# befelix/safe_learning

Hardware: NVIDIA H100
Metric: grid-point Lyapunov checks/sec (2D pendulum, M=500 GP) (higher is better)
Workload: dtype f64

## Files before the change

### include/slb200.h

```cpp
#ifndef SLB200_H
#define SLB200_H

#include <stdint.h>

#ifdef __cplusplus
extern "C" {
#endif

#define SLB_ABI_VERSION 6
#define SLB_MAX_DIM 6
#define SLB_MAX_IN  8
#define SLB_MAX_OUT 6
#define SLB_MAX_ACT 2
#define SLB_TILE_POINTS 64
#define SLB_HEAD_RANK 64
#define SLB_MAX_RANKS 16

typedef struct slb_grid {
    int32_t ndim;
    int32_t _pad;
    int64_t nindex;
    int64_t num_points[SLB_MAX_DIM];
    double  offset[SLB_MAX_DIM];
    double  unit_maxes[SLB_MAX_DIM];
    double  upper[SLB_MAX_DIM];
    const double* discrete_points;
} slb_grid;

enum slb_fn_kind {
    SLB_FN_NONE = 0,
    SLB_FN_CONSTANT = 1,
    SLB_FN_LINEAR = 2,
    SLB_FN_QUADRATIC = 3,
    SLB_FN_TRIANGULATION = 4,
    SLB_FN_PENDULUM = 5,
    SLB_FN_CARTPOLE = 6,
    SLB_FN_LYAPUNOV_NN = 7,
    SLB_FN_MLP = 8,
    SLB_FN_VANDERPOL = 9,
    SLB_FN_PIECEWISE_CONSTANT = 10
};
#define SLB_FLAG_SATURATE 1u
#define SLB_FLAG_ABS      2u
#define SLB_FLAG_NORM1    4u
#define SLB_FLAG_PROJECT  8u
#define SLB_FLAG_SCALE   16u
#define SLB_FLAG_GRADIENT 32u
#define SLB_FLAG_MAXABS  64u

typedef struct slb_function {
    int32_t kind;
    int32_t in_dim;
    int32_t out_dim;
    uint32_t flags;
    double  out_scale;
    double  lower, upper;
    double  cparams[24];
    const double*  matrix;
    const double*  hyperplanes;
    const int64_t* unit_simplices;
    const int32_t* corner_simplex;
    int32_t nsimplex;
    int32_t _pad;
    slb_grid grid;
} slb_function;

enum slb_kernel_kind {
    SLB_K_RBF = 0,
    SLB_K_MATERN12 = 1,
    SLB_K_MATERN32 = 2,
    SLB_K_MATERN52 = 3,
    SLB_K_LINEAR = 4,
    SLB_K_CONSTANT = 5,
    SLB_K_WHITE = 6
};
#define SLB_MAX_KPRIM 6

typedef struct slb_kernel_prim {
    int32_t kind;
    int32_t term;
    double  variance;
    double  w[SLB_MAX_IN];
} slb_kernel_prim;

typedef struct slb_kernel {
    int32_t num_prims;
    int32_t _pad;
    slb_kernel_prim prims[SLB_MAX_KPRIM];
} slb_kernel;

typedef struct slb_gp_factor {
    int32_t M;
    int32_t nrb;
    const double* Xs;
    const double* Wpack;
    double lengthscales[SLB_MAX_IN];
    double variance;
    double scale;
    double kss;
    slb_kernel kernel;
    const double* Whead;
    const double* Wheadp;
    const double* Xhead;
    int32_t head_rows;
    int32_t _pad2;
    const double* Xf;
    double hmax;
} slb_gp_factor;

typedef struct slb_gp_output {
    int32_t factor;
    int32_t _pad;
    double  beta;
    const double* alpha;
    const double* gamma;
    const double* prior_mean;
    const double* gamma_f;
    double gamma_l1;
} slb_gp_output;

typedef struct slb_gp_stack {
    int32_t num_outputs;
    int32_t num_factors;
    int32_t input_dim;
    int32_t _pad;
    slb_gp_factor factors[SLB_MAX_OUT];
    slb_gp_output outputs[SLB_MAX_OUT];
} slb_gp_stack;

typedef struct slb_sweep {
    slb_grid     grid;
    slb_function policy;
    slb_function dynamics;
    slb_gp_stack gp;
    slb_function lyapunov;
    slb_function lipschitz_v;
    double lv_const;
    double lf_const;
    double tau;
    slb_function lipschitz_f;
    const double* lf_values;
    int64_t lf_index_base;
} slb_sweep;

typedef struct slb_bellman {
    slb_grid     grid;
    slb_function policy;
    slb_function dynamics;
    slb_gp_stack gp;
    slb_function reward;
    slb_function value;
    double gamma;
    int32_t fixed_action;
    int32_t _pad;
    double action[SLB_MAX_ACT];
} slb_bellman;


typedef struct slb_fail_key {
    uint64_t key_value;
    int64_t  key_index;
    int64_t  n_ok;
    int64_t  _pad;
} slb_fail_key;

typedef struct slb_prefix_stats {
    int64_t  n_safe;
    int64_t  n_below;
    uint64_t max_below;
    uint64_t max_all;
} slb_prefix_stats;

typedef struct slb_exchange {
    int32_t world;
    int32_t rank;
    slb_fail_key* slots[SLB_MAX_RANKS];
    int64_t* seq_dev;
} slb_exchange;

int         slb_abi_version(void);
const char* slb_last_error(void);
int         slb_device_count(void);
int         slb_struct_sizes(int64_t* out, int32_t n);
int64_t     slb_launch_count(void);
void        slb_note_graph_replay(int64_t kernels);

int         slb_debug_phase_timing(void* buffer_dev);
int         slb_debug_head_timing(void* buffer_dev);
int         slb_debug_stage1_timing(void* buffer_dev);
int         slb_record_factor_dependency(void* stream);
int         slb_restore_tables(void* dst_dev, const void* src_host, int64_t split_bytes, int64_t total_bytes,
                               void* stream, void* side_stream);
int         slb_debug_filter_stages(int32_t mask);
int         slb_debug_screening_probe(double* mu_dev, double* dm_dev);
int         slb_debug_det_fast(int32_t enable);
int         slb_debug_refine_split(int64_t upto32);

int64_t slb_packed_len(int32_t M);
int slb_pack_factor(void* stream, const double* Linv_dev, int32_t M, double* Wpack_dev);

int slb_pivoted_subset(void* stream, const double* kernel_dev, int32_t M, int32_t r,
                       int64_t* picks_dev, double* scratch_dev);

int slb_gp_predict(void* stream, const slb_gp_stack* gp, const double* points_dev, int64_t n,
                   double* mean_dev, double* err_dev, int32_t want_var);
int slb_gp_mean(void* stream, const slb_gp_stack* gp, const double* points_dev, int64_t n, double* mean_dev);
int64_t slb_gp_vjp_workspace(const slb_gp_stack* gp, int64_t n);
int slb_gp_vjp(void* stream, const slb_gp_stack* gp, const double* points_dev, int64_t n,
               const double* grad_mean_dev, const double* grad_err_dev, double* grad_points_dev,
               void* workspace_dev);

#define SLB_GP_HYPER_TILE 64
#define SLB_GP_HYPER_SLOTS (SLB_MAX_KPRIM * (1 + SLB_MAX_IN) + 1)
int64_t slb_gp_lml_grad_workspace(int32_t M);
int slb_gp_lml_grad(void* stream, const double* X_dev, int32_t M, int32_t d_in, const slb_kernel* kern,
                    const double* Kinv_dev, const double* alpha_dev, double* grad_dev, void* workspace_dev);
int slb_gp_lml_grad_cols(void* stream, const double* X_dev, int32_t M, int32_t d_in, const slb_kernel* kern,
                         const double* Kinv_dev, const double* alpha_dev, int32_t k, double* grad_dev,
                         void* workspace_dev);

int slb_lyapunov_sweep(void* stream, const slb_sweep* cfg, int64_t idx_begin, int64_t idx_end,
                       uint8_t* negative_dev, double* values_dev, double* decrease_dev,
                       double* threshold_dev, double* mean_dev, double* err_dev);
int64_t slb_filter_workspace(int64_t n);
int slb_debug_filter_lists(int64_t n, int64_t* offsets);
int slb_filter_stage1(const slb_sweep* cfg);
#define SLB_MEAN_NONE 0
#define SLB_MEAN_FP64 1
#define SLB_MEAN_FP32_SCREENED 2
#define SLB_MEAN_GRID_FACTORED 3
int slb_filter_mean_scheme(const slb_sweep* cfg);
int slb_lyapunov_sweep_filtered(void* stream, const slb_sweep* cfg, int64_t idx_begin,
                                int64_t idx_end, uint8_t* negative_dev, double* values_dev,
                                void* workspace_dev, int64_t* stats_dev);
int slb_safe_set_step(void* stream, const slb_sweep* cfg, int64_t idx_begin, int64_t idx_end,
                      uint8_t* negative_dev, const double* values_dev, const uint8_t* initial_dev,
                      void* workspace_dev, int64_t* stats_dev, slb_fail_key* key_dev, uint8_t* safe_dev,
                      slb_prefix_stats* prefix_stats_dev);
int slb_debug_refine(void* stream, const slb_sweep* cfg, int64_t idx_begin, int64_t n_max,
                     const int64_t* list_dev, const unsigned long long* count_dev,
                     uint8_t* negative_dev, double* values_dev, double* mean_dev, double* err_dev,
                     void* workspace_dev);
int slb_lyapunov_points(void* stream, const slb_sweep* cfg, const double* states_dev, int64_t n,
                        uint8_t* negative_dev, double* values_dev, double* decrease_dev,
                        double* threshold_dev, double* mean_dev, double* err_dev);

int64_t slb_first_fail_workspace(int64_t n);
int slb_first_fail(void* stream, const double* values_dev, const uint8_t* negative_dev,
                   const uint8_t* initial_dev , int64_t n, int64_t idx_begin,
                   void* workspace_dev, slb_fail_key* result_dev);
int slb_first_fail_x(void* stream, const double* values_dev, const uint8_t* negative_dev,
                     const uint8_t* initial_dev, int64_t n, int64_t idx_begin, void* workspace_dev,
                     slb_fail_key* result_dev, const slb_exchange* xchg);
int slb_apply_prefix_x(void* stream, const double* values_dev, const uint8_t* initial_dev,
                       int64_t n, int64_t idx_begin, slb_fail_key* key_out_dev, uint8_t* safe_dev,
                       void* workspace_dev, slb_prefix_stats* stats_dev, const slb_exchange* xchg);
int slb_combine_fail_keys(void* stream, const slb_fail_key* gathered_dev, int32_t world,
                          slb_fail_key* out_dev);
int slb_apply_prefix(void* stream, const double* values_dev, const uint8_t* initial_dev,
                     int64_t n, int64_t idx_begin, const slb_fail_key* key_dev,
                     uint8_t* safe_dev, void* workspace_dev, slb_prefix_stats* stats_dev);

int64_t slb_no_shrink_workspace(int64_t n, int64_t batch);
int slb_no_shrink_scan(void* stream, const int64_t* order_dev, const uint8_t* negative_dev,
                       const uint8_t* prev_safe_dev, const uint8_t* initial_dev, const double* n_req_dev,
                       int64_t n, int64_t batch, int64_t max_refinement, void* workspace_dev,
                       uint8_t* candidates_dev);
int slb_no_shrink_resolve(void* stream, const int64_t* order_dev, const double* values_dev,
                          const uint8_t* negative_dev, const uint8_t* prev_safe_dev,
                          const int64_t* prev_refinement_dev, const uint8_t* initial_dev,
                          const double* n_req_dev, const uint8_t* refined_dev, int64_t n, int64_t batch,
                          int64_t max_refinement, void* workspace_dev, uint8_t* safe_dev,
                          int64_t* refinement_dev, int64_t* cmax_position_dev, double* cmax_dev);

int slb_eval_function(void* stream, const slb_function* fn, const double* points_dev, int64_t n,
                      double* out_dev);
int slb_function_columns(const slb_function* fn);
int slb_index_to_state(void* stream, const slb_grid* grid, int64_t idx_begin, int64_t idx_end,
                       double* states_dev);

int slb_bellman_sweep(void* stream, const slb_bellman* cfg, int64_t idx_begin, int64_t idx_end,
                      double* out_dev);
int64_t slb_bellman_argmax_workspace(const slb_bellman* cfg, int32_t n_actions);
int slb_bellman_argmax(void* stream, const slb_bellman* cfg, int64_t idx_begin, int64_t idx_end,
                       const double* actions_dev, int32_t n_actions, const double* constraint_dev,
                       int32_t* best_dev, double* best_value_dev, void* workspace_dev);
int slb_max_abs_diff(void* stream, const double* a_dev, const double* b_dev, int64_t n,
                     double* result_dev);

int64_t slb_rollout_workspace(const slb_bellman* cfg, int64_t n, int32_t reward);
int slb_rollout(void* stream, const slb_bellman* cfg, const double* states_dev, int64_t idx_begin,
                int64_t n, int32_t horizon, const double* equilibrium_host, double tol,
                uint8_t* roa_dev, double* end_states_dev, double* traj_dev, void* workspace_dev);
int slb_reward_rollout(void* stream, const slb_bellman* cfg, const double* states_dev, int64_t idx_begin,
                       int64_t n, int32_t horizon, const double* discount_dev, double tol,
                       double* sums_dev, int64_t* stop_dev, void* workspace_dev);
int slb_rollout_gp_mean(void* stream, const slb_bellman* cfg, const double* states_dev, int64_t idx_begin,
                        int64_t n, int32_t horizon, const double* equilibrium_host, double tol,
                        uint8_t* roa_dev, double* end_states_dev, double* traj_dev, void* workspace_dev);
int slb_reward_rollout_gp_mean(void* stream, const slb_bellman* cfg, const double* states_dev,
                               int64_t idx_begin, int64_t n, int32_t horizon, const double* discount_dev,
                               double tol, double* sums_dev, int64_t* stop_dev, void* workspace_dev);

#define SLB_VALUE_STATS 16
#define SLB_VALUE_CONVERGED 0
#define SLB_VALUE_MAX_ITERS 1
#define SLB_VALUE_NEGATIVE_WEIGHT 2
#define SLB_VALUE_NOT_CONTRACTIVE 3
#define SLB_VALUE_NAN 4
int slb_value_operator(void* stream, const slb_bellman* cfg, int64_t idx_begin, int64_t idx_end,
                       void* cols_dev, double* weights_dev, double* rewards_dev, uint64_t* stats_dev);
int slb_value_operator_points(void* stream, const slb_function* value, const double* next_states_dev,
                              int64_t n, void* cols_dev, double* weights_dev, uint64_t* stats_dev);
int64_t slb_value_solve_workspace(int64_t n, int32_t ncols);
int slb_value_solve(void* stream, int64_t n, int32_t ncols, const void* cols_dev, const double* weights_dev,
                    const double* rewards_dev, double gamma, double tol, int64_t max_iters,
                    double* v_inout_dev, void* workspace_dev, uint64_t* stats_dev);

int64_t slb_function_vjp_workspace(const slb_function* fn, int64_t n);
int slb_function_vjp(void* stream, const slb_function* fn, const double* points_dev, int64_t n,
                     const double* grad_out_dev, double* grad_in_dev, double* grad_params_dev,
                     double* out_dev, void* workspace_dev);
int slb_grid_nearest_index(void* stream, const slb_grid* grid, const double* points_dev, int64_t n,
                           int64_t* idx_dev);
int slb_triangulation_rows(void* stream, const slb_function* fn, const double* points_dev, int64_t n,
                           int64_t* cols_dev, double* weights_dev);

#ifdef __cplusplus
}
#endif
#endif
```

### safe_learning_b200/_native.py

```python

from __future__ import annotations

import ctypes as C
import os

SLB_MAX_DIM = 6
SLB_MAX_IN = 8
SLB_MAX_OUT = 6
SLB_MAX_ACT = 2
SLB_TILE_POINTS = 64
SLB_HEAD_RANK = 64
SLB_MAX_RANKS = 16

FN_NONE, FN_CONSTANT, FN_LINEAR, FN_QUADRATIC, FN_TRIANGULATION, FN_PENDULUM, FN_CARTPOLE, \
    FN_LYAPUNOV_NN, FN_MLP, FN_VANDERPOL, FN_PIECEWISE_CONSTANT = range(11)
FLAG_SATURATE, FLAG_ABS, FLAG_NORM1, FLAG_PROJECT, FLAG_SCALE, FLAG_GRADIENT, FLAG_MAXABS = \
    1, 2, 4, 8, 16, 32, 64
K_RBF, K_MATERN12, K_MATERN32, K_MATERN52, K_LINEAR, K_CONSTANT, K_WHITE = range(7)
SLB_MAX_KPRIM = 6
SLB_GP_HYPER_TILE = 64
SLB_GP_HYPER_SLOTS = SLB_MAX_KPRIM * (1 + SLB_MAX_IN) + 1
ABI_VERSION = 6
VALUE_STATS = 16
VALUE_CONVERGED, VALUE_MAX_ITERS, VALUE_NEGATIVE_WEIGHT, VALUE_NOT_CONTRACTIVE, VALUE_NAN = range(5)
MEAN_NONE, MEAN_FP64, MEAN_FP32_SCREENED, MEAN_GRID_FACTORED = range(4)

UINT64_MAX = (1 << 64) - 1
INT64_MAX = (1 << 63) - 1


class NativeLibraryError(RuntimeError):
    """libslb200 is missing, mismatched, or reported an error."""


class SlbGrid(C.Structure):
    _fields_ = [("ndim", C.c_int32), ("_pad", C.c_int32), ("nindex", C.c_int64),
                ("num_points", C.c_int64 * SLB_MAX_DIM), ("offset", C.c_double * SLB_MAX_DIM),
                ("unit_maxes", C.c_double * SLB_MAX_DIM), ("upper", C.c_double * SLB_MAX_DIM),
                ("discrete_points", C.c_void_p)]


class SlbFunction(C.Structure):
    _fields_ = [("kind", C.c_int32), ("in_dim", C.c_int32), ("out_dim", C.c_int32),
                ("flags", C.c_uint32), ("out_scale", C.c_double), ("lower", C.c_double),
                ("upper", C.c_double), ("cparams", C.c_double * 24), ("matrix", C.c_void_p),
                ("hyperplanes", C.c_void_p), ("unit_simplices", C.c_void_p),
                ("corner_simplex", C.c_void_p), ("nsimplex", C.c_int32), ("_pad", C.c_int32), ("grid", SlbGrid)]


class SlbKernelPrim(C.Structure):
    _fields_ = [("kind", C.c_int32), ("term", C.c_int32), ("variance", C.c_double),
                ("w", C.c_double * SLB_MAX_IN)]


class SlbKernel(C.Structure):
    _fields_ = [("num_prims", C.c_int32), ("_pad", C.c_int32),
                ("prims", SlbKernelPrim * SLB_MAX_KPRIM)]


class SlbGpFactor(C.Structure):
    _fields_ = [("M", C.c_int32), ("nrb", C.c_int32), ("Xs", C.c_void_p), ("Wpack", C.c_void_p),
                ("lengthscales", C.c_double * SLB_MAX_IN), ("variance", C.c_double),
                ("scale", C.c_double), ("kss", C.c_double), ("kernel", SlbKernel),
                ("Whead", C.c_void_p), ("Wheadp", C.c_void_p), ("Xhead", C.c_void_p),
                ("head_rows", C.c_int32),
                ("_pad2", C.c_int32), ("Xf", C.c_void_p), ("hmax", C.c_double)]


class SlbGpOutput(C.Structure):
    _fields_ = [("factor", C.c_int32), ("_pad", C.c_int32), ("beta", C.c_double),
                ("alpha", C.c_void_p), ("gamma", C.c_void_p), ("prior_mean", C.c_void_p),
                ("gamma_f", C.c_void_p), ("gamma_l1", C.c_double)]


class SlbGpStack(C.Structure):
    _fields_ = [("num_outputs", C.c_int32), ("num_factors", C.c_int32),
                ("input_dim", C.c_int32), ("_pad", C.c_int32),
                ("factors", SlbGpFactor * SLB_MAX_OUT), ("outputs", SlbGpOutput * SLB_MAX_OUT)]


class SlbSweep(C.Structure):
    _fields_ = [("grid", SlbGrid), ("policy", SlbFunction), ("dynamics", SlbFunction),
                ("gp", SlbGpStack), ("lyapunov", SlbFunction), ("lipschitz_v", SlbFunction),
                ("lv_const", C.c_double), ("lf_const", C.c_double), ("tau", C.c_double),
                ("lipschitz_f", SlbFunction), ("lf_values", C.c_void_p),
                ("lf_index_base", C.c_int64)]


class SlbBellman(C.Structure):
    _fields_ = [("grid", SlbGrid), ("policy", SlbFunction), ("dynamics", SlbFunction),
                ("gp", SlbGpStack), ("reward", SlbFunction), ("value", SlbFunction),
                ("gamma", C.c_double), ("fixed_action", C.c_int32), ("_pad", C.c_int32),
                ("action", C.c_double * SLB_MAX_ACT)]


class SlbFailKey(C.Structure):
    _fields_ = [("key_value", C.c_uint64), ("key_index", C.c_int64), ("n_ok", C.c_int64),
                ("_pad", C.c_int64)]


class SlbPrefixStats(C.Structure):
    _fields_ = [("n_safe", C.c_int64), ("n_below", C.c_int64), ("max_below", C.c_uint64),
                ("max_all", C.c_uint64)]


class SlbExchange(C.Structure):
    _fields_ = [("world", C.c_int32), ("rank", C.c_int32),
                ("slots", C.c_void_p * SLB_MAX_RANKS), ("seq_dev", C.c_void_p)]


_STRUCTS = (SlbGrid, SlbFunction, SlbGpFactor, SlbGpOutput, SlbGpStack, SlbSweep, SlbBellman,
            SlbFailKey, SlbPrefixStats, SlbExchange)

LIB_PATH = os.path.join(os.path.dirname(os.path.abspath(__file__)), "libslb200.so")

_vp, _i64, _i32, _dp = C.c_void_p, C.c_int64, C.c_int32, C.c_void_p

SIGNATURES = {
    "slb_abi_version": (C.c_int, []),
    "slb_last_error": (C.c_char_p, []),
    "slb_device_count": (C.c_int, []),
    "slb_struct_sizes": (C.c_int, [C.POINTER(C.c_int64), _i32]),
    "slb_launch_count": (C.c_int64, []),
    "slb_note_graph_replay": (None, [_i64]),
    "slb_debug_phase_timing": (C.c_int, [_vp]),
    "slb_debug_head_timing": (C.c_int, [_vp]),
    "slb_debug_stage1_timing": (C.c_int, [_vp]),
    "slb_record_factor_dependency": (C.c_int, [_vp]),
    "slb_restore_tables": (C.c_int, [_vp, _vp, _i64, _i64, _vp, _vp]),
    "slb_debug_refine_split": (C.c_int, [_i64]),
    "slb_debug_det_fast": (C.c_int, [_i32]),
    "slb_debug_filter_stages": (C.c_int, [_i32]),
    "slb_debug_screening_probe": (C.c_int, [_dp, _dp]),
    "slb_filter_stage1": (C.c_int, [C.POINTER(SlbSweep)]),
    "slb_filter_mean_scheme": (C.c_int, [C.POINTER(SlbSweep)]),
    "slb_packed_len": (C.c_int64, [_i32]),
    "slb_pack_factor": (C.c_int, [_vp, _dp, _i32, _dp]),
    "slb_pivoted_subset": (C.c_int, [_vp, _dp, _i32, _i32, _vp, _dp]),
    "slb_gp_predict": (C.c_int, [_vp, C.POINTER(SlbGpStack), _dp, _i64, _dp, _dp, _i32]),
    "slb_lyapunov_sweep": (C.c_int, [_vp, C.POINTER(SlbSweep), _i64, _i64, _dp, _dp, _dp, _dp,
                                     _dp, _dp]),
    "slb_lyapunov_points": (C.c_int, [_vp, C.POINTER(SlbSweep), _dp, _i64, _dp, _dp, _dp, _dp,
                                      _dp, _dp]),
    "slb_filter_workspace": (C.c_int64, [_i64]),
    "slb_debug_filter_lists": (C.c_int, [_i64, C.POINTER(C.c_int64)]),
    "slb_lyapunov_sweep_filtered": (C.c_int, [_vp, C.POINTER(SlbSweep), _i64, _i64, _dp, _dp, _vp,
                                              _vp]),
    "slb_safe_set_step": (C.c_int, [_vp, C.POINTER(SlbSweep), _i64, _i64, _dp, _dp, _dp, _vp, _vp, _vp,
                                    _dp, _vp]),
    "slb_debug_refine": (C.c_int, [_vp, C.POINTER(SlbSweep), _i64, _i64, _vp, _vp, _vp, _dp, _dp, _dp,
                                   _vp]),
    "slb_first_fail_workspace": (C.c_int64, [_i64]),
    "slb_first_fail_x": (C.c_int, [_vp, _dp, _dp, _dp, _i64, _i64, _vp, _vp,
                                   C.POINTER(SlbExchange)]),
    "slb_apply_prefix_x": (C.c_int, [_vp, _dp, _dp, _i64, _i64, _vp, _dp, _vp, _vp,
                                     C.POINTER(SlbExchange)]),
    "slb_first_fail": (C.c_int, [_vp, _dp, _dp, _dp, _i64, _i64, _vp, _vp]),
    "slb_combine_fail_keys": (C.c_int, [_vp, _vp, _i32, _vp]),
    "slb_apply_prefix": (C.c_int, [_vp, _dp, _dp, _i64, _i64, _vp, _dp, _vp, _vp]),
    "slb_no_shrink_workspace": (C.c_int64, [_i64, _i64]),
    "slb_no_shrink_scan": (C.c_int, [_vp, _dp, _dp, _dp, _dp, _dp, _i64, _i64, _i64, _vp, _dp]),
    "slb_no_shrink_resolve": (C.c_int, [_vp, _dp, _dp, _dp, _dp, _dp, _dp, _dp, _dp, _i64, _i64, _i64,
                                        _vp, _dp, _dp, _dp, _dp]),
    "slb_eval_function": (C.c_int, [_vp, C.POINTER(SlbFunction), _dp, _i64, _dp]),
    "slb_function_columns": (C.c_int, [C.POINTER(SlbFunction)]),
    "slb_index_to_state": (C.c_int, [_vp, C.POINTER(SlbGrid), _i64, _i64, _dp]),
    "slb_bellman_sweep": (C.c_int, [_vp, C.POINTER(SlbBellman), _i64, _i64, _dp]),
    "slb_bellman_argmax_workspace": (C.c_int64, [C.POINTER(SlbBellman), _i32]),
    "slb_bellman_argmax": (C.c_int, [_vp, C.POINTER(SlbBellman), _i64, _i64, _dp, _i32, _dp, _dp,
                                     _dp, _vp]),
    "slb_max_abs_diff": (C.c_int, [_vp, _dp, _dp, _i64, _dp]),
    "slb_rollout_workspace": (C.c_int64, [C.POINTER(SlbBellman), _i64, _i32]),
    "slb_rollout": (C.c_int, [_vp, C.POINTER(SlbBellman), _dp, _i64, _i64, _i32, _dp, C.c_double,
                              _vp, _dp, _dp, _vp]),
    "slb_reward_rollout": (C.c_int, [_vp, C.POINTER(SlbBellman), _dp, _i64, _i64, _i32, _dp,
                                     C.c_double, _dp, _vp, _vp]),
    "slb_rollout_gp_mean": (C.c_int, [_vp, C.POINTER(SlbBellman), _dp, _i64, _i64, _i32, _dp, C.c_double,
                                      _vp, _dp, _dp, _vp]),
    "slb_reward_rollout_gp_mean": (C.c_int, [_vp, C.POINTER(SlbBellman), _dp, _i64, _i64, _i32, _dp,
                                             C.c_double, _dp, _vp, _vp]),
    "slb_value_operator": (C.c_int, [_vp, C.POINTER(SlbBellman), _i64, _i64, _vp, _dp, _dp, _vp]),
    "slb_value_operator_points": (C.c_int, [_vp, C.POINTER(SlbFunction), _dp, _i64, _vp, _dp, _vp]),
    "slb_value_solve_workspace": (C.c_int64, [_i64, _i32]),
    "slb_value_solve": (C.c_int, [_vp, _i64, _i32, _vp, _dp, _dp, C.c_double, C.c_double, _i64, _dp,
                                  _vp, _vp]),
    "slb_function_vjp_workspace": (C.c_int64, [C.POINTER(SlbFunction), _i64]),
    "slb_function_vjp": (C.c_int, [_vp, C.POINTER(SlbFunction), _dp, _i64, _dp, _dp, _dp, _dp, _vp]),
    "slb_triangulation_rows": (C.c_int, [_vp, C.POINTER(SlbFunction), _dp, _i64, _vp, _dp]),
    "slb_grid_nearest_index": (C.c_int, [_vp, C.POINTER(SlbGrid), _dp, _i64, _vp]),
    "slb_gp_mean": (C.c_int, [_vp, C.POINTER(SlbGpStack), _dp, _i64, _dp]),
    "slb_gp_vjp_workspace": (C.c_int64, [C.POINTER(SlbGpStack), _i64]),
    "slb_gp_vjp": (C.c_int, [_vp, C.POINTER(SlbGpStack), _dp, _i64, _dp, _dp, _dp, _vp]),
    "slb_gp_lml_grad_workspace": (C.c_int64, [_i32]),
    "slb_gp_lml_grad": (C.c_int, [_vp, _dp, _i32, _i32, C.POINTER(SlbKernel), _dp, _dp, _dp, _vp]),
    "slb_gp_lml_grad_cols": (C.c_int, [_vp, _dp, _i32, _i32, C.POINTER(SlbKernel), _dp, _dp, _i32, _dp, _vp]),
}

_lib = None


def load():
    global _lib
    if _lib is not None:
        return _lib
    if not os.path.exists(LIB_PATH):
        raise NativeLibraryError(
            "%s not found: build it with `python -c 'import __graft_entry__ as g; g.build()'` "
            "(nvcc, sm_90a). safe_learning_b200 has no CPU fallback." % LIB_PATH)
    lib = C.CDLL(LIB_PATH)
    for name, (res, args) in SIGNATURES.items():
        fn = getattr(lib, name)
        fn.restype = res
        fn.argtypes = args
    if lib.slb_abi_version() != ABI_VERSION:
        raise NativeLibraryError("libslb200 ABI version %d != %d (rebuild: python -c 'import "
                                 "__graft_entry__ as g; g.build()')"
                                 % (lib.slb_abi_version(), ABI_VERSION))
    _check_layout(lib)
    _lib = lib
    return lib


def _check_layout(lib):
    sizes = (C.c_int64 * len(_STRUCTS))()
    n = lib.slb_struct_sizes(sizes, len(_STRUCTS))
    if n != len(_STRUCTS):
        raise NativeLibraryError("libslb200 reports %d ABI structs, binding has %d"
                                 % (n, len(_STRUCTS)))
    for st, size in zip(_STRUCTS, sizes):
        if C.sizeof(st) != size:
            raise NativeLibraryError("layout mismatch for %s: ctypes %d bytes, C %d bytes"
                                     % (st.__name__, C.sizeof(st), size))


def last_error():
    return load().slb_last_error().decode("utf-8", "replace")


def check(rc, what):
    if rc != 0:
        raise NativeLibraryError("%s failed (rc=%d): %s" % (what, rc, last_error()))


def require_device():
    lib = load()
    n = lib.slb_device_count()
    if n <= 0:
        raise NativeLibraryError("no CUDA device available: %s" % (last_error() or "count=0"))
    return n


def launch_count():
    return int(load().slb_launch_count())
```

### safe_learning_b200/csrc/common.cuh

```cuda
#pragma once
#include <cuda_runtime.h>
#include <stdint.h>
#include <math.h>

#include <type_traits>

#include "../../include/slb200.h"
#include "exp2_tab64.h"

constexpr int SLB_NUM_SMS = 132;

void slb_set_error(const char* fmt, ...);
void slb_count_launch();

#define SLB_CHECK(cond, ...)                                                     \
    do {                                                                         \
        if (!(cond)) { slb_set_error(__VA_ARGS__); return 1; }                   \
    } while (0)

#define SLB_CUDA(call)                                                           \
    do {                                                                         \
        cudaError_t e__ = (call);                                                \
        if (e__ != cudaSuccess) {                                                \
            slb_set_error("%s failed: %s (%s:%d)", #call, cudaGetErrorString(e__), \
                          __FILE__, __LINE__);                                   \
            return 2;                                                            \
        }                                                                        \
    } while (0)

#define SLB_LAUNCH_CHECK()                                                       \
    do {                                                                         \
        slb_count_launch();                                                      \
        SLB_CUDA(cudaGetLastError());                                            \
    } while (0)

int slb_validate_function(const slb_function* f, const char* what, int expect_in );
int slb_fn_columns(const slb_function& f);
int slb_validate_dynamics(const slb_function* f, const char* who, int d, int m);
int slb_validate_kernel(const slb_kernel& K, int d_in, const char* who);
int slb_validate_gp(const slb_gp_stack* gp);
int slb_validate_staged_tables(const slb_gp_stack* gp, const char* who);
int slb_validate_grid(const slb_grid* g, bool need_points);
int slb_validate_range(const char* who, int64_t idx_begin, int64_t idx_end, int64_t nindex);
int slb_validate_sweep(const slb_sweep* cfg, bool explicit_states, int* m_out);

template <int LO, int HI, class F>
int slb_dispatch_dim(int d, const char* what, F&& launch) {
    SLB_CHECK(d >= LO && d <= HI, "%s %d not compiled (%d..%d)", what, d, LO, HI);
    if constexpr (LO < HI) {
        if (d > LO) return slb_dispatch_dim<LO + 1, HI>(d, what, launch);
    }
    return launch(std::integral_constant<int, LO>{});
}

#define SLB_DEV __device__ __forceinline__

SLB_DEV double f64mul(double a, double b) { return __dmul_rn(a, b); }
SLB_DEV double f64add(double a, double b) { return __dadd_rn(a, b); }
SLB_DEV double f64sub(double a, double b) { return __dsub_rn(a, b); }

SLB_DEV uint64_t value_key(double v) {
    if (v == 0.0) v = 0.0;
    uint64_t b = (uint64_t)__double_as_longlong(v);
    return (b & 0x8000000000000000ull) ? ~b : (b | 0x8000000000000000ull);
}
SLB_DEV double key_value(uint64_t k) {
    uint64_t b = (k & 0x8000000000000000ull) ? (k & 0x7fffffffffffffffull) : ~k;
    return __longlong_as_double((long long)b);
}

struct __align__(16) slb_fold {
    unsigned long long lo, hi;
    unsigned long long n_ok;
    unsigned int ticket;
    unsigned int _pad;
    unsigned long long acc[4];
};
struct slb_fold_target {
    const double* values;
    const uint8_t* initial;
    slb_fold* rec;
};

SLB_DEV unsigned long long atom_cas128(slb_fold* p, unsigned long long lo, unsigned long long hi,
                                       unsigned long long new_lo, unsigned long long new_hi,
                                       unsigned long long* got_hi) {
    unsigned long long got_lo;
    asm volatile("{\n\t.reg .b128 d, c, s;\n\t"
                 "mov.b128 c, {%2, %3};\n\t"
                 "mov.b128 s, {%4, %5};\n\t"
                 "atom.global.cas.b128 d, [%6], c, s;\n\t"
                 "mov.b128 {%0, %1}, d;\n\t}"
                 : "=l"(got_lo), "=l"(*got_hi)
                 : "l"(lo), "l"(hi), "l"(new_lo), "l"(new_hi), "l"(p)
                 : "memory");
    return got_lo;
}

SLB_DEV void fold_key(slb_fold* rec, uint64_t kv, int64_t ki) {
    const unsigned long long hi = ~kv, lo = (unsigned long long)(INT64_MAX - ki);
    unsigned long long cur_hi;
    asm volatile("ld.relaxed.gpu.global.u64 %0, [%1];" : "=l"(cur_hi) : "l"(&rec->hi) : "memory");
    if (hi < cur_hi) return;
    unsigned long long cur_lo = 0;
    while (hi > cur_hi || (hi == cur_hi && lo > cur_lo)) {
        unsigned long long got_hi;
        const unsigned long long got_lo = atom_cas128(rec, cur_lo, cur_hi, lo, hi, &got_hi);
        if (got_lo == cur_lo && got_hi == cur_hi) return;
        cur_lo = got_lo;
        cur_hi = got_hi;
    }
}

SLB_DEV void fold_decided(const slb_fold_target& t, bool mine, bool negative, int64_t rel, int64_t idx_begin) {
    const bool ok = mine && (negative || (t.initial != nullptr && t.initial[rel] != 0));
    const bool fail = mine && !ok;
    const unsigned okb = __ballot_sync(0xffffffffu, ok);
    const unsigned failb = __ballot_sync(0xffffffffu, fail);
    uint64_t kv = fail ? value_key(t.values[rel]) : ~0ull;
    int64_t ki = fail ? idx_begin + rel : INT64_MAX;
    if (failb != 0) {
#pragma unroll
        for (int off = 16; off > 0; off >>= 1) {
            const uint64_t ov = __shfl_xor_sync(0xffffffffu, kv, off);
            const int64_t oi = __shfl_xor_sync(0xffffffffu, ki, off);
            if (ov < kv || (ov == kv && oi < ki)) { kv = ov; ki = oi; }
        }
    }
    if ((threadIdx.x & 31) != 0) return;
    if (okb != 0) atomicAdd(&t.rec->n_ok, (unsigned long long)__popc(okb));
    if (failb != 0) fold_key(t.rec, kv, ki);
}

__constant__ double c_exp2_tab[64] = {SLB_EXP2_TAB64};

SLB_DEV void load_exp_table(double* tab_smem) {
    for (int i = threadIdx.x; i < 64; i += blockDim.x) tab_smem[i] = c_exp2_tab[i];
}

SLB_DEV double exp_neg_tab(double x, const double* __restrict__ tab) {
    const double MAGIC = 6755399441055744.0;
    const double t = fma(x, 92.33248261689366, MAGIC);
    const int n = __double2loint(t);
    const double nd = t - MAGIC;
    double r = fma(nd, -0.01083042469326756, x);
    r = fma(nd, -2.9815858269852933e-12, r);
    double p = 1.0 / 120.0;
    p = fma(p, r, 1.0 / 24.0);
    p = fma(p, r, 1.0 / 6.0);
    p = fma(p, r, 0.5);
    p = fma(p, r, 1.0);
    p = p * r;
    const double T = tab[n & 63];
    const double v = fma(T, p, T);
    const double s = __hiloint2double(__double2hiint(v) + ((n >> 6) << 20), __double2loint(v));
    return x < -700.0 ? 0.0 : s;
}

template <int DIN>
SLB_DEV double kernel_expr_cross(const slb_kernel& K, const double* z, const double* x,
                                 const double* exptab) {
    double total = 0.0, term = 1.0;
    int cur = 0;
    for (int i = 0; i < K.num_prims; ++i) {
        const slb_kernel_prim& P = K.prims[i];
        if (P.term != cur) { total += term; term = 1.0; cur = P.term; }
        double v;
        if (P.kind == SLB_K_LINEAR) {
            v = 0.0;
#pragma unroll
            for (int c = 0; c < DIN; ++c) v = fma(P.w[c] * z[c], x[c], v);
        } else if (P.kind == SLB_K_CONSTANT) {
            v = P.variance;
        } else if (P.kind == SLB_K_WHITE) {
            v = 0.0;
        } else {
            double r2 = 0.0;
#pragma unroll
            for (int c = 0; c < DIN; ++c) {
                const double df = (z[c] - x[c]) * P.w[c];
                r2 = fma(df, df, r2);
            }
            if (P.kind == SLB_K_RBF) {
                v = P.variance * exp_neg_tab(-0.5 * r2, exptab);
            } else {
                const double r = sqrt(r2 + 1e-12);
                if (P.kind == SLB_K_MATERN12) {
                    v = P.variance * exp_neg_tab(-r, exptab);
                } else if (P.kind == SLB_K_MATERN32) {
                    const double sr = 1.7320508075688772 * r;
                    v = P.variance * (1.0 + sr) * exp_neg_tab(-sr, exptab);
                } else {
                    const double sr = 2.23606797749979 * r;
                    v = P.variance * (1.0 + sr + (5.0 / 3.0) * (r * r)) * exp_neg_tab(-sr, exptab);
                }
            }
        }
        term *= v;
    }
    return K.num_prims > 0 ? total + term : 0.0;
}

template <int DIN, int U>
SLB_DEV void kernel_expr_cross_n(const slb_kernel& K, const double* z, const double* const (&x)[U],
                                 const double* exptab, double (&out)[U]) {
    double total[U], term[U];
#pragma unroll
    for (int u = 0; u < U; ++u) { total[u] = 0.0; term[u] = 1.0; }
    int cur = 0;
    for (int i = 0; i < K.num_prims; ++i) {
        const slb_kernel_prim& P = K.prims[i];
        const int kind = P.kind;
        const double var = P.variance;
        if (P.term != cur) {
#pragma unroll
            for (int u = 0; u < U; ++u) { total[u] += term[u]; term[u] = 1.0; }
            cur = P.term;
        }
        double w[DIN];
#pragma unroll
        for (int c = 0; c < DIN; ++c) w[c] = P.w[c];
        double v[U];
        if (kind == SLB_K_LINEAR) {
#pragma unroll
            for (int c = 0; c < DIN; ++c) w[c] *= z[c];
#pragma unroll
            for (int u = 0; u < U; ++u) {
                double a = 0.0;
#pragma unroll
                for (int c = 0; c < DIN; ++c) a = fma(w[c], x[u][c], a);
                v[u] = a;
            }
        } else if (kind == SLB_K_CONSTANT || kind == SLB_K_WHITE) {
#pragma unroll
            for (int u = 0; u < U; ++u) v[u] = kind == SLB_K_CONSTANT ? var : 0.0;
        } else {
            double r2[U];
#pragma unroll
            for (int u = 0; u < U; ++u) {
                double a = 0.0;
#pragma unroll
                for (int c = 0; c < DIN; ++c) {
                    const double df = (z[c] - x[u][c]) * w[c];
                    a = fma(df, df, a);
                }
                r2[u] = a;
            }
            if (kind == SLB_K_RBF) {
#pragma unroll
                for (int u = 0; u < U; ++u) v[u] = var * exp_neg_tab(-0.5 * r2[u], exptab);
            } else {
                const double cs = kind == SLB_K_MATERN12 ? 1.0
                                : kind == SLB_K_MATERN32 ? 1.7320508075688772 : 2.23606797749979;
                const double c1 = kind == SLB_K_MATERN12 ? 0.0 : 1.0;
                const double c2 = kind == SLB_K_MATERN52 ? 1.0 / 3.0 : 0.0;
#pragma unroll
                for (int u = 0; u < U; ++u) {
                    const double sr = cs * sqrt(r2[u] + 1e-12);
                    v[u] = var * fma(fma(c2, sr, c1), sr, 1.0) * exp_neg_tab(-sr, exptab);
                }
            }
        }
#pragma unroll
        for (int u = 0; u < U; ++u) term[u] *= v[u];
    }
#pragma unroll
    for (int u = 0; u < U; ++u) out[u] = K.num_prims > 0 ? total[u] + term[u] : 0.0;
}

template <int DIN>
SLB_DEV double kernel_expr_diag(const slb_kernel& K, const double* z) {
    double total = 0.0, term = 1.0;
    int cur = 0;
    for (int i = 0; i < K.num_prims; ++i) {
        const slb_kernel_prim& P = K.prims[i];
        if (P.term != cur) { total += term; term = 1.0; cur = P.term; }
        double v = P.variance;
        if (P.kind == SLB_K_LINEAR) {
            v = 0.0;
#pragma unroll
            for (int c = 0; c < DIN; ++c) v = fma(P.w[c] * z[c], z[c], v);
        }
        term *= v;
    }
    return K.num_prims > 0 ? total + term : 0.0;
}

SLB_DEV void grid_index_to_state(const slb_grid& g, int64_t idx, double* x) {
    if (g.nindex <= 0x7fffffffll) {
        unsigned rest = (unsigned)idx;
#pragma unroll
        for (int c = SLB_MAX_DIM - 1; c >= 0; --c) {
            if (c < g.ndim) {
                const unsigned n = (unsigned)g.num_points[c];
                const unsigned q = rest / n;
                const unsigned i = rest - q * n;
                rest = q;
                x[c] = f64add(f64mul((double)i, g.unit_maxes[c]), g.offset[c]);
            }
        }
        return;
    }
#pragma unroll
    for (int c = SLB_MAX_DIM - 1; c >= 0; --c) {
        if (c < g.ndim) {
            const int64_t n = g.num_points[c];
            const int64_t i = idx % n;
            idx /= n;
            x[c] = f64add(f64mul((double)i, g.unit_maxes[c]), g.offset[c]);
        }
    }
}

SLB_DEV int64_t grid_nearest_index(const slb_grid& g, const double* inv, const double* x) {
    int64_t idx = 0;
    for (int c = 0; c < g.ndim; ++c) {
        const double xc = x[c];
        if (xc != xc) return -1;
        const double cl = xc < g.offset[c] ? g.offset[c] : (xc > g.upper[c] ? g.upper[c] : xc);
        const double k = rint(f64mul(f64sub(cl, g.offset[c]), inv[c]));
        const int64_t n = g.num_points[c];
        const int64_t i = k > 0.0 ? (k < (double)(n - 1) ? (int64_t)k : n - 1) : 0;
        idx = idx * n + i;
    }
    return idx;
}

SLB_DEV double fmod_exact_pos(double a, double b) {
    double q = floor(a / b);
    double r = fma(-q, b, a);
    if (r < 0.0) r = fma(-(q - 1.0), b, a);
    else if (r >= b) r = fma(-(q + 1.0), b, a);
    return r;
}

enum { TRI_EVAL, TRI_WEIGHTS, TRI_CELL };

template <int FORM>
SLB_DEV void tri_lookup(const slb_function& f, const double* xin, double* out, int64_t* corner_out = nullptr,
                        int* simplex_out = nullptr) {
    const slb_grid& g = f.grid;
    const int d = g.ndim;
    const double eps = 2.220446049250313e-16;
    double unit[SLB_MAX_DIM];
    int64_t corner = 0;
    int poff = 0;
    int pattern = 0;
    bool all_clipped = true;
    for (int c = 0; c < d; ++c) {
        const double* pts = g.discrete_points + poff;
        const int n = (int)g.num_points[c];
        poff += n;
        const double xc = xin[c];
        int k = (int)floor((xc - g.offset[c]) / g.unit_maxes[c]);
        k = k < 0 ? 0 : (k > n - 1 ? n - 1 : k);
        while (k + 1 <= n - 1 && pts[k + 1] <= xc) ++k;
        while (k >= 0 && pts[k] > xc) --k;
        k = k < 0 ? 0 : (k > n - 2 ? n - 2 : k);
        corner = corner * g.num_points[c] + k;
        double cen = f64sub(xc, g.offset[c]);
        const double lo = 2.0 * eps;
        const double hi = f64sub(f64sub(g.upper[c], g.offset[c]), 2.0 * eps);
        if (cen < lo) cen = lo;
        else if (cen > hi) { cen = hi; pattern |= 1 << c; }
        else all_clipped = false;
        unit[c] = fmod_exact_pos(cen, g.unit_maxes[c]);
    }
    if constexpr (FORM == TRI_CELL) {
        double base[SLB_MAX_DIM];
        grid_index_to_state(g, corner, base);
        for (int c = 0; c < d; ++c) unit[c] = f64sub(fmin(fmax(xin[c], g.offset[c]), g.upper[c]), base[c]);
        all_clipped = false;
    }
    int best = 0;
    double best_min = -1e300;
    const bool tabled = all_clipped && f.corner_simplex != nullptr;
    if (tabled) best = f.corner_simplex[pattern];
    for (int s = 0; s < f.nsimplex && !tabled; ++s) {
        const int64_t v0 = f.unit_simplices[s * (d + 1)];
        double o[SLB_MAX_DIM];
        if (g.nindex <= 0x7fffffffll) {
            unsigned t = (unsigned)v0;
            for (int c = d - 1; c >= 0; --c) {
                const unsigned n = (unsigned)g.num_points[c];
                const unsigned qq = t / n;
                o[c] = (double)(t - qq * n) * g.unit_maxes[c];
                t = qq;
            }
        } else {
            int64_t t = v0;
            for (int c = d - 1; c >= 0; --c) {
                o[c] = (double)(t % g.num_points[c]) * g.unit_maxes[c];
                t /= g.num_points[c];
            }
        }
        const double* H = f.hyperplanes + (size_t)s * d * d;
        double wsum = 0.0, wmin = 1e300;
        for (int c = 0; c < d; ++c) {
            double w = 0.0;
            for (int k = 0; k < d; ++k) w += (unit[k] - o[k]) * H[k * d + c];
            wsum += w;
            wmin = fmin(wmin, w);
        }
        wmin = fmin(wmin, 1.0 - wsum);
        if (wmin > best_min) { best_min = wmin; best = s; }
        if (wmin >= -1e-12) break;
    }
    const int64_t* simp = f.unit_simplices + (size_t)best * (d + 1);
    const double* H = f.hyperplanes + (size_t)best * d * d;
    double origin[SLB_MAX_DIM], off[SLB_MAX_DIM];
    grid_index_to_state(g, simp[0] + corner, origin);
    for (int c = 0; c < d; ++c) {
        double xc = xin[c];
        if (f.flags & SLB_FLAG_PROJECT) xc = xc < g.offset[c] ? g.offset[c] : (xc > g.upper[c] ? g.upper[c] : xc);
        off[c] = f64sub(xc, origin[c]);
    }
    double w[SLB_MAX_DIM + 1];
    for (int c = 0; c < d; ++c) {
        double acc = f64mul(off[0], H[c]);
        for (int k = 1; k < d; ++k) acc = f64add(acc, f64mul(off[k], H[k * d + c]));
        w[c + 1] = acc;
    }
    double acc = w[1];
    for (int c = 2; c <= d; ++c) acc = f64add(acc, w[c]);
    w[0] = f64sub(1.0, acc);
    if constexpr (FORM != TRI_EVAL) {
        for (int c = 0; c <= d; ++c) out[c] = w[c];
        *corner_out = corner;
        *simplex_out = best;
        return;
    }
    if (f.flags & SLB_FLAG_GRADIENT) {
        bool nan = false;
        for (int c = 0; c < d; ++c) nan = nan || xin[c] != xin[c];
        if (nan) {
            for (int k = 0; k < d; ++k) out[k] = __longlong_as_double(0x7ff8000000000000ll);
            return;
        }
        for (int k = 0; k < d; ++k) {
            double hs = H[k * d];
            for (int c = 1; c < d; ++c) hs = f64add(hs, H[k * d + c]);
            double v = f64mul(-hs, f.matrix[simp[0] + corner]);
            for (int c = 0; c < d; ++c)
                v = f64add(v, f64mul(H[k * d + c], f.matrix[simp[c + 1] + corner]));
            out[k] = v;
        }
        return;
    }
    const int od = f.out_dim;
    for (int o = 0; o < od; ++o) {
        double v = f64mul(w[0], f.matrix[(simp[0] + corner) * od + o]);
        for (int k = 1; k <= d; ++k)
            v = f64add(v, f64mul(w[k], f.matrix[(simp[k] + corner) * od + o]));
        out[o] = v;
    }
}

SLB_DEV void eval_pendulum(const slb_function& f, const double* in, double* out) {
    const double* p = f.cparams;
    const double g_l = p[0], inertia = p[1], fric_i = p[2], dt = p[3];
    const bool has_norm = p[9] != 0.0, has_fric = p[10] != 0.0;
    double th = in[0], om = in[1], u = in[2];
    if (has_norm) { th = f64mul(th, p[4]); om = f64mul(om, p[5]); u = f64mul(u, p[6]); }
    const double ui = u / inertia;
    for (int i = 0; i < 10; ++i) {
        double acc = f64add(f64mul(g_l, sin(th)), ui);
        if (has_fric) acc = f64sub(acc, f64mul(fric_i, om));
        const double th_n = f64add(th, f64mul(dt, om));
        const double om_n = f64add(om, f64mul(dt, acc));
        th = th_n; om = om_n;
    }
    if (has_norm) { th = f64mul(th, p[7]); om = f64mul(om, p[8]); }
    out[0] = th; out[1] = om;
}

SLB_DEV void eval_cartpole(const slb_function& f, const double* in, double* out) {
    const double* p = f.cparams;
    const double m = p[0], M = p[1], L = p[2], b = p[3], g = p[4], dt = p[5];
    const bool has_norm = p[15] != 0.0;
    double s[4] = {in[0], in[1], in[2], in[3]};
    double u = in[4];
    if (has_norm) { for (int c = 0; c < 4; ++c) s[c] = f64mul(s[c], p[6 + c]); u = f64mul(u, p[10]); }
    for (int i = 0; i < 10; ++i) {
        const double th = s[1], v = s[2], om = s[3];
        const double st = sin(th), ct = cos(th), s2t = sin(2.0 * th);
        const double det = L * (M + m * (st * st));
        const double v_dot = (u - m * L * (om * om) * st - b * om * ct + 0.5 * m * g * L * s2t) * L / det;
        const double om_dot = (u * ct - 0.5 * m * L * (om * om) * s2t - b * (m + M) * om / (m * L)
                               + (m + M) * g * st) / det;
        s[0] = f64add(s[0], f64mul(dt, v));
        s[1] = f64add(s[1], f64mul(dt, om));
        s[2] = f64add(s[2], f64mul(dt, v_dot));
        s[3] = f64add(s[3], f64mul(dt, om_dot));
    }
    if (has_norm) for (int c = 0; c < 4; ++c) s[c] = f64mul(s[c], p[11 + c]);
    for (int c = 0; c < 4; ++c) out[c] = s[c];
}

SLB_DEV void vanderpol_scale(double& x, double& y, double tx, double ty) {
    const double xs = f64add(f64mul(x, tx), f64mul(y, 0.0));
    y = f64add(f64mul(x, 0.0), f64mul(y, ty));
    x = xs;
}

SLB_DEV void eval_vanderpol(const slb_function& f, const double* in, double* out) {
    const double* p = f.cparams;
    const double damping = p[0], dt = p[1];
    const bool has_norm = p[2] != 0.0;
    double x = in[0], y = in[1];
    if (has_norm) vanderpol_scale(x, y, p[3], p[4]);
    for (int i = 0; i < 10; ++i) {
        const double y_dot = f64add(x, f64mul(f64mul(damping, f64sub(f64mul(x, x), 1.0)), y));
        x = f64add(x, f64mul(dt, -y));
        y = f64add(y, f64mul(dt, y_dot));
    }
    if (has_norm) vanderpol_scale(x, y, p[5], p[6]);
    out[0] = x; out[1] = y;
}

#define SLB_NN_MAX_LAYERS 8
#define SLB_NN_MAX_WIDTH 64
#define SLB_NN_HD __host__ __device__ __forceinline__

SLB_NN_HD int nn_layers(const slb_function& f) { return (int)f.cparams[0]; }
SLB_NN_HD int nn_out(const slb_function& f, int l) { return (int)f.cparams[1 + l]; }
SLB_NN_HD int nn_width(const slb_function& f, int l) { return l == 0 ? f.in_dim : nn_out(f, l - 1); }
SLB_NN_HD int nn_act(const slb_function& f, int l) { return (int)f.cparams[9 + l]; }
SLB_NN_HD bool nn_use_bias(const slb_function& f) { return f.kind == SLB_FN_MLP && f.cparams[18] != 0.0; }
SLB_NN_HD bool nn_bias(const slb_function& f, int l) { return nn_use_bias(f) && l + 1 < nn_layers(f); }
SLB_NN_HD double nn_scale(const slb_function& f) { return f.cparams[17]; }
SLB_NN_HD int64_t nn_layer_size(int wi, int wo, bool bias) { return (int64_t)wo * wi + (bias ? wo : 0); }

SLB_DEV double activate(double acc, int act) {
    return act == 0 ? tanh(acc) : (act == 1 ? fmax(acc, 0.0) : acc);
}

SLB_DEV double activate_grad(double h, int act) {
    return act == 0 ? 1.0 - h * h : (act == 1 ? (h > 0.0 ? 1.0 : 0.0) : 1.0);
}

template <class X, class W, class B>
SLB_DEV double nn_unit(int n, X x, W w, bool has_bias, B bias, int act) {
    double acc = f64mul(x(0), w(0));
    for (int k = 1; k < n; ++k) acc = f64add(acc, f64mul(x(k), w(k)));
    if (has_bias) acc = f64add(acc, bias());
    return activate(acc, act);
}

SLB_DEV void nn_layer(const double* P, int wi, int wo, bool bias, int act, const double* h, double* g) {
    const double* b = P + (size_t)wo * wi;
    for (int o = 0; o < wo; ++o) {
        const double* row = P + (size_t)o * wi;
        g[o] = nn_unit(wi, [&](int k) { return h[k]; }, [&](int k) { return row[k]; }, bias,
                       [&] { return b[o]; }, act);
    }
}

template <int KIND>
SLB_DEV void eval_network(const slb_function& f, const double* in, double* out) {
    double h[SLB_NN_MAX_WIDTH], g[SLB_NN_MAX_WIDTH];
    int width = f.in_dim;
    for (int k = 0; k < width; ++k) h[k] = in[k];
    const double* P = f.matrix;
    const int layers = nn_layers(f);
    const bool use_bias = KIND == SLB_FN_MLP && nn_use_bias(f);
    for (int l = 0; l < layers; ++l) {
        const int od = nn_out(f, l);
        const bool bias = use_bias && l + 1 < layers;
        nn_layer(P, width, od, bias, nn_act(f, l), h, g);
        P += nn_layer_size(width, od, bias);
        width = od;
        for (int k = 0; k < width; ++k) h[k] = g[k];
    }
    if constexpr (KIND == SLB_FN_MLP) {
        for (int k = 0; k < width; ++k) out[k] = f64mul(h[k], nn_scale(f));
    } else {
        double v = f64mul(h[0], h[0]);
        for (int k = 1; k < width; ++k) v = f64add(v, f64mul(h[k], h[k]));
        out[0] = v;
    }
}

static __device__ __noinline__ int network_input_gradient(const slb_function& f, const double* in, double* out) {
    double h[SLB_NN_MAX_WIDTH], g[SLB_NN_MAX_WIDTH];
    double d[SLB_NN_MAX_WIDTH], e[SLB_NN_MAX_WIDTH];
    const int layers = nn_layers(f);
    const bool mlp = f.kind == SLB_FN_MLP, use_bias = nn_use_bias(f);
    for (int l = layers - 1; l >= 0; --l) {
        int width = f.in_dim;
        for (int k = 0; k < width; ++k) h[k] = in[k];
        const double* P = f.matrix;
        const double* W = P;
        int wi = width;
        for (int j = 0; j <= l; ++j) {
            const int od = nn_out(f, j);
            const bool bias = use_bias && j + 1 < layers;
            nn_layer(P, width, od, bias, nn_act(f, j), h, g);
            W = P;
            wi = width;
            P += nn_layer_size(width, od, bias);
            width = od;
            for (int k = 0; k < width; ++k) h[k] = g[k];
        }
        const int act = nn_act(f, l);
        if (l == layers - 1) {
            for (int o = 0; o < width; ++o) d[o] = (mlp ? nn_scale(f) : 2.0 * h[o]) * activate_grad(h[o], act);
        } else {
            for (int o = 0; o < width; ++o) d[o] = e[o] * activate_grad(h[o], act);
        }
        for (int k = 0; k < wi; ++k) {
            double s = 0.0;
            for (int o = 0; o < width; ++o) s = fma(d[o], W[(size_t)o * wi + k], s);
            e[k] = s;
        }
    }
    for (int k = 0; k < f.in_dim; ++k) out[k] = e[k];
    return f.in_dim;
}

#ifdef SLB_EVAL_NOINLINE
#define SLB_EVAL_ATTR static __device__ __noinline__
#else
#define SLB_EVAL_ATTR static __device__ __forceinline__
#endif
SLB_EVAL_ATTR int eval_fn(const slb_function& f, const double* in, double* out) {
    int od = f.out_dim;
    switch (f.kind) {
    case SLB_FN_CONSTANT:
        for (int o = 0; o < od; ++o) out[o] = f.cparams[o];
        break;
    case SLB_FN_LINEAR:
        for (int o = 0; o < od; ++o) {
            const double* row = f.matrix + o * f.in_dim;
            double acc = f64mul(in[0], row[0]);
            for (int k = 1; k < f.in_dim; ++k) acc = f64add(acc, f64mul(in[k], row[k]));
            out[o] = acc;
        }
        break;
    case SLB_FN_QUADRATIC: {
        const int n = f.in_dim;
        double total = 0.0;
        for (int c = 0; c < n; ++c) {
            double lin = f64mul(in[0], f.matrix[c]);
            for (int r = 1; r < n; ++r) lin = f64add(lin, f64mul(in[r], f.matrix[r * n + c]));
            const double prod = f64mul(lin, in[c]);
            total = (c == 0) ? prod : f64add(total, prod);
        }
        out[0] = total;
        od = 1;
        break;
    }
    case SLB_FN_TRIANGULATION:
        tri_lookup<TRI_EVAL>(f, in, out);
        break;
    case SLB_FN_PENDULUM:
        eval_pendulum(f, in, out); od = 2;
        break;
    case SLB_FN_CARTPOLE:
        eval_cartpole(f, in, out); od = 4;
        break;
    case SLB_FN_VANDERPOL:
        eval_vanderpol(f, in, out); od = 2;
        break;
    case SLB_FN_LYAPUNOV_NN:
#ifndef SLB_NO_NETWORK_GRADIENT
        if (f.flags & SLB_FLAG_GRADIENT) { od = network_input_gradient(f, in, out); break; }
#endif
        eval_network<SLB_FN_LYAPUNOV_NN>(f, in, out); od = 1;
        break;
    case SLB_FN_MLP:
#ifndef SLB_NO_NETWORK_GRADIENT
        if (f.flags & SLB_FLAG_GRADIENT) { od = network_input_gradient(f, in, out); break; }
#endif
        eval_network<SLB_FN_MLP>(f, in, out);
        break;
    default: {
        const int64_t v = f.kind == SLB_FN_PIECEWISE_CONSTANT ? grid_nearest_index(f.grid, f.cparams, in) : -1;
        for (int o = 0; o < od; ++o)
            out[o] = v < 0 ? __longlong_as_double(0x7ff8000000000000ll) : f.matrix[v * od + o];
        break;
    }
    }
    if (f.flags & SLB_FLAG_SATURATE)
        for (int o = 0; o < od; ++o) out[o] = fmin(fmax(out[o], f.lower), f.upper);
    if (f.flags & (SLB_FLAG_ABS | SLB_FLAG_NORM1))
        for (int o = 0; o < od; ++o) out[o] = fabs(out[o]);
    if (f.flags & SLB_FLAG_NORM1) {
        double acc = out[0];
        for (int o = 1; o < od; ++o) acc = f64add(acc, out[o]);
        out[0] = acc;
        od = 1;
    }
    if (f.flags & SLB_FLAG_MAXABS) {
        double acc = fabs(out[0]);
        for (int o = 1; o < od; ++o) acc = fmax(acc, fabs(out[o]));
        out[0] = acc;
        od = 1;
    }
    if (f.flags & SLB_FLAG_SCALE)
        for (int o = 0; o < od; ++o) out[o] = f64mul(out[o], f.out_scale);
    return od;
}

SLB_DEV int eval_fn_small(const slb_function& f, const double* in, double* out) {
    const int n = f.in_dim;
    if (f.kind == SLB_FN_LINEAR && n <= 4 && f.out_dim <= 2 &&
        !(f.flags & (SLB_FLAG_MAXABS | SLB_FLAG_GRADIENT))) {
        int od = f.out_dim;
        double x[4];
#pragma unroll
        for (int k = 0; k < 4; ++k) x[k] = k < n ? in[k] : 0.0;
        double y[2];
#pragma unroll
        for (int o = 0; o < 2; ++o) {
            if (o < od) {
                const double* row = f.matrix + o * n;
                double acc = f64mul(x[0], __ldg(row));
#pragma unroll
                for (int k = 1; k < 4; ++k)
                    if (k < n) acc = f64add(acc, f64mul(x[k], __ldg(row + k)));
                y[o] = acc;
            } else {
                y[o] = 0.0;
            }
        }
        if (f.flags & SLB_FLAG_SATURATE) {
            y[0] = fmin(fmax(y[0], f.lower), f.upper);
            y[1] = fmin(fmax(y[1], f.lower), f.upper);
        }
        if (f.flags & (SLB_FLAG_ABS | SLB_FLAG_NORM1)) { y[0] = fabs(y[0]); y[1] = fabs(y[1]); }
        if (f.flags & SLB_FLAG_NORM1) {
            if (od == 2) y[0] = f64add(y[0], y[1]);
            od = 1;
        }
        if (f.flags & SLB_FLAG_SCALE) { y[0] = f64mul(y[0], f.out_scale); y[1] = f64mul(y[1], f.out_scale); }
        out[0] = y[0];
        if (od == 2) out[1] = y[1];
        return od;
    }
    if (f.kind == SLB_FN_QUADRATIC && n <= 4 && !(f.flags & ~SLB_FLAG_SCALE)) {
        double x[4];
#pragma unroll
        for (int k = 0; k < 4; ++k) x[k] = k < n ? in[k] : 0.0;
        double total = 0.0;
#pragma unroll
        for (int c = 0; c < 4; ++c) {
            if (c < n) {
                double lin = f64mul(x[0], __ldg(f.matrix + c));
#pragma unroll
                for (int r = 1; r < 4; ++r)
                    if (r < n) lin = f64add(lin, f64mul(x[r], __ldg(f.matrix + r * n + c)));
                const double prod = f64mul(lin, x[c]);
                total = (c == 0) ? prod : f64add(total, prod);
            }
        }
        if (f.flags & SLB_FLAG_SCALE) total = f64mul(total, f.out_scale);
        out[0] = total;
        return 1;
    }
    return eval_fn(f, in, out);
}

template <int N> struct slb_vec { double v[N]; };
constexpr int SLB_MAX_LIN_OUT = 4;

template <int N, int MO>
SLB_DEV slb_vec<MO> eval_linear_reg(const slb_function& f, const double (&x)[N], int& cols) {
    const int od = f.out_dim;
    slb_vec<MO> y;
#pragma unroll
    for (int o = 0; o < MO; ++o) {
        y.v[o] = 0.0;
        if (o < od) {
            const double* row = f.matrix + o * N;
            double acc = f64mul(x[0], __ldg(row));
#pragma unroll
            for (int k = 1; k < N; ++k) acc = f64add(acc, f64mul(x[k], __ldg(row + k)));
            y.v[o] = acc;
        }
    }
    if (f.flags & SLB_FLAG_SATURATE) {
#pragma unroll
        for (int o = 0; o < MO; ++o) y.v[o] = fmin(fmax(y.v[o], f.lower), f.upper);
    }
    if (f.flags & (SLB_FLAG_ABS | SLB_FLAG_NORM1)) {
#pragma unroll
        for (int o = 0; o < MO; ++o) y.v[o] = fabs(y.v[o]);
    }
    cols = od;
    if (f.flags & SLB_FLAG_NORM1) {
#pragma unroll
        for (int o = 1; o < MO; ++o)
            if (o < od) y.v[0] = f64add(y.v[0], y.v[o]);
        cols = 1;
    }
    if (f.flags & SLB_FLAG_SCALE) {
#pragma unroll
        for (int o = 0; o < MO; ++o) y.v[o] = f64mul(y.v[o], f.out_scale);
    }
    return y;
}

template <int N>
SLB_DEV double eval_quadratic_reg(const slb_function& f, const double (&x)[N]) {
    double total = 0.0;
#pragma unroll
    for (int c = 0; c < N; ++c) {
        double lin = f64mul(x[0], __ldg(f.matrix + c));
#pragma unroll
        for (int r = 1; r < N; ++r) lin = f64add(lin, f64mul(x[r], __ldg(f.matrix + r * N + c)));
        const double prod = f64mul(lin, x[c]);
        total = (c == 0) ? prod : f64add(total, prod);
    }
    if (f.flags & SLB_FLAG_SCALE) total = f64mul(total, f.out_scale);
    return total;
}

SLB_DEV void prefetch_descriptor_operands(const slb_sweep& cfg) {
    const int i = threadIdx.x;
    const void* p = nullptr;
    if (i == 0) p = cfg.policy.matrix;
    else if (i == 1) p = cfg.lyapunov.matrix;
    else if (i == 2) p = cfg.lipschitz_v.matrix;
    else if (i == 3) p = cfg.lipschitz_f.matrix;
    else if (i < 4 + cfg.gp.num_outputs && i < 4 + SLB_MAX_OUT) p = cfg.gp.outputs[i - 4].prior_mean;
    if (p != nullptr) asm volatile("prefetch.global.L1 [%0];" ::"l"(p));
}

struct slb_decision { double vx, decrease, threshold; bool negative; };

SLB_DEV void lyapunov_state_terms(const slb_sweep& cfg, const double* x, int64_t flat_index,
                                  double* vx_out, double* threshold_out) {
    double tmp[SLB_MAX_OUT], vx[1];
    eval_fn_small(cfg.lyapunov, x, vx);
    *vx_out = vx[0];
    double lvx;
    if (cfg.lipschitz_v.kind != SLB_FN_NONE) {
        const int nl = eval_fn_small(cfg.lipschitz_v, x, tmp);
        lvx = tmp[0];
        if (nl > 1) {
            lvx = fabs(tmp[0]);
            for (int j = 1; j < nl; ++j) lvx = f64add(lvx, fabs(tmp[j]));
        }
    } else {
        lvx = cfg.lv_const;
    }
    double lf = cfg.lf_const;
    if (cfg.lf_values != nullptr && flat_index >= 0) {
        lf = cfg.lf_values[flat_index - cfg.lf_index_base];
    } else if (cfg.lipschitz_f.kind != SLB_FN_NONE) {
        eval_fn_small(cfg.lipschitz_f, x, tmp);
        lf = tmp[0];
    }
    *threshold_out = f64mul(f64mul(-lvx, f64add(1.0, lf)), cfg.tau);
}

template <int D>
SLB_DEV void lyapunov_state_terms_closed(const slb_sweep& cfg, const double (&x)[D], int64_t flat_index,
                                         double* vx_out, double* threshold_out) {
    *vx_out = eval_quadratic_reg<D>(cfg.lyapunov, x);
    double lvx = cfg.lv_const;
    if (cfg.lipschitz_v.kind != SLB_FN_NONE) {
        int nl;
        const slb_vec<SLB_MAX_LIN_OUT> lv = eval_linear_reg<D, SLB_MAX_LIN_OUT>(cfg.lipschitz_v, x, nl);
        lvx = lv.v[0];
        if (nl > 1) {
            lvx = fabs(lv.v[0]);
#pragma unroll
            for (int j = 1; j < SLB_MAX_LIN_OUT; ++j)
                if (j < nl) lvx = f64add(lvx, fabs(lv.v[j]));
        }
    }
    double lf = cfg.lf_const;
    if (cfg.lf_values != nullptr && flat_index >= 0) {
        lf = cfg.lf_values[flat_index - cfg.lf_index_base];
    } else if (cfg.lipschitz_f.kind != SLB_FN_NONE) {
        int nf;
        lf = eval_linear_reg<D, SLB_MAX_LIN_OUT>(cfg.lipschitz_f, x, nf).v[0];
    }
    *threshold_out = f64mul(f64mul(-lvx, f64add(1.0, lf)), cfg.tau);
}

SLB_DEV double lyapunov_error_bound(const slb_sweep& cfg, const double* mu, const double* err) {
    const int d = cfg.grid.ndim;
    double tmp[SLB_MAX_OUT];
    double bound;
    if (cfg.lipschitz_v.kind != SLB_FN_NONE) {
        const int nl = eval_fn_small(cfg.lipschitz_v, mu, tmp);
        if (nl == 1) {
            bound = f64mul(tmp[0], err[0]);
            for (int j = 1; j < d; ++j) bound = f64add(bound, f64mul(tmp[0], err[j]));
        } else {
            bound = f64mul(tmp[0], err[0]);
            for (int j = 1; j < d; ++j) bound = f64add(bound, f64mul(tmp[j], err[j]));
        }
    } else {
        bound = f64mul(cfg.lv_const, err[0]);
        for (int j = 1; j < d; ++j) bound = f64add(bound, f64mul(cfg.lv_const, err[j]));
    }
    return bound;
}

SLB_DEV slb_decision lyapunov_combine(double vx, double threshold, double vm, double bound) {
    slb_decision r;
    r.vx = vx;
    r.threshold = threshold;
    r.decrease = f64add(f64sub(vm, vx), bound);
    r.negative = r.decrease < r.threshold;
    return r;
}

SLB_DEV slb_decision lyapunov_decide(const slb_sweep& cfg, const double* x, int64_t flat_index,
                                     const double* mu, const double* err) {
    double vx, threshold, vm[1];
    lyapunov_state_terms(cfg, x, flat_index, &vx, &threshold);
    eval_fn_small(cfg.lyapunov, mu, vm);
    const double bound = err != nullptr ? lyapunov_error_bound(cfg, mu, err) : 0.0;
    return lyapunov_combine(vx, threshold, vm[0], bound);
}
```

### safe_learning_b200/csrc/filter.cu

```cuda
#define SLB_EVAL_NOINLINE 1
#include "common.cuh"

#include <atomic>
#include <string.h>
#include <type_traits>

#include "gp_mean_staged.cuh"
#include "gp_mean_grid.cuh"
#include "gp_args.h"

namespace {

constexpr int FT = 64;
constexpr int HR = SLB_HEAD_RANK;
constexpr int HT = 512;
constexpr int HW = HT / 32;
constexpr int HP = 8;
constexpr int HEAD_CTAS = SLB_NUM_SMS;
constexpr int64_t CHUNK = 1 << 22;
constexpr int64_t WS_FOLD = 64 + SLB_SPLIT_TICKET_BYTES;
constexpr int64_t WS_PARTIAL = WS_FOLD + 128;
constexpr int64_t WS_HEAD = WS_PARTIAL + (int64_t)SLB_SPLIT_PARTIAL_BYTES;
static_assert(sizeof(slb_fold) <= WS_PARTIAL - WS_FOLD && WS_FOLD % 16 == 0, "fold record slot");


struct filter_side { double dec0, thr, guard, coef[SLB_MAX_OUT], z[SLB_MAX_IN], dm[SLB_MAX_OUT]; };

struct filter_plan {
    int mean_scheme;
    int factors_staged;
    int mean_off[SLB_MAX_OUT];
    int mean_doubles;
    int tabs;
    int kbuf;
    int sd;
    int wbuf, xbuf;
    int mbuf, mu, merr;
    int need;
    int doubles;
};

struct filter_args {
    int64_t n;
    int64_t idx_begin;
    uint8_t* negative;
    double* values;
    int64_t* list_a;
    filter_side* side_a;
    int64_t* list_b;
    unsigned long long* counts;
    unsigned long long* stats;
    int chunk_rows;
    int max_outputs_per_factor;
    filter_plan plan;
    int prefetch_factors;
    double* probe_mu;
    double* probe_dm;
    unsigned long long* timing;
    unsigned long long* timing1;
    int head_schedule;
    slb_fold_target fold;
};

enum { HM_ENTRY, HM_TABLES, HM_BOUND0, HM_BOUND, HM_SCREENED, HM_MEANS, HM_DECIDED, HM_EXIT };
SLB_DEV void timing_mark(const filter_args& a, int slot) {
    if (a.timing == nullptr || (threadIdx.x & 31) != 0) return;
    unsigned long long t;
    asm volatile("mov.u64 %0, %%globaltimer;" : "=l"(t));
    atomicMax(a.timing + slot, t);
}
SLB_DEV void head_mark(const filter_args& a, int mark) { timing_mark(a, blockIdx.x * 8 + mark); }
enum { S1_ENTRY, S1_PROLOGUE, S1_ITEM, S1_MEANS = S1_ITEM + 4, S1_EXIT };
SLB_DEV void stage1_mark(const filter_args& a, int mark) {
    if (a.timing1 == nullptr || (threadIdx.x & 31) != 0) return;
    unsigned long long t;
    asm volatile("mov.u64 %0, %%globaltimer;" : "=l"(t));
    atomicMax(a.timing1 + blockIdx.x * 8 + mark, t);
}

SLB_DEV int decide(const filter_side& t, const double* shi, int d) {
    double ub = 0.0, lb = 0.0;
    for (int j = 0; j < d; ++j) {
        const double e = t.coef[j] * shi[j];
        ub += fmax(e, 0.0);
        lb += fmin(e, 0.0);
        if (!(e == e)) { ub = e; lb = e; break; }
    }
    const double slack = t.guard + 1e-6 * (fabs(ub) + fabs(lb));
    if (t.dec0 + ub + slack < t.thr) return 1;
    if (t.dec0 + lb - slack >= t.thr) return 0;
    return -1;
}

SLB_DEV long long list_append(bool take, unsigned long long* counter) {
    const unsigned ballot = __ballot_sync(0xffffffffu, take);
    if (ballot == 0) return -1;
    const int lane = threadIdx.x & 31;
    unsigned long long base = 0;
    if (lane == __ffs(ballot) - 1) base = atomicAdd(counter, (unsigned long long)__popc(ballot));
    base = __shfl_sync(0xffffffffu, base, __ffs(ballot) - 1);
    return take ? (long long)(base + __popc(ballot & ((1u << lane) - 1))) : -1;
}

SLB_DEV void count_stat(bool hit, unsigned long long* slot) {
    const unsigned ballot = __ballot_sync(0xffffffffu, hit);
    if (ballot != 0 && (threadIdx.x & 31) == 0) atomicAdd(slot, (unsigned long long)__popc(ballot));
}

SLB_DEV void mean_decision_terms(const slb_sweep& cfg, filter_side& t, double vx, const double* mu,
                                 const double* mean_err) {
    const int D = cfg.gp.num_outputs;
    double vm[1];
    eval_fn_small(cfg.lyapunov, mu, vm);
    t.dec0 = f64sub(vm[0], vx);
    double lvmu = 0.0;
    double lverr = 0.0;
    {
        double lv[SLB_MAX_OUT];
        int nl = 1;
        if (cfg.lipschitz_v.kind != SLB_FN_NONE) nl = eval_fn_small(cfg.lipschitz_v, mu, lv);
        else lv[0] = cfg.lv_const;
        for (int j = 0; j < SLB_MAX_OUT; ++j) {
            const double l = j < D ? (nl == 1 ? lv[0] : lv[j]) : 0.0;
            t.coef[j] = j < D ? l * cfg.gp.outputs[j].beta : 0.0;
            if (j < D) { lvmu += fabs(l * mu[j]); lverr += fabs(l) * mean_err[j]; }
        }
    }
    t.guard = 1e-6 * (fabs(vm[0]) + fabs(vx) + fabs(t.thr) + lvmu) + 4.0 * lverr + 1e-300;
}

template <int D>
struct cf_terms { double dec0, thr, guard, coef[D]; };

template <int D>
SLB_DEV void cf_mean_terms(const slb_sweep& cfg, cf_terms<D>& t, double vx, const double (&mu)[D],
                           const double (&mean_err)[D]) {
    const double vm = eval_quadratic_reg<D>(cfg.lyapunov, mu);
    t.dec0 = f64sub(vm, vx);
    int nl = 1;
    slb_vec<SLB_MAX_LIN_OUT> lv;
    lv.v[0] = cfg.lv_const;
    if (cfg.lipschitz_v.kind != SLB_FN_NONE) lv = eval_linear_reg<D, SLB_MAX_LIN_OUT>(cfg.lipschitz_v, mu, nl);
    double lvmu = 0.0, lverr = 0.0;
#pragma unroll
    for (int j = 0; j < D; ++j) {
        const double l = nl == 1 ? lv.v[0] : lv.v[j];
        t.coef[j] = l * cfg.gp.outputs[j].beta;
        lvmu += fabs(l * mu[j]);
        lverr += fabs(l) * mean_err[j];
    }
    t.guard = 1e-6 * (fabs(vm) + fabs(vx) + fabs(t.thr) + lvmu) + 4.0 * lverr + 1e-300;
}

template <int D>
SLB_DEV double screening_slack(const slb_sweep& cfg, const double (&mu)[D], const double (&dm)[D],
                               const double (&shi)[D]) {
    const slb_function& V = cfg.lyapunov;
    double poison = 0.0;
    if constexpr (D < 4) {
#pragma unroll
        for (int i = 0; i < D; ++i) poison += 0.0 * mu[i] + 0.0 * dm[i];
    }
    double bs[D];
#pragma unroll
    for (int j = 0; j < D; ++j) bs[j] = f64mul(fabs(cfg.gp.outputs[j].beta), shi[j]);
    double dv = 0.0;
#pragma unroll
    for (int i = 0; i < D; ++i) {
        double gi = 0.0;
#pragma unroll
        for (int r = 0; r < D; ++r) gi += mu[r] * (__ldg(V.matrix + r * D + i) + __ldg(V.matrix + i * D + r));
        dv += fabs(gi) * dm[i];
#pragma unroll
        for (int j = 0; j < D; ++j) dv += fabs(__ldg(V.matrix + i * D + j)) * dm[i] * dm[j];
    }
    dv += poison;
    if (V.flags & SLB_FLAG_SCALE) dv *= fabs(V.out_scale);
    double dl = 0.0;
    const slb_function& L = cfg.lipschitz_v;
    if (L.kind == SLB_FN_LINEAR) {
        const double sc = (L.flags & SLB_FLAG_SCALE) ? fabs(L.out_scale) : 1.0;
        const int mo = L.out_dim;
        double row[SLB_MAX_LIN_OUT];
#pragma unroll
        for (int o = 0; o < SLB_MAX_LIN_OUT; ++o) {
            row[o] = 0.0;
#pragma unroll
            for (int i = 0; i < D; ++i)
                if (o < mo) row[o] += fabs(__ldg(L.matrix + o * D + i)) * dm[i];
        }
        if ((L.flags & SLB_FLAG_NORM1) || mo == 1) {
            double sb = bs[0];
#pragma unroll
            for (int j = 1; j < D; ++j) sb = f64add(sb, bs[j]);
            dl = sc * (row[0] + row[1] + row[2] + row[3]) * sb;
        } else {
#pragma unroll
            for (int j = 0; j < D; ++j) dl += sc * row[j] * bs[j];
            if constexpr (D < 4) dl += 0.0 * sc;
        }
    }
    return 1.000001 * (dv + dl);
}

template <int D>
SLB_DEV int cf_decide(const cf_terms<D>& t, const double (&shi)[D]) {
    double ub = 0.0, lb = 0.0;
#pragma unroll
    for (int j = 0; j < D; ++j) {
        const double e = t.coef[j] * shi[j];
        ub += fmax(e, 0.0);
        lb += fmin(e, 0.0);
        if (!(e == e)) { ub = e; lb = e; }
    }
    const double slack = t.guard + 1e-6 * (fabs(ub) + fabs(lb));
    if (t.dec0 + ub + slack < t.thr) return 1;
    if (t.dec0 + lb - slack >= t.thr) return 0;
    return -1;
}

template <int D>
SLB_DEV int screened_outcome(const slb_sweep& cfg, double vx, double thr, const double (&mu)[D],
                             const double (&dm)[D], const double (&shi)[D]) {
    cf_terms<D> t;
    t.thr = thr;
    double zero[D];
#pragma unroll
    for (int j = 0; j < D; ++j) zero[j] = 0.0;
    cf_mean_terms<D>(cfg, t, vx, mu, zero);
    t.guard += screening_slack<D>(cfg, mu, dm, shi);
    return cf_decide<D>(t, shi);
}

template <int D>
SLB_DEV void cf_prior_sigma(const slb_gp_stack& gp, double (&shi)[D]) {
#pragma unroll
    for (int j = 0; j < D; ++j) shi[j] = sqrt(gp.factors[gp.outputs[j].factor].variance);
}

template <int D, class Fn>
SLB_DEV void cf_for_outputs_on_factor(const slb_gp_stack& gp, int f, Fn&& fn) {
    unsigned mask = 0;
#pragma unroll
    for (int o = 0; o < D; ++o)
        if (gp.outputs[o].factor == f) mask |= 1u << o;
    const auto call = [&](auto no) {
        constexpr int NO = decltype(no)::value;
        int outs[NO];
        unsigned m = mask;
#pragma unroll
        for (int q = 0; q < NO; ++q) { outs[q] = __ffs(m) - 1; m &= m - 1; }
        fn(no, outs);
    };
    switch (__popc(mask)) {
    case 1: call(std::integral_constant<int, 1>{}); break;
    case 2: if constexpr (D >= 2) call(std::integral_constant<int, 2>{}); break;
    case 3: if constexpr (D >= 3) call(std::integral_constant<int, 3>{}); break;
    case 4: if constexpr (D >= 4) call(std::integral_constant<int, 4>{}); break;
    default: break;
    }
}

template <int DIN>
SLB_DEV bool stage1_point(const slb_sweep& cfg, int64_t index, double* z, double* vx, double* thr) {
    grid_index_to_state(cfg.grid, index, z);
    lyapunov_state_terms(cfg, z, index, vx, thr);
    double u[SLB_MAX_OUT];
    const int m = eval_fn_small(cfg.policy, z, u);
    for (int c = 0; c < m; ++c) z[cfg.grid.ndim + c] = u[c];
    bool sane = true;
#pragma unroll
    for (int c = 0; c < DIN; ++c) sane &= fabs(z[c]) < 1e100;
    return sane;
}

template <int DIN>
SLB_DEV void prior_sigma_bound(const slb_gp_stack& gp, const double* z, double* shi) {
    for (int j = 0; j < gp.num_outputs; ++j) {
        const slb_gp_factor& F = gp.factors[gp.outputs[j].factor];
        shi[j] = sqrt(F.kernel.num_prims > 0 ? kernel_expr_diag<DIN>(F.kernel, z) : F.variance);
    }
}

SLB_DEV long long stage1_finish(const filter_args& a, bool valid, int64_t rel, int outcome, double vx) {
    const bool undecided = valid && outcome < 0;
    if (valid) {
        a.negative[rel] = outcome > 0 ? 1 : 0;
        if (a.values != nullptr) a.values[rel] = vx;
    }
    const long long slot = list_append(undecided, a.counts + 0);
    if (undecided) a.list_a[slot] = rel;
    if (a.fold.rec != nullptr) fold_decided(a.fold, valid && outcome >= 0, outcome > 0, rel, a.idx_begin);
    if (a.stats != nullptr) {
        count_stat(valid && !undecided, a.stats + 0);
        count_stat(valid, a.stats + 3);
    }
    return slot;
}

template <int DIN, int D>
SLB_DEV void stage1_screened_finish(const slb_sweep& cfg, const filter_args& a, bool valid, bool sane, int64_t rel,
                                    const double* z, double thr, double vx, const double* mu_in,
                                    const double* dm_in) {
    double mu[D], dm[D], shi[D];
#pragma unroll
    for (int j = 0; j < D; ++j) { mu[j] = mu_in[j]; dm[j] = dm_in[j]; }
    if (a.probe_mu != nullptr && valid) {
#pragma unroll
        for (int o = 0; o < D; ++o) {
            a.probe_mu[rel * D + o] = mu[o];
            a.probe_dm[rel * D + o] = sane ? dm[o] : f64_inf();
        }
    }
    cf_prior_sigma<D>(cfg.gp, shi);
    const int screened = screened_outcome<D>(cfg, vx, thr, mu, dm, shi);
    const long long slot = stage1_finish(a, valid, rel, sane ? screened : -1, vx);
    if (slot >= 0) {
        filter_side* dst = a.side_a + slot;
        dst->dec0 = vx;
        dst->thr = thr;
#pragma unroll
        for (int c = 0; c < DIN; ++c) dst->z[c] = z[c];
#pragma unroll
        for (int j = 0; j < D; ++j) {
            dst->coef[j] = mu[j];
            dst->dm[j] = sane ? dm[j] : f64_inf();
        }
    }
}

template <int DIN>
__global__ void __launch_bounds__(FT, 7)
filter_mean_kernel(const __grid_constant__ slb_sweep cfg, const filter_args a) {
    extern __shared__ __align__(16) unsigned char smem_raw[];
    prefetch_descriptor_operands(cfg);
    mean_pipe P;
    double *tab512, *tab64;
    mean_pipe_setup(P, smem_raw, DIN, a.chunk_rows, a.max_outputs_per_factor, cfg.gp, &tab512, &tab64);
    uint64_t* bar = P.bar;
    if (threadIdx.x == 0) mean_pipe_init(P, tab512);
    mean_pipe_start<DIN>(cfg.gp, P);
    __syncthreads();

    const int64_t rel0 = (int64_t)blockIdx.x * FT + threadIdx.x;
    const bool valid = rel0 < a.n;
    const int64_t rel = valid ? rel0 : a.n - 1;
    filter_side t;
    double vx;
    const bool sane = stage1_point<DIN>(cfg, a.idx_begin + rel, t.z, &vx, &t.thr);

    slb_bulk::mbar_wait(bar + 2, 0);
    double mu[SLB_MAX_OUT];
    double mean_err[SLB_MAX_OUT];
    gp_mean_staged<DIN, true>(cfg.gp, t.z, mu, mean_err, tab512, tab64, P);

    mean_decision_terms(cfg, t, vx, mu, mean_err);

    double shi[SLB_MAX_OUT];
    prior_sigma_bound<DIN>(cfg.gp, t.z, shi);
    const long long slot = stage1_finish(a, valid, rel, sane ? decide(t, shi, cfg.gp.num_outputs) : -1, vx);
    if (slot >= 0) a.side_a[slot] = t;
    timing_mark(a, HEAD_CTAS * 8);
}

template <int DIN, int D>
__global__ void __launch_bounds__(FT, 7)
filter_mean32_kernel(const __grid_constant__ slb_sweep cfg, const filter_args a) {
    extern __shared__ __align__(16) unsigned char smem_raw[];
    __shared__ double s_cen[SLB_MAX_IN];
    prefetch_descriptor_operands(cfg);
    mean_pipe P;
    mean32_bufs B;
    mean32_bufs_setup<DIN>(B, mean_pipe_setup(P, smem_raw, DIN, a.chunk_rows, a.max_outputs_per_factor, cfg.gp,
                                              nullptr, nullptr), a.chunk_rows, FT / 32);
    if (threadIdx.x == 0) mean_pipe_init(P, nullptr);
    mean_pipe_start<DIN>(cfg.gp, P);

    const int64_t rel0 = (int64_t)blockIdx.x * FT + threadIdx.x;
    const bool valid = rel0 < a.n;
    const int64_t rel = valid ? rel0 : a.n - 1;
    double z[SLB_MAX_IN], vx, thr;
    bool sane = stage1_point<DIN>(cfg, a.idx_begin + rel, z, &vx, &thr);
    if (threadIdx.x == FT / 2) {
#pragma unroll
        for (int c = 0; c < DIN; ++c) s_cen[c] = z[c];
    }
    __syncthreads();
    double zcen[DIN];
#pragma unroll
    for (int c = 0; c < DIN; ++c) zcen[c] = s_cen[c];

    double mu[SLB_MAX_OUT], dm[SLB_MAX_OUT];
    gp_mean32_staged<DIN>(cfg.gp, z, zcen, mu, dm, sane, P, B);
    stage1_screened_finish<DIN, D>(cfg, a, valid, sane, rel, z, thr, vx, mu, dm);
    timing_mark(a, HEAD_CTAS * 8);
}

constexpr int GRID_OUTPUTS = 2;

template <int D>
__global__ void __launch_bounds__(GT, 2)
filter_grid_mean_kernel(const __grid_constant__ slb_sweep cfg, const filter_args a) {
    static_assert(D == GRID_OUTPUTS, "the factored grid mean is written for z = [x0, x1, u]");
    stage1_mark(a, S1_ENTRY);
    extern __shared__ __align__(16) unsigned char smem_raw[];
    double* smem = reinterpret_cast<double*>(smem_raw);
    double* tab = smem + GSMEM_TAB;
    double* zs = smem + GSMEM_Z;
    double* mus = smem + GSMEM_MU;
    double* dms = smem + GSMEM_DM;
    int* present = reinterpret_cast<int*>(smem + GSMEM_REG);
    int8_t* regs = reinterpret_cast<int8_t*>(present + GT / 32);
    for (int i = threadIdx.x; i < 512; i += GT) tab[i] = g_exp_tables[i];
    prefetch_descriptor_operands(cfg);
    for (int f = 0; f < cfg.gp.num_factors; ++f) {
        const size_t bytes = (size_t)padded_rows(cfg.gp.factors[f].M) * 4 * sizeof(double);
        for (size_t off = (size_t)threadIdx.x * 128; off < bytes; off += (size_t)GT * 128)
            asm volatile("prefetch.global.L2 [%0];" ::"l"(reinterpret_cast<const char*>(cfg.gp.factors[f].Xf) + off));
    }
#pragma unroll
    for (int o = 0; o < D; ++o) {
        const size_t bytes = (size_t)padded_rows(cfg.gp.factors[cfg.gp.outputs[o].factor].M) * sizeof(double);
        for (size_t off = (size_t)threadIdx.x * 128; off < bytes; off += (size_t)GT * 128)
            asm volatile("prefetch.global.L2 [%0];" ::"l"(reinterpret_cast<const char*>(cfg.gp.outputs[o].gamma_f) + off));
    }
    const slb_grid& g = cfg.grid;
    const int64_t n0 = g.num_points[0], n1 = g.num_points[1];
    const int64_t ntc = (n1 + GC - 1) / GC;
    const int64_t row0 = a.idx_begin / n1 + (int64_t)(blockIdx.x / ntc) * GR;
    const int64_t col0 = (int64_t)(blockIdx.x % ntc) * GC;
    const slb_function& pol = cfg.policy;

    const int pt = threadIdx.x;
    const int64_t gi = row0 + pt / GC, gk = col0 + pt % GC;
    const int64_t flat = gi * n1 + gk;
    const bool valid = gi < n0 && gk < n1 && flat >= a.idx_begin && flat < a.idx_begin + a.n;
    const int64_t rel = valid ? flat - a.idx_begin : 0;
    const double x[D] = {f64add(f64mul((double)gi, g.unit_maxes[0]), g.offset[0]),
                         f64add(f64mul((double)gk, g.unit_maxes[1]), g.offset[1])};
    double vx, thr;
    lyapunov_state_terms_closed<D>(cfg, x, a.idx_begin + rel, &vx, &thr);
    int cols;
    const double u = eval_linear_reg<D, 1>(pol, x, cols).v[0];
    const bool sane = fabs(x[0]) < 1e100 && fabs(x[1]) < 1e100 && fabs(u) < 1e100;
    zs[pt * 3 + 0] = x[0];
    zs[pt * 3 + 1] = x[1];
    zs[pt * 3 + 2] = u;
    {
        const double ulo = (pol.flags & SLB_FLAG_SCALE) ? f64mul(pol.lower, pol.out_scale) : pol.lower;
        const double uhi = (pol.flags & SLB_FLAG_SCALE) ? f64mul(pol.upper, pol.out_scale) : pol.upper;
        const int reg = !(valid && sane) ? -1
                        : (pol.flags & SLB_FLAG_SATURATE) && u == ulo ? 0
                        : (pol.flags & SLB_FLAG_SATURATE) && u == uhi ? 1 : 2;
        regs[pt] = (int8_t)reg;
        const unsigned rbits = __reduce_or_sync(0xffffffffu, reg >= 0 ? 1u << reg : 0u);
        if ((threadIdx.x & 31) == 0) present[threadIdx.x >> 5] = (int)rbits;
    }
#pragma unroll
    for (int o = 0; o < GNO; ++o) { mus[pt * GNO + o] = 0.0; dms[pt * GNO + o] = f64_inf(); }
    __syncthreads();
    stage1_mark(a, S1_PROLOGUE);

    int regimes = 0;
#pragma unroll
    for (int w = 0; w < GT / 32; ++w) regimes |= present[w];
    const int grp = threadIdx.x / GGT;
    int item = 0;
    for (int f = 0; f < cfg.gp.num_factors; ++f) {
        cf_for_outputs_on_factor<D>(cfg.gp, f, [&](auto no, const int* outs) {
            constexpr int NO = decltype(no)::value;
            for (int r = 0; r < 3; ++r) {
                if (!((regimes >> r) & 1)) continue;
                if (item % GG == grp) {
                    constexpr int NP = NO == 4 ? 2 : NO;
#pragma unroll
                    for (int q0 = 0; q0 < NO; q0 += NP)
                        grid_mean_item<NP>(cfg, f, r, outs + q0, smem + grp * GGRP, tab, row0, col0, zs, regs, mus,
                                           dms);
                    stage1_mark(a, S1_ITEM + min(item, 3));
                }
                ++item;
            }
        });
    }
    __syncthreads();
    stage1_mark(a, S1_MEANS);

    double mu[D], dm[D], shi[D];
#pragma unroll
    for (int j = 0; j < D; ++j) {
        mu[j] = mus[pt * GNO + j];
        dm[j] = sane ? dms[pt * GNO + j] : f64_inf();
    }
    if (a.probe_mu != nullptr && valid) {
#pragma unroll
        for (int o = 0; o < D; ++o) {
            a.probe_mu[rel * D + o] = mu[o];
            a.probe_dm[rel * D + o] = dm[o];
        }
    }
    cf_prior_sigma<D>(cfg.gp, shi);
    const int outcome = sane ? screened_outcome<D>(cfg, vx, thr, mu, dm, shi) : -1;
    const bool undecided = valid && outcome < 0;
    if (valid) {
        a.negative[rel] = outcome > 0 ? 1 : 0;
        if (a.values != nullptr) a.values[rel] = vx;
    }
    if (a.fold.rec != nullptr) fold_decided(a.fold, valid && outcome >= 0, outcome > 0, rel, a.idx_begin);
    bool fp64 = sane;
#pragma unroll
    for (int j = 0; j < D; ++j) fp64 &= dm[j] < f64_inf();
    constexpr int NW = GT / 32;
    unsigned* s_cnt = reinterpret_cast<unsigned*>(zs);
    unsigned long long* s_base = reinterpret_cast<unsigned long long*>(s_cnt + 4 * NW);
    const int lane = threadIdx.x & 31, warp = threadIdx.x >> 5;
    const unsigned und = __ballot_sync(0xffffffffu, undecided);
    {
        const unsigned dec = __ballot_sync(0xffffffffu, valid && !undecided);
        const unsigned val = __ballot_sync(0xffffffffu, valid);
        const unsigned open = __ballot_sync(0xffffffffu, undecided && !fp64);
        if (lane == 0) {
            s_cnt[0 * NW + warp] = __popc(und);
            s_cnt[1 * NW + warp] = __popc(dec);
            s_cnt[2 * NW + warp] = __popc(val);
            s_cnt[3 * NW + warp] = __popc(open);
        }
    }
    __syncthreads();
    if (threadIdx.x < 4) {
        unsigned total = 0;
#pragma unroll
        for (int w = 0; w < NW; ++w) total += s_cnt[threadIdx.x * NW + w];
        if (threadIdx.x == 0) *s_base = total != 0 ? atomicAdd(a.counts + 0, (unsigned long long)total) : 0;
        else if (total != 0 && threadIdx.x == 3) atomicAdd(a.counts + 2, (unsigned long long)total);
        else if (total != 0 && a.stats != nullptr) atomicAdd(a.stats + (threadIdx.x == 1 ? 0 : 3), (unsigned long long)total);
    }
    __syncthreads();
    if (undecided) {
        unsigned long long slot = *s_base + __popc(und & ((1u << lane) - 1));
        for (int w = 0; w < warp; ++w) slot += s_cnt[w];
        a.list_a[slot] = rel;
        filter_side* dst = a.side_a + slot;
        dst->dec0 = vx;
        dst->thr = thr;
        dst->z[0] = x[0];
        dst->z[1] = x[1];
        dst->z[2] = u;
#pragma unroll
        for (int j = 0; j < D; ++j) {
            dst->coef[j] = mu[j];
            dst->dm[j] = dm[j];
        }
    }
    timing_mark(a, HEAD_CTAS * 8);
    stage1_mark(a, S1_EXIT);
}


template <int DIN, int NO>
SLB_DEV void head_mean_factor(const double* __restrict__ xf, int Mp, const double* zs, double zz, int r,
                              int L, const double* __restrict__ tab512, double* dot) {
    constexpr int W = DIN + 1;
    const double* __restrict__ gm = xf + (size_t)Mp * W;
    double d0[NO], d1[NO];
#pragma unroll
    for (int q = 0; q < NO; ++q) { d0[q] = 0.0; d1[q] = 0.0; }
    for (int j = r; j < Mp; j += 4 * L) {
        double arg[4];
#pragma unroll
        for (int u = 0; u < 4; ++u) {
            const int jc = min(j + L * u, Mp - 1);
            double row[W];
            load_row<W>(xf + jc * W, row);
            double acc = row[DIN] + zz;
#pragma unroll
            for (int c = 0; c < DIN; ++c) acc = fma(zs[c], row[c], acc);
            arg[u] = acc;
        }
#pragma unroll
        for (int u = 0; u < 4; ++u) {
            bool far;
            double k = exp_neg_fast(arg[u], tab512, far);
            k = (far || j + L * u >= Mp) ? 0.0 : k;
            const int jc = min(j + L * u, Mp - 1);
#pragma unroll
            for (int q = 0; q < NO; ++q) {
                if (u & 1) d1[q] = fma(k, gm[q * Mp + jc], d1[q]);
                else d0[q] = fma(k, gm[q * Mp + jc], d0[q]);
            }
        }
    }
#pragma unroll
    for (int q = 0; q < NO; ++q) {
        double v = d0[q] + d1[q];
        for (int off = L >> 1; off > 0; off >>= 1) v += __shfl_xor_sync(0xffffffffu, v, off);
        dot[q] = v;
    }
}

template <int DIN, int D>
SLB_DEV void head_round_means(const slb_sweep& cfg, const filter_args& a, const int* slots, int nneed,
                              int64_t grp0, int64_t count, const double* mbuf, const double* tab512,
                              double* mu_s, double* merr_s, int tid0, int nthreads) {
    const int nf = cfg.gp.num_factors;
    int L = 32;
    while (L > 4 && nneed * L > nthreads) L >>= 1;
    const int r = threadIdx.x & (L - 1);
    const int per_warp = 32 / L;
    const int nloop = (nneed + per_warp - 1) / per_warp * per_warp;
    for (int i = ((int)threadIdx.x - tid0) / L; i < nloop; i += nthreads / L) {
        const bool live = i < nneed;
        const int slot = live ? (slots != nullptr ? slots[i] : i) : 0;
        const int64_t k = (grp0 + (int64_t)(slot / HP) * gridDim.x) * HP + (slot % HP);
        double z[DIN];
#pragma unroll
        for (int c = 0; c < DIN; ++c) z[c] = (live && k < count) ? a.side_a[k].z[c] : 0.0;
        for (int f = 0; f < nf; ++f) {
            const slb_gp_factor& F = cfg.gp.factors[f];
            double zs[DIN];
            double zz = 0.0;
#pragma unroll
            for (int c = 0; c < DIN; ++c) {
                zs[c] = z[c] / F.lengthscales[c];
                zz = fma(zs[c], zs[c], zz);
            }
            zz *= -0.5;
            const int Mp = padded_rows(F.M);
            const double* xf = mbuf + a.plan.mean_off[f];
            const auto factor_means = [&](auto no, const int* outs) {
                constexpr int NO = decltype(no)::value;
                double dot[NO];
                head_mean_factor<DIN, NO>(xf, Mp, zs, zz, r, L, tab512, dot);
                if (r == 0 && live) {
#pragma unroll
                    for (int q = 0; q < NO; ++q)
                        mean_output_finish<DIN>(F, cfg.gp.outputs[outs[q]], z, dot[q], zz, 1.0, false,
                                                &mu_s[slot * SLB_MAX_OUT + outs[q]],
                                                &merr_s[slot * SLB_MAX_OUT + outs[q]]);
                }
            };
            cf_for_outputs_on_factor<D>(cfg.gp, f, factor_means);
        }
    }
}

template <int DIN>
SLB_DEV void head_group_entries(const slb_sweep& cfg, const filter_args& a, int64_t grp, int64_t count,
                                filter_side& t, int64_t& rel, bool& mine, double* shi) {
    const int lane = threadIdx.x & 31;
    const int64_t k = grp * HP + min(lane, HP - 1);
    mine = lane < HP && k < count;
    t = filter_side{};
    rel = 0;
    if (mine) { t = a.side_a[k]; rel = a.list_a[k]; }
    prior_sigma_bound<DIN>(cfg.gp, t.z, shi);
    if (!mine)
        for (int j = 0; j < cfg.gp.num_outputs; ++j) shi[j] = 0.0;
}

template <int DIN, bool ALL_STAGED, bool PLAIN>
SLB_DEV double head_factor_sdev(const slb_sweep& cfg, const filter_args& a, int f, const double* z,
                                bool mine, const double* exptab, double* kw, const double* wbuf,
                                const double* xbuf, uint64_t* bar) {
    const int lane = threadIdx.x & 31;
    const slb_gp_factor& F = cfg.gp.factors[f];
    const int rows = F.head_rows;
    const bool general = !PLAIN && F.kernel.num_prims > 0;
    const double s2 = f64mul(F.scale, F.scale);
    const bool staged = ALL_STAGED || f < a.plan.factors_staged;
    const double* xh = xbuf + (size_t)f * HR * DIN;
    if (!ALL_STAGED && !staged) xh = F.Xhead;
    double zown[DIN];
#pragma unroll
    for (int c = 0; c < DIN; ++c) zown[c] = general ? z[c] : z[c] / F.lengthscales[c];
#pragma unroll
    for (int p = 0; p < HP; ++p) {
        double zs[DIN];
#pragma unroll
        for (int c = 0; c < DIN; ++c) zs[c] = __shfl_sync(0xffffffffu, zown[c], p);
#pragma unroll
        for (int h = 0; h < 2; ++h) {
            const int j = lane + 32 * h;
            double kv = 0.0;
            if (j < rows) {
                const double* xr = xh + j * DIN;
                if (general) {
                    kv = kernel_expr_cross<DIN>(F.kernel, zs, xr, exptab);
                } else {
                    double a2 = 0.0;
#pragma unroll
                    for (int c = 0; c < DIN; ++c) { const double df = zs[c] - xr[c]; a2 = fma(df, df, a2); }
                    kv = F.variance * exp_neg_tab(-0.5 * a2, exptab);
                }
                kv = s2 * kv;
            }
            kw[j * HP + p] = kv;
        }
    }
    __syncwarp();
    double ssp = 0.0;
    const double* __restrict__ Wp = wbuf + (size_t)f * HR * HR;
    if (!ALL_STAGED && !staged) Wp = F.Wheadp;
    else slb_bulk::mbar_wait(bar + 1, 0);
    double acc[8][2];
#pragma unroll
    for (int b = 0; b < 8; ++b) { acc[b][0] = 0.0; acc[b][1] = 0.0; }
#pragma unroll
    for (int sk = 0; sk < 16; ++sk) {
        const double bf = kw[(4 * sk + (lane & 3)) * HP + (lane >> 2)];
#pragma unroll
        for (int b = sk / 2; b < 8; ++b) {
            const double af = Wp[(b * 16 + sk) * 32 + lane];
            asm volatile("mma.sync.aligned.m8n8k4.row.col.f64.f64.f64.f64 {%0,%1}, {%2}, {%3}, {%0,%1};"
                         : "+d"(acc[b][0]), "+d"(acc[b][1]) : "d"(af), "d"(bf));
        }
    }
    __syncwarp();
    double v0 = 0.0, v1 = 0.0;
#pragma unroll
    for (int b = 0; b < 8; ++b) { v0 = fma(acc[b][0], acc[b][0], v0); v1 = fma(acc[b][1], acc[b][1], v1); }
#pragma unroll
    for (int off = 4; off < 32; off <<= 1) {
        v0 += __shfl_xor_sync(0xffffffffu, v0, off);
        v1 += __shfl_xor_sync(0xffffffffu, v1, off);
    }
    const double s0 = __shfl_sync(0xffffffffu, v0, (lane >> 1) & 3);
    const double s1 = __shfl_sync(0xffffffffu, v1, (lane >> 1) & 3);
    ssp = (lane & 1) ? s1 : s0;
    double kss = F.kss;
    if (general && mine) kss = s2 * kernel_expr_diag<DIN>(F.kernel, z);
    const double sdev = sqrt(f64sub(kss, ssp) / s2);
    return sdev;
}

template <int DIN, bool ALL_STAGED, int CD, int D>
SLB_DEV void head_group_bound(const slb_sweep& cfg, const filter_args& a, const double* z, bool mine,
                              const double* exptab, double* kw, const double* wbuf, const double* xbuf,
                              uint64_t* bar, double (&shi)[D]) {
    slb_bulk::mbar_wait(bar + 0, 0);
    head_mark(a, HM_TABLES);
    for (int f = 0; f < cfg.gp.num_factors; ++f) {
        if (cfg.gp.factors[f].head_rows <= 0) continue;
        const double sdev = head_factor_sdev<DIN, ALL_STAGED, (CD > 0)>(cfg, a, f, z, mine, exptab, kw, wbuf, xbuf,
                                                                        bar);
#pragma unroll
        for (int j = 0; j < D; ++j)
            if (j < cfg.gp.num_outputs && cfg.gp.outputs[j].factor == f) shi[j] = sdev;
        if (f == 0) head_mark(a, HM_BOUND0);
    }
    head_mark(a, HM_BOUND);
}

SLB_DEV int head_entry_decision(const slb_sweep& cfg, const filter_args&, filter_side& t, const double* shi,
                                bool mine, double&, bool& need) {
    need = false;
    return mine ? decide(t, shi, cfg.gp.num_outputs) : 0;
}

template <int DIN, int D>
struct cf_entry { int k; int64_t rel; double vx, thr, z[DIN], mu[D], dm[D]; };

template <int DIN, int D>
SLB_DEV void head_group_entries(const slb_sweep& cfg, const filter_args& a, int64_t grp, int64_t count,
                                cf_entry<DIN, D>& t, int64_t& rel, bool& mine, double (&shi)[D]) {
    const int lane = threadIdx.x & 31;
    const int64_t k = grp * HP + min(lane, HP - 1);
    mine = lane < HP && k < count;
    t.k = mine ? (int)k : -1;
#pragma unroll
    for (int c = 0; c < DIN; ++c) t.z[c] = mine ? a.side_a[k].z[c] : 0.0;
    rel = 0;
    cf_prior_sigma<D>(cfg.gp, shi);
    if (!mine) {
#pragma unroll
        for (int j = 0; j < D; ++j) shi[j] = 0.0;
    }
}

template <int DIN, int D>
SLB_DEV int head_entry_decision(const slb_sweep& cfg, const filter_args& a, cf_entry<DIN, D>& t,
                                const double (&shi)[D], bool mine, double& vx, bool& need) {
    t.rel = 0;
    t.vx = 0.0;
    t.thr = 0.0;
#pragma unroll
    for (int j = 0; j < D; ++j) { t.mu[j] = 0.0; t.dm[j] = 0.0; }
    if (t.k >= 0) {
        t.rel = a.list_a[t.k];
        const filter_side* e = a.side_a + t.k;
        t.vx = e->dec0;
        t.thr = e->thr;
#pragma unroll
        for (int j = 0; j < D; ++j) { t.mu[j] = e->coef[j]; t.dm[j] = e->dm[j]; }
    }
    vx = t.vx;
    const int screened = screened_outcome<D>(cfg, vx, t.thr, t.mu, t.dm, shi);
    const int outcome = mine ? screened : 0;
    bool finite = a.plan.mean_scheme == SLB_MEAN_GRID_FACTORED;
#pragma unroll
    for (int j = 0; j < D; ++j) finite &= t.dm[j] < f64_inf();
    need = mine && outcome < 0 && !finite;
    head_mark(a, HM_SCREENED);
    return outcome;
}

template <int DIN, int D>
SLB_DEV int head_mean_decision(const slb_sweep& cfg, cf_entry<DIN, D>& t, double vx, const double (&shi)[D],
                               const double* mu_s, const double* merr_s, int slot) {
    double mu[D], merr[D];
#pragma unroll
    for (int j = 0; j < D; ++j) {
        mu[j] = mu_s[slot * SLB_MAX_OUT + j];
        merr[j] = merr_s[slot * SLB_MAX_OUT + j];
    }
    cf_terms<D> terms;
    terms.thr = t.thr;
    cf_mean_terms<D>(cfg, terms, vx, mu, merr);
    return cf_decide<D>(terms, shi);
}

SLB_DEV int64_t entry_rel(const filter_side&, int64_t rel) { return rel; }
template <int DIN, int D>
SLB_DEV int64_t entry_rel(const cf_entry<DIN, D>& t, int64_t) { return t.rel; }

SLB_DEV void head_wait_landings(uint64_t* bar) {
    for (int b = 0; b < 3; ++b) slb_bulk::mbar_wait(bar + b, 0);
}

SLB_DEV void head_group_finish(const filter_args& a, bool mine, int outcome, int64_t rel, unsigned* s_stat) {
    const int lane = threadIdx.x & 31;
    const bool undecided = mine && outcome < 0;
    if (mine && outcome >= 0) a.negative[rel] = outcome > 0 ? 1 : 0;
    if (a.fold.rec != nullptr) fold_decided(a.fold, mine && outcome >= 0, outcome > 0, rel, a.idx_begin);
    const long long slot = list_append(undecided, a.counts + 1);
    if (undecided) a.list_b[slot] = rel;
    const unsigned dec = __ballot_sync(0xffffffffu, mine && !undecided);
    const unsigned und = __ballot_sync(0xffffffffu, undecided);
    if (lane == 0) {
        if (dec) atomicAdd(s_stat + 0, (unsigned)__popc(dec));
        if (und) atomicAdd(s_stat + 1, (unsigned)__popc(und));
    }
}

template <int DIN, int CD>
__global__ void __launch_bounds__(HT, 1)
filter_head_kernel(const __grid_constant__ slb_sweep cfg, const filter_args a) {
    constexpr int ND = CD > 0 ? CD : SLB_MAX_OUT;
    using entry_t = std::conditional_t<(CD > 0), cf_entry<DIN, ND>, filter_side>;
    extern __shared__ __align__(16) unsigned char smem_raw[];
    if (threadIdx.x == 0) head_mark(a, HM_ENTRY);
    prefetch_descriptor_operands(cfg);
    const filter_plan& lay = a.plan;
    double* smem = reinterpret_cast<double*>(smem_raw);
    uint64_t* bar = reinterpret_cast<uint64_t*>(smem);
    unsigned* s_stat = reinterpret_cast<unsigned*>(smem + 3);
    double* tab512 = smem + lay.tabs;
    double* exptab = tab512 + 512;
    double* kbuf = smem + lay.kbuf;
    double* wbuf = smem + lay.wbuf;
    double* xbuf = smem + lay.xbuf;
    double* mbuf = smem + lay.mbuf;
    const int nf = cfg.gp.num_factors;
    const bool means = CD > 0 && (lay.mean_scheme != SLB_MEAN_GRID_FACTORED || a.counts[2] != 0);
    if (threadIdx.x == 0) {
        for (int b = 0; b < 3; ++b) slb_bulk::mbar_init(bar + b, 1);
        slb_bulk::fence_barrier_init();
        slb_bulk::fence_proxy_async();
        unsigned xbytes = 576 * sizeof(double), wbytes = 0;
        for (int f = 0; f < lay.factors_staged; ++f)
            if (cfg.gp.factors[f].head_rows > 0) {
                xbytes += (unsigned)(HR * DIN) * sizeof(double);
                wbytes += (unsigned)(HR * HR) * sizeof(double);
            }
        slb_bulk::mbar_arrive_expect_tx(bar + 0, xbytes);
        slb_bulk::copy_g2s(tab512, g_exp_tables, 576 * sizeof(double), bar + 0);
        for (int f = 0; f < lay.factors_staged; ++f)
            if (cfg.gp.factors[f].head_rows > 0)
                slb_bulk::copy_g2s(xbuf + (size_t)f * HR * DIN, cfg.gp.factors[f].Xhead,
                                   HR * DIN * sizeof(double), bar + 0);
        slb_bulk::mbar_arrive_expect_tx(bar + 1, wbytes);
        for (int f = 0; f < lay.factors_staged; ++f)
            if (cfg.gp.factors[f].head_rows > 0)
                slb_bulk::copy_g2s(wbuf + (size_t)f * HR * HR, cfg.gp.factors[f].Wheadp,
                                   HR * HR * sizeof(double), bar + 1);
        slb_bulk::mbar_arrive_expect_tx(bar + 2, means ? (unsigned)lay.mean_doubles * sizeof(double) : 0u);
        if (means) {
            for (int f = 0; f < nf; ++f) {
                const slb_gp_factor& F = cfg.gp.factors[f];
                const int Mp = padded_rows(F.M);
                if (Mp == 0) continue;
                double* dst = mbuf + lay.mean_off[f];
                slb_bulk::copy_g2s(dst, F.Xf, (unsigned)(Mp * (DIN + 1)) * sizeof(double), bar + 2);
                dst += (size_t)Mp * (DIN + 1);
                for (int o = 0; o < cfg.gp.num_outputs; ++o) {
                    if (cfg.gp.outputs[o].factor != f) continue;
                    slb_bulk::copy_g2s(dst, cfg.gp.outputs[o].gamma_f, (unsigned)Mp * sizeof(double), bar + 2);
                    dst += Mp;
                }
            }
        }
    }
    if (a.prefetch_factors) {
        for (int f = 0; f < nf; ++f) {
            const slb_gp_factor& F = cfg.gp.factors[f];
            const char* base = reinterpret_cast<const char*>(F.Wpack);
            const size_t nbytes = (size_t)F.nrb * (F.nrb + 1) * 32 * sizeof(double);
            for (size_t off = ((size_t)blockIdx.x * HT + threadIdx.x) * 128; off < nbytes;
                 off += (size_t)gridDim.x * HT * 128)
                asm volatile("prefetch.global.L2 [%0];" ::"l"(base + off));
            const char* xs = reinterpret_cast<const char*>(F.Xs);
            const size_t xbytes = (size_t)F.M * DIN * sizeof(double);
            if (blockIdx.x == (unsigned)f)
                for (size_t off = (size_t)threadIdx.x * 128; off < xbytes; off += (size_t)HT * 128)
                    asm volatile("prefetch.global.L2 [%0];" ::"l"(xs + off));
        }
        if (blockIdx.x == gridDim.x - 1 && threadIdx.x < cfg.gp.num_outputs) {
            const slb_gp_output& G = cfg.gp.outputs[threadIdx.x];
            const size_t abytes = (size_t)cfg.gp.factors[G.factor].M * sizeof(double);
            for (size_t off = 0; off < abytes; off += 128)
                asm volatile("prefetch.global.L2 [%0];" ::"l"(reinterpret_cast<const char*>(G.alpha) + off));
        }
    }
    if (threadIdx.x < 2) s_stat[threadIdx.x] = 0;
    if constexpr (CD > 0)
        if (threadIdx.x < 2) reinterpret_cast<int*>(smem + lay.need)[threadIdx.x] = 0;
    __syncthreads();
    const int64_t count = (int64_t)a.counts[0];
    const int64_t nwarps = (int64_t)gridDim.x * HW;
    const int64_t ngroups = (count + HP - 1) / HP;
    if ((int64_t)blockIdx.x >= ngroups) {
        head_wait_landings(bar);
        if (threadIdx.x == 0) head_mark(a, HM_EXIT);
        return;
    }
    const int warp = threadIdx.x >> 5;
    double* kw = kbuf + warp * HR * HP;
    double* sd_s = smem + lay.sd;
    double* mu_s = smem + lay.mu;
    double* merr_s = smem + lay.merr;
    int* need_s = reinterpret_cast<int*>(smem + lay.need);
    const int ng_first = (int)min((int64_t)HW, (ngroups - blockIdx.x + gridDim.x - 1) / gridDim.x);
    const bool split = a.head_schedule == 1 ||
                       (a.head_schedule == 0 && ngroups <= nwarps && ng_first * nf < HW);
    if (split) {
        const int lane = threadIdx.x & 31;
        for (int64_t grp0 = blockIdx.x; grp0 < ngroups; grp0 += nwarps) {
            const int ngr = (int)min((int64_t)HW, (ngroups - grp0 + gridDim.x - 1) / gridDim.x);
            const int npairs = ngr * nf;
            const int nbw = min(npairs, HW);
            const bool early_means = means && nbw < HW;
            if (warp < nbw) {
                slb_bulk::mbar_wait(bar + 0, 0);
                head_mark(a, HM_TABLES);
                for (int p = warp; p < npairs; p += nbw) {
                    const int i = p / nf, f = p % nf;
                    if (cfg.gp.factors[f].head_rows <= 0) continue;
                    const int64_t k = (grp0 + (int64_t)i * gridDim.x) * HP + min(lane, HP - 1);
                    const bool mine = lane < HP && k < count;
                    double tz[DIN];
#pragma unroll
                    for (int c = 0; c < DIN; ++c) tz[c] = mine ? a.side_a[k].z[c] : 0.0;
                    const double sd =
                        lay.factors_staged == nf
                            ? head_factor_sdev<DIN, true, (CD > 0)>(cfg, a, f, tz, mine, exptab, kw, wbuf, xbuf, bar)
                            : head_factor_sdev<DIN, false, (CD > 0)>(cfg, a, f, tz, mine, exptab, kw, wbuf, xbuf, bar);
                    if (lane < HP) sd_s[(i * HP + lane) * SLB_MAX_OUT + f] = sd;
                    if (f == 0) head_mark(a, HM_BOUND0);
                }
                head_mark(a, HM_BOUND);
            } else if constexpr (CD > 0) {
                if (early_means) {
                    slb_bulk::mbar_wait(bar + 0, 0);
                    slb_bulk::mbar_wait(bar + 2, 0);
                    head_round_means<DIN, CD>(cfg, a, nullptr, ngr * HP, grp0, count, mbuf, tab512, mu_s, merr_s,
                                              nbw * 32, HT - nbw * 32);
                    head_mark(a, HM_MEANS);
                }
            }
            __syncthreads();
            if constexpr (CD > 0) {
                if (means && !early_means) {
                    slb_bulk::mbar_wait(bar + 0, 0);
                    slb_bulk::mbar_wait(bar + 2, 0);
                    head_round_means<DIN, CD>(cfg, a, nullptr, ngr * HP, grp0, count, mbuf, tab512, mu_s, merr_s, 0,
                                              HT);
                    head_mark(a, HM_MEANS);
                    __syncthreads();
                }
            }
            if (warp < ngr) {
                entry_t t;
                int64_t rel;
                bool mine;
                double shi[ND];
                head_group_entries<DIN>(cfg, a, grp0 + (int64_t)warp * gridDim.x, count, t, rel, mine, shi);
                const int slot = warp * HP + min(lane, HP - 1);
#pragma unroll
                for (int j = 0; j < ND; ++j) {
                    if (j >= cfg.gp.num_outputs) break;
                    const int f = cfg.gp.outputs[j].factor;
                    if (cfg.gp.factors[f].head_rows > 0) shi[j] = sd_s[slot * SLB_MAX_OUT + f];
                }
                double vx = 0.0;
                bool need;
                int outcome = head_entry_decision(cfg, a, t, shi, mine, vx, need);
                if constexpr (CD > 0)
                    if (need) outcome = head_mean_decision(cfg, t, vx, shi, mu_s, merr_s, slot);
                head_mark(a, HM_DECIDED);
                head_group_finish(a, mine, outcome, entry_rel(t, rel), s_stat);
            }
            __syncthreads();
        }
    } else {
        int round = 0;
        for (int64_t grp0 = blockIdx.x; grp0 < ngroups; grp0 += nwarps, ++round) {
            const int64_t grp = grp0 + (int64_t)warp * gridDim.x;
            const bool active = grp < ngroups;
            const int lane = threadIdx.x & 31;
            entry_t t;
            int64_t rel = 0;
            bool mine = false, need = false;
            double shi[ND];
            double vx = 0.0;
            int outcome = 0;
            if (active) {
                head_group_entries<DIN>(cfg, a, grp, count, t, rel, mine, shi);
                if (lay.factors_staged == nf)
                    head_group_bound<DIN, true, CD>(cfg, a, t.z, mine, exptab, kw, wbuf, xbuf, bar, shi);
                else
                    head_group_bound<DIN, false, CD>(cfg, a, t.z, mine, exptab, kw, wbuf, xbuf, bar, shi);
                outcome = head_entry_decision(cfg, a, t, shi, mine, vx, need);
                if (need) need_s[2 + atomicAdd(need_s + (round & 1), 1)] = warp * HP + lane;
            }
            if constexpr (CD > 0) {
                if (threadIdx.x == 0) need_s[(round + 1) & 1] = 0;
                __syncthreads();
                const int nneed = need_s[round & 1];
                if (nneed > 0) {
                    slb_bulk::mbar_wait(bar + 2, 0);
                    head_round_means<DIN, CD>(cfg, a, need_s + 2, nneed, grp0, count, mbuf, tab512, mu_s, merr_s, 0, HT);
                    head_mark(a, HM_MEANS);
                    __syncthreads();
                    if (need) outcome = head_mean_decision(cfg, t, vx, shi, mu_s, merr_s, warp * HP + lane);
                }
            }
            if (active) {
                head_mark(a, HM_DECIDED);
                head_group_finish(a, mine, outcome, entry_rel(t, rel), s_stat);
            }
        }
    }
    head_wait_landings(bar);
    __syncthreads();
    if (a.stats != nullptr && threadIdx.x < 2 && s_stat[threadIdx.x] != 0)
        atomicAdd(a.stats + 1 + threadIdx.x, (unsigned long long)s_stat[threadIdx.x]);
    if (threadIdx.x == 0) head_mark(a, HM_EXIT);
}

double* g_probe_mu = nullptr;
double* g_probe_dm = nullptr;
unsigned long long* g_head_timing = nullptr;
unsigned long long* g_stage1_timing = nullptr;
int g_filter_stages = 3;

bool screening_applicable(const slb_sweep& cfg) {
    if (g_filter_stages & 4) return false;
    const int D = cfg.gp.num_outputs;
    for (int f = 0; f < cfg.gp.num_factors; ++f)
        if (cfg.gp.factors[f].kernel.num_prims > 0) return false;
    const slb_function& V = cfg.lyapunov;
    if (D > 4) return false;
    if (V.kind != SLB_FN_QUADRATIC || V.in_dim != D || (V.flags & ~(uint32_t)SLB_FLAG_SCALE)) return false;
    const slb_function& L = cfg.lipschitz_v;
    if (L.kind == SLB_FN_NONE) return true;
    if (L.kind != SLB_FN_LINEAR || L.in_dim != D) return false;
    if (L.flags & ~(uint32_t)(SLB_FLAG_ABS | SLB_FLAG_NORM1 | SLB_FLAG_SCALE)) return false;
    if (L.out_dim > 4) return false;
    return (L.flags & SLB_FLAG_NORM1) || L.out_dim == 1 || L.out_dim == D;
}

bool grid_mean_applicable(const slb_sweep& cfg) {
    if (g_filter_stages & 32) return false;
    const slb_function& P = cfg.policy;
    const slb_function& Lf = cfg.lipschitz_f;
    const bool lf_closed = Lf.kind == SLB_FN_NONE || cfg.lf_values != nullptr ||
                           (Lf.kind == SLB_FN_LINEAR && Lf.in_dim == 2 && Lf.out_dim <= SLB_MAX_LIN_OUT &&
                            Lf.matrix != nullptr &&
                            !(Lf.flags & ~(uint32_t)(SLB_FLAG_SATURATE | SLB_FLAG_ABS | SLB_FLAG_NORM1 |
                                                     SLB_FLAG_SCALE)));
    return screening_applicable(cfg) && cfg.grid.ndim == 2 && cfg.gp.input_dim == 3 &&
           P.kind == SLB_FN_LINEAR && P.in_dim == 2 && P.out_dim == 1 && P.matrix != nullptr &&
           !(P.flags & ~(uint32_t)(SLB_FLAG_SATURATE | SLB_FLAG_SCALE)) && lf_closed;
}

filter_plan stage1_plan(const slb_sweep& cfg) {
    const int din = cfg.gp.input_dim, nf = cfg.gp.num_factors;
    const int budget = 226 * 1024 / (int)sizeof(double);
    const int slots = HW * HP * SLB_MAX_OUT;
    filter_plan p = {};
    p.mean_scheme = SLB_MEAN_FP64;
    p.factors_staged = nf;
    while (p.factors_staged > 0 && 4 + 576 + HW * HR * HP + slots + p.factors_staged * (HR * HR + HR * din) > budget)
        --p.factors_staged;
    int off = 4;
    p.tabs = off;   off += 576;
    p.kbuf = off;   off += HW * HR * HP;
    p.sd = off;     off += slots;
    p.wbuf = off;   off += p.factors_staged * HR * HR;
    p.xbuf = off;   off += p.factors_staged * HR * din;
    p.doubles = off;
    if (!screening_applicable(cfg) || p.factors_staged != nf) return p;
    int tables = 0;
    for (int f = 0; f < nf; ++f) {
        int no = 0;
        for (int o = 0; o < cfg.gp.num_outputs; ++o) no += cfg.gp.outputs[o].factor == f;
        p.mean_off[f] = tables;
        tables += ((cfg.gp.factors[f].M + 7) & ~7) * (din + 1 + no);
    }
    const int need = (HW * HP + 4) * (int)sizeof(int) / (int)sizeof(double);
    if (off + tables + 2 * slots + need > budget) return p;
    p.mean_scheme = grid_mean_applicable(cfg) ? SLB_MEAN_GRID_FACTORED : SLB_MEAN_FP32_SCREENED;
    p.mean_doubles = tables;
    p.mbuf = off;   off += tables;
    p.mu = off;     off += slots;
    p.merr = off;   off += slots;
    p.need = off;   off += need;
    p.doubles = off;
    return p;
}

template <int DIN, int D>
int launch_filter(cudaStream_t st, const slb_sweep& cfg, const filter_args& a) {
    static std::atomic<bool> configured[64];
    int device = 0;
    SLB_CUDA(cudaGetDevice(&device));
    if (device < 0 || device >= 64 || !configured[device].load(std::memory_order_acquire)) {
        if constexpr (D == 0)
            SLB_CUDA(cudaFuncSetAttribute(filter_mean_kernel<DIN>,
                                          cudaFuncAttributeMaxDynamicSharedMemorySize, 96 * 1024));
        else
            SLB_CUDA(cudaFuncSetAttribute(filter_mean32_kernel<DIN, D>,
                                          cudaFuncAttributeMaxDynamicSharedMemorySize, 96 * 1024));
        SLB_CUDA(cudaFuncSetAttribute(filter_head_kernel<DIN, D>,
                                      cudaFuncAttributeMaxDynamicSharedMemorySize, 227 * 1024));
        if constexpr (DIN == 3 && D == GRID_OUTPUTS) {
            SLB_CUDA(cudaFuncSetAttribute(filter_grid_mean_kernel<GRID_OUTPUTS>,
                                          cudaFuncAttributeMaxDynamicSharedMemorySize,
                                          (int)grid_mean_smem_bytes()));
            SLB_CUDA(cudaFuncSetAttribute(filter_grid_mean_kernel<GRID_OUTPUTS>,
                                          cudaFuncAttributePreferredSharedMemoryCarveout,
                                          (int)cudaSharedmemCarveoutMaxShared));
        }
        if (device >= 0 && device < 64) configured[device].store(true, std::memory_order_release);
    }
    const int64_t blocks = (a.n + FT - 1) / FT;
    switch (a.plan.mean_scheme) {
    case SLB_MEAN_GRID_FACTORED:
        SLB_CHECK(DIN == 3 && D == GRID_OUTPUTS, "filtered sweep: the factored grid mean needs d_in = 3 and %d outputs",
                  GRID_OUTPUTS);
        if constexpr (DIN == 3 && D == GRID_OUTPUTS) {
            const int64_t n1 = cfg.grid.num_points[1];
            const int64_t r0 = a.idx_begin / n1, r1 = (a.idx_begin + a.n - 1) / n1;
            const int64_t tiles = ((r1 - r0) / GR + 1) * ((n1 + GC - 1) / GC);
            filter_grid_mean_kernel<GRID_OUTPUTS><<<(unsigned)tiles, GT, grid_mean_smem_bytes(), st>>>(cfg, a);
        }
        break;
    case SLB_MEAN_FP32_SCREENED:
        if constexpr (D > 0)
            filter_mean32_kernel<DIN, D><<<(unsigned)blocks, FT,
                                           mean32_smem_bytes(DIN, a.max_outputs_per_factor, a.chunk_rows, FT / 32),
                                           st>>>(cfg, a);
        break;
    default:
        if constexpr (D == 0)
            filter_mean_kernel<DIN><<<(unsigned)blocks, FT,
                                      mean_smem_bytes(DIN, a.max_outputs_per_factor, a.chunk_rows), st>>>(cfg, a);
    }
    SLB_LAUNCH_CHECK();
    if (!(g_filter_stages & 1)) return 0;
    filter_head_kernel<DIN, D><<<HEAD_CTAS, HT, (size_t)a.plan.doubles * sizeof(double), st>>>(cfg, a);
    SLB_LAUNCH_CHECK();
    return 0;
}

static_assert(SLB_MAX_ACT == 2, "the screened instantiations cover m = 1, 2");
int dispatch_filter(cudaStream_t st, const slb_sweep& cfg, const filter_args& a) {
    return slb_dispatch_dim<2, 6>(cfg.gp.input_dim, "GP input_dim", [&](auto din) {
        constexpr int DIN = decltype(din)::value;
        if (a.plan.mean_scheme == SLB_MEAN_FP64) return launch_filter<DIN, 0>(st, cfg, a);
        constexpr int DLO = DIN - 2 > 1 ? DIN - 2 : 1, DHI = DIN - 1 < 4 ? DIN - 1 : 4;
        return slb_dispatch_dim<DLO, DHI>(cfg.gp.num_outputs, "screened filter: outputs", [&](auto d) {
            return launch_filter<DIN, decltype(d)::value>(st, cfg, a);
        });
    });
}

}

int slb_launch_apply_prefix_folded(cudaStream_t st, const double* values, const uint8_t* initial, int64_t n,
                                   int64_t idx_begin, slb_fold* rec, slb_fail_key* key, uint8_t* safe,
                                   slb_prefix_stats* stats);

int slb_launch_refine(cudaStream_t st, const slb_sweep& cfg, int64_t n_max, int64_t idx_begin,
                      const int64_t* list, const unsigned long long* count, uint8_t* negative,
                      double* values, double* mean, double* err, double* split_partial, int* split_ticket,
                      const slb_fold_target& fold);

extern "C" {

int slb_debug_filter_stages(int32_t mask) {
    g_filter_stages = mask;
    return 0;
}

int slb_filter_stage1(const slb_sweep* cfg) {
    const int scheme = slb_filter_mean_scheme(cfg);
    return scheme == SLB_MEAN_NONE ? 0 : scheme == SLB_MEAN_FP64 ? 64 : 32;
}

int slb_filter_mean_scheme(const slb_sweep* cfg) {
    if (cfg == nullptr || cfg->gp.num_outputs <= 0) return SLB_MEAN_NONE;
    return stage1_plan(*cfg).mean_scheme;
}

int slb_debug_screening_probe(double* mu_dev, double* dm_dev) {
    g_probe_mu = (mu_dev != nullptr && dm_dev != nullptr) ? mu_dev : nullptr;
    g_probe_dm = g_probe_mu != nullptr ? dm_dev : nullptr;
    return 0;
}

int slb_debug_head_timing(void* buffer_dev) {
    g_head_timing = static_cast<unsigned long long*>(buffer_dev);
    return 0;
}

int slb_debug_stage1_timing(void* buffer_dev) {
    g_stage1_timing = static_cast<unsigned long long*>(buffer_dev);
    return 0;
}

int64_t slb_filter_workspace(int64_t n) {
    if (n < 0) n = 0;
    if (n > CHUNK) n = CHUNK;
    return WS_HEAD + n * (int64_t)(2 * sizeof(int64_t) + sizeof(filter_side));
}

int slb_debug_filter_lists(int64_t n, int64_t* offsets) {
    SLB_CHECK(offsets != nullptr, "slb_debug_filter_lists: null offsets");
    SLB_CHECK(n >= 0 && n <= CHUNK, "slb_debug_filter_lists: n %lld outside [0, %lld] (one pass)", (long long)n,
              (long long)CHUNK);
    offsets[0] = 0;
    offsets[1] = WS_HEAD;
    offsets[2] = WS_HEAD + n * (int64_t)sizeof(int64_t);
    return 0;
}

}

static int filtered_sweep(cudaStream_t st, const slb_sweep* cfg, int64_t idx_begin, int64_t idx_end,
                          uint8_t* negative_dev, double* values_dev, void* workspace_dev, int64_t* stats_dev,
                          slb_fold_target fold) {
    int m;
    if (slb_validate_sweep(cfg, false, &m)) return 1;
    if (slb_validate_range("slb_lyapunov_sweep_filtered", idx_begin, idx_end, cfg->grid.nindex)) return 1;
    SLB_CHECK(cfg->gp.num_outputs > 0, "slb_lyapunov_sweep_filtered needs GP dynamics "
              "(deterministic dynamics have nothing to filter: use slb_lyapunov_sweep)");
    if (slb_validate_staged_tables(&cfg->gp, "filtered sweep")) return 1;
    int nomax = 1;
    for (int f = 0; f < cfg->gp.num_factors; ++f) {
        const slb_gp_factor& F = cfg->gp.factors[f];
        SLB_CHECK(F.M == 0 || (F.Whead != nullptr && F.Wheadp != nullptr && F.Xhead != nullptr),
                  "filtered sweep: GP factor %d lacks the filter tables (Whead / Wheadp / Xhead)", f);
        SLB_CHECK(F.M == 0 || ((reinterpret_cast<uintptr_t>(F.Wheadp) & 15) == 0 &&
                               (reinterpret_cast<uintptr_t>(F.Xhead) & 15) == 0),
                  "filtered sweep: GP factor %d: Wheadp / Xhead must be 16-byte aligned", f);
        SLB_CHECK(F.head_rows >= 0 && F.head_rows <= SLB_HEAD_RANK && F.head_rows <= F.M,
                  "filtered sweep: GP factor %d has %d head rows (0..min(M, %d))", f, F.head_rows,
                  SLB_HEAD_RANK);
        int no = 0;
        for (int o = 0; o < cfg->gp.num_outputs; ++o) no += cfg->gp.outputs[o].factor == f;
        if (no > nomax) nomax = no;
    }
    for (int o = 0; o < cfg->gp.num_outputs; ++o)
        SLB_CHECK(cfg->gp.outputs[o].gamma_l1 >= 0.0, "filtered sweep: GP output %d has no gamma_l1", o);
    const int64_t n_all = idx_end - idx_begin;
    if (n_all == 0) return 0;
    SLB_CHECK(negative_dev != nullptr && workspace_dev != nullptr,
              "slb_lyapunov_sweep_filtered: negative_dev and workspace_dev are required");
    char* ws = static_cast<char*>(workspace_dev);
    const int64_t cap = n_all < CHUNK ? n_all : CHUNK;
    filter_args a;
    memset(&a, 0, sizeof(a));
    a.counts = reinterpret_cast<unsigned long long*>(ws);
    int* tickets = reinterpret_cast<int*>(ws + 64);
    double* partial = reinterpret_cast<double*>(ws + WS_PARTIAL);
    a.list_a = reinterpret_cast<int64_t*>(ws + WS_HEAD);
    a.list_b = a.list_a + cap;
    a.side_a = reinterpret_cast<filter_side*>(a.list_b + cap);
    a.stats = reinterpret_cast<unsigned long long*>(stats_dev);
    const int din = cfg->gp.input_dim;
    a.chunk_rows = mean_chunk_rows(din, nomax, 24);
    a.max_outputs_per_factor = nomax;
    a.plan = stage1_plan(*cfg);
    a.prefetch_factors = (g_filter_stages & 2) ? 1 : 0;
    a.head_schedule = (g_filter_stages >> 3) & 3;
    a.probe_mu = g_probe_mu;
    a.probe_dm = g_probe_dm;
    a.timing = g_head_timing;
    a.timing1 = g_stage1_timing;
    for (int64_t off = 0; off < n_all; off += CHUNK) {
        const int64_t n = n_all - off < CHUNK ? n_all - off : CHUNK;
        const bool first_fold = fold.rec != nullptr && off == 0;
        SLB_CUDA(cudaMemsetAsync(a.counts, 0, first_fold ? WS_PARTIAL : WS_FOLD, st));
        a.n = n; a.idx_begin = idx_begin + off;
        a.negative = negative_dev + off;
        a.values = values_dev ? values_dev + off : nullptr;
        a.fold = fold;
        if (fold.rec != nullptr) {
            a.fold.values = fold.values + off;
            a.fold.initial = fold.initial ? fold.initial + off : nullptr;
        }
        int rc = dispatch_filter(st, *cfg, a);
        if (rc) return rc;
        if (!(g_filter_stages & 2)) continue;
        rc = slb_launch_refine(st, *cfg, n, idx_begin + off, a.list_b, a.counts + 1,
                               negative_dev + off, values_dev ? values_dev + off : nullptr,
                               nullptr, nullptr, partial, tickets, a.fold);
        if (rc) return rc;
    }
    return 0;
}

extern "C" {

int slb_lyapunov_sweep_filtered(void* stream, const slb_sweep* cfg, int64_t idx_begin,
                                int64_t idx_end, uint8_t* negative_dev, double* values_dev,
                                void* workspace_dev, int64_t* stats_dev) {
    return filtered_sweep((cudaStream_t)stream, cfg, idx_begin, idx_end, negative_dev, values_dev, workspace_dev,
                          stats_dev, slb_fold_target{});
}

int slb_safe_set_step(void* stream, const slb_sweep* cfg, int64_t idx_begin, int64_t idx_end,
                      uint8_t* negative_dev, const double* values_dev, const uint8_t* initial_dev,
                      void* workspace_dev, int64_t* stats_dev, slb_fail_key* key_dev, uint8_t* safe_dev,
                      slb_prefix_stats* prefix_stats_dev) {
    SLB_CHECK(cfg != nullptr, "slb_safe_set_step: null config");
    SLB_CHECK(idx_end > idx_begin, "slb_safe_set_step: empty range [%lld, %lld)", (long long)idx_begin,
              (long long)idx_end);
    SLB_CHECK(values_dev != nullptr && workspace_dev != nullptr && key_dev != nullptr && safe_dev != nullptr &&
                  prefix_stats_dev != nullptr,
              "slb_safe_set_step: null values, workspace, key, safe set or statistics");
    cudaStream_t st = (cudaStream_t)stream;
    slb_fold* rec = reinterpret_cast<slb_fold*>(static_cast<char*>(workspace_dev) + WS_FOLD);
    const int rc = filtered_sweep(st, cfg, idx_begin, idx_end, negative_dev, nullptr, workspace_dev, stats_dev,
                                  slb_fold_target{values_dev, initial_dev, rec});
    if (rc) return rc;
    return slb_launch_apply_prefix_folded(st, values_dev, initial_dev, idx_end - idx_begin, idx_begin, rec,
                                          key_dev, safe_dev, prefix_stats_dev);
}

int slb_debug_refine(void* stream, const slb_sweep* cfg, int64_t idx_begin, int64_t n_max,
                     const int64_t* list_dev, const unsigned long long* count_dev,
                     uint8_t* negative_dev, double* values_dev, double* mean_dev, double* err_dev,
                     void* workspace_dev) {
    SLB_CHECK(cfg != nullptr, "slb_debug_refine: null config");
    SLB_CHECK(cfg->gp.num_outputs > 0, "slb_debug_refine needs GP dynamics (the refine pass is the GP posterior)");
    SLB_CHECK(n_max >= 0 && n_max <= CHUNK, "slb_debug_refine: n_max %lld outside [0, %lld]", (long long)n_max,
              (long long)CHUNK);
    SLB_CHECK(list_dev != nullptr && count_dev != nullptr && negative_dev != nullptr && workspace_dev != nullptr,
              "slb_debug_refine: null list, count, negative or workspace");
    int m;
    if (slb_validate_sweep(cfg, false, &m)) return 1;
    if (slb_validate_range("slb_debug_refine", idx_begin, idx_begin + n_max, cfg->grid.nindex)) return 1;
    cudaStream_t st = (cudaStream_t)stream;
    char* ws = static_cast<char*>(workspace_dev);
    SLB_CUDA(cudaMemsetAsync(ws + 64, 0, SLB_SPLIT_TICKET_BYTES, st));
    return slb_launch_refine(st, *cfg, n_max, idx_begin, list_dev, count_dev, negative_dev, values_dev, mean_dev,
                             err_dev, reinterpret_cast<double*>(ws + WS_PARTIAL), reinterpret_cast<int*>(ws + 64),
                             slb_fold_target{});
}

}
```

### safe_learning_b200/csrc/gp_args.h

```cpp
#pragma once
#include <stdint.h>

enum { MODE_SWEEP_GRID = 0, MODE_SWEEP_STATES = 1, MODE_PREDICT = 2 };
enum { SLB_SPLIT_ITEMS = 512, SLB_SPLIT_MAX = 8, SLB_SPLIT_TICKET_BYTES = 2048 };
#define SLB_SPLIT_PARTIAL_BYTES ((size_t)SLB_SPLIT_ITEMS * SLB_MAX_OUT * (1 + SLB_MAX_OUT) * 64 * sizeof(double))

struct slb_gp_args {
    const double* points;
    int64_t n;
    int64_t idx_begin;
    int32_t mode;
    int32_t want_var;
    uint8_t* negative;
    double* values;
    double* decrease;
    double* threshold;
    double* mean;
    double* err;
    const int64_t* index_list;
    const unsigned long long* count;
    int64_t count_min, count_max;
    double* split_partial;
    int* split_ticket;
    slb_fold_target fold;
    long long* timing;
};

template <int DIN, int TPV>
int slb_gp_tile_launch(cudaStream_t st, const slb_sweep& cfg, const slb_gp_args& a, bool kexpr, bool timing);
```

### safe_learning_b200/csrc/gp_sweep.cu

```cuda
#include "common.cuh"

#include <string.h>

#include "gp_args.h"

namespace {

__global__ void pack_factor_kernel(const double* __restrict__ Linv, int M, int nrb,
                                   double* __restrict__ W, int64_t total) {
    const int64_t e = (int64_t)blockIdx.x * blockDim.x + threadIdx.x;
    if (e >= total) return;
    const int64_t pair = e >> 6;
    const int lane = (int)((e >> 1) & 31);
    const int half = (int)(e & 1);
    int64_t b = (int64_t)((sqrt(8.0 * (double)pair + 1.0) - 1.0) * 0.5);
    while (b * (b + 1) / 2 > pair) --b;
    while ((b + 1) * (b + 2) / 2 <= pair) ++b;
    const int64_t kp = pair - b * (b + 1) / 2;
    const int64_t row = 8 * b + (lane >> 2);
    const int64_t col = 8 * kp + 4 * half + (lane & 3);
    W[e] = (row < M && col <= row) ? Linv[row * M + col] : 0.0;
}


cudaEvent_t g_factor_event[64] = {};
bool g_factor_pending[64] = {};

int wait_for_factors(cudaStream_t st) {
    int device = 0;
    SLB_CUDA(cudaGetDevice(&device));
    if (device < 0 || device >= 64 || !g_factor_pending[device]) return 0;
    cudaStreamCaptureStatus cs = cudaStreamCaptureStatusNone;
    SLB_CUDA(cudaStreamIsCapturing(st, &cs));
    SLB_CUDA(cudaStreamWaitEvent(st, g_factor_event[device],
                                 cs == cudaStreamCaptureStatusActive ? cudaEventWaitExternal : 0));
    return 0;
}

int dispatch_gp_tile(cudaStream_t st, const slb_sweep& cfg, const slb_gp_args& a, int tp = 64) {
    if (a.n <= 0) return 0;
    if (wait_for_factors(st)) return 1;
    SLB_CHECK(a.n <= (int64_t)0x7fffffff * tp, "too many points for one launch");
    const bool timing = a.timing != nullptr;
    bool kexpr = false;
    for (int f = 0; f < cfg.gp.num_factors; ++f) kexpr |= cfg.gp.factors[f].kernel.num_prims > 0;
    return slb_dispatch_dim<1, 6>(cfg.gp.input_dim, "GP input_dim", [&](auto D) {
        return tp == 64 ? slb_gp_tile_launch<D, 64>(st, cfg, a, kexpr, timing)
                        : slb_gp_tile_launch<D, 32>(st, cfg, a, kexpr, timing);
    });
}

}

int slb_wait_for_factors(cudaStream_t st) { return wait_for_factors(st); }

int slb_launch_det_sweep(cudaStream_t st, const slb_sweep& cfg, const double* states, int64_t n,
                         int64_t idx_begin, uint8_t* negative, double* values, double* decrease,
                         double* threshold, double* mean);

static long long* g_timing_buffer = nullptr;

static int64_t g_refine_split = 32 * SLB_NUM_SMS;

int slb_launch_refine(cudaStream_t st, const slb_sweep& cfg, int64_t n_max, int64_t idx_begin,
                      const int64_t* list, const unsigned long long* count, uint8_t* negative,
                      double* values, double* mean, double* err, double* split_partial, int* split_ticket,
                      const slb_fold_target& fold) {
    slb_gp_args a;
    memset(&a, 0, sizeof(a));
    a.idx_begin = idx_begin; a.mode = MODE_SWEEP_GRID;
    a.negative = negative; a.values = values;
    a.mean = mean; a.err = err;
    a.index_list = list; a.count = count;
    a.fold = fold;
    a.timing = g_timing_buffer;
    const int tps[2] = {32, 64};
    const int64_t lo[2] = {0, g_refine_split};
    const int64_t hi[2] = {g_refine_split, INT64_MAX};
    for (int v = 0; v < 2; ++v) {
        if (lo[v] >= hi[v] || lo[v] >= n_max) continue;
        a.count_min = lo[v]; a.count_max = hi[v];
        a.n = n_max < hi[v] ? n_max : hi[v];
        a.split_partial = nullptr; a.split_ticket = nullptr;
        if (v == 0 && split_partial != nullptr) {
            if (a.n < (int64_t)SLB_NUM_SMS * tps[v]) a.n = (int64_t)SLB_NUM_SMS * tps[v];
            if ((a.n + tps[v] - 1) / tps[v] <= SLB_SPLIT_ITEMS) {
                a.split_partial = split_partial; a.split_ticket = split_ticket;
            }
        }
        const int rc = dispatch_gp_tile(st, cfg, a, tps[v]);
        if (rc) return rc;
    }
    return 0;
}

extern "C" {

int slb_debug_refine_split(int64_t upto32) {
    g_refine_split = upto32 < 0 ? 0 : upto32;
    return 0;
}

int slb_restore_tables(void* dst_dev, const void* src_host, int64_t split_bytes, int64_t total_bytes,
                       void* stream, void* side_stream) {
    SLB_CHECK(dst_dev != nullptr && src_host != nullptr, "slb_restore_tables: null buffer");
    SLB_CHECK(split_bytes >= 0 && split_bytes <= total_bytes, "slb_restore_tables: split %lld outside [0, %lld]",
              (long long)split_bytes, (long long)total_bytes);
    cudaStream_t st = static_cast<cudaStream_t>(stream), side = static_cast<cudaStream_t>(side_stream);
    char* dst = static_cast<char*>(dst_dev);
    const char* src = static_cast<const char*>(src_host);
    if (split_bytes > 0) SLB_CUDA(cudaMemcpyAsync(dst, src, (size_t)split_bytes, cudaMemcpyHostToDevice, st));
    const int64_t rest = total_bytes - split_bytes;
    if (rest <= 0) return 0;
    if (side == nullptr || side == st) {
        SLB_CUDA(cudaMemcpyAsync(dst + split_bytes, src + split_bytes, (size_t)rest, cudaMemcpyHostToDevice, st));
        return 0;
    }
    int device = 0;
    SLB_CUDA(cudaGetDevice(&device));
    SLB_CHECK(device >= 0 && device < 64, "slb_restore_tables: device %d unsupported", device);
    static cudaEvent_t order[64] = {};
    if (order[device] == nullptr) SLB_CUDA(cudaEventCreateWithFlags(&order[device], cudaEventDisableTiming));
    SLB_CUDA(cudaEventRecord(order[device], st));
    SLB_CUDA(cudaStreamWaitEvent(side, order[device], 0));
    SLB_CUDA(cudaMemcpyAsync(dst + split_bytes, src + split_bytes, (size_t)rest, cudaMemcpyHostToDevice, side));
    return slb_record_factor_dependency(side);
}

int slb_record_factor_dependency(void* stream) {
    int device = 0;
    SLB_CUDA(cudaGetDevice(&device));
    SLB_CHECK(device >= 0 && device < 64, "slb_record_factor_dependency: device %d unsupported", device);
    if (g_factor_event[device] == nullptr)
        SLB_CUDA(cudaEventCreateWithFlags(&g_factor_event[device], cudaEventDisableTiming));
    SLB_CUDA(cudaEventRecord(g_factor_event[device], static_cast<cudaStream_t>(stream)));
    g_factor_pending[device] = true;
    return 0;
}

int slb_debug_phase_timing(void* buffer_dev) {
    g_timing_buffer = static_cast<long long*>(buffer_dev);
    return 0;
}

int64_t slb_packed_len(int32_t M) {
    if (M <= 0) return 0;
    const int64_t nrb = (M + 7) / 8;
    return nrb * (nrb + 1) * 32;
}

int slb_pack_factor(void* stream, const double* Linv_dev, int32_t M, double* Wpack_dev) {
    SLB_CHECK(Linv_dev != nullptr && Wpack_dev != nullptr, "slb_pack_factor: null pointer");
    SLB_CHECK(M > 0, "slb_pack_factor: M must be positive (got %d)", M);
    const int nrb = (M + 7) / 8;
    const int64_t total = slb_packed_len(M);
    const int threads = 256;
    const int64_t blocks = (total + threads - 1) / threads;
    pack_factor_kernel<<<(unsigned)blocks, threads, 0, (cudaStream_t)stream>>>(Linv_dev, M, nrb,
                                                                              Wpack_dev, total);
    SLB_LAUNCH_CHECK();
    return 0;
}

int slb_gp_predict(void* stream, const slb_gp_stack* gp, const double* points_dev, int64_t n,
                   double* mean_dev, double* err_dev, int32_t want_var) {
    SLB_CHECK(gp != nullptr, "slb_gp_predict: null gp");
    if (slb_validate_gp(gp)) return 1;
    SLB_CHECK(gp->num_outputs > 0, "slb_gp_predict: GP stack has no outputs");
    SLB_CHECK(n >= 0, "slb_gp_predict: negative n");
    SLB_CHECK(n == 0 || (points_dev && mean_dev && err_dev), "slb_gp_predict: null buffer");
    slb_sweep cfg;
    memset(&cfg, 0, sizeof(cfg));
    cfg.gp = *gp;
    slb_gp_args a;
    memset(&a, 0, sizeof(a));
    a.points = points_dev; a.n = n; a.mode = MODE_PREDICT; a.want_var = want_var;
    a.mean = mean_dev; a.err = err_dev;
    return dispatch_gp_tile((cudaStream_t)stream, cfg, a);
}

static int sweep_common(void* stream, const slb_sweep* cfg, const double* states, int64_t n,
                        int64_t idx_begin, uint8_t* negative, double* values, double* decrease,
                        double* threshold, double* mean, double* err) {
    int m;
    if (slb_validate_sweep(cfg, states != nullptr, &m)) return 1;
    SLB_CHECK(n >= 0, "lyapunov sweep: negative point count");
    if (n == 0) return 0;
    SLB_CHECK(negative != nullptr, "lyapunov sweep: negative_dev is required");
    if (cfg->gp.num_outputs > 0) {
        slb_gp_args a;
        memset(&a, 0, sizeof(a));
        a.points = states; a.n = n; a.idx_begin = idx_begin;
        a.mode = states ? MODE_SWEEP_STATES : MODE_SWEEP_GRID;
        a.negative = negative; a.values = values; a.decrease = decrease; a.threshold = threshold;
        a.mean = mean; a.err = err;
        a.timing = g_timing_buffer;
        return dispatch_gp_tile((cudaStream_t)stream, *cfg, a);
    }
    SLB_CHECK(err == nullptr, "deterministic dynamics have no error bounds (err_dev must be NULL)");
    return slb_launch_det_sweep((cudaStream_t)stream, *cfg, states, n, idx_begin, negative, values,
                                decrease, threshold, mean);
}

int slb_lyapunov_sweep(void* stream, const slb_sweep* cfg, int64_t idx_begin, int64_t idx_end,
                       uint8_t* negative_dev, double* values_dev, double* decrease_dev,
                       double* threshold_dev, double* mean_dev, double* err_dev) {
    SLB_CHECK(cfg != nullptr, "slb_lyapunov_sweep: null config");
    if (slb_validate_range("slb_lyapunov_sweep", idx_begin, idx_end, cfg->grid.nindex)) return 1;
    return sweep_common(stream, cfg, nullptr, idx_end - idx_begin, idx_begin, negative_dev,
                        values_dev, decrease_dev, threshold_dev, mean_dev, err_dev);
}

int slb_lyapunov_points(void* stream, const slb_sweep* cfg, const double* states_dev, int64_t n,
                        uint8_t* negative_dev, double* values_dev, double* decrease_dev,
                        double* threshold_dev, double* mean_dev, double* err_dev) {
    SLB_CHECK(n == 0 || states_dev != nullptr, "slb_lyapunov_points: null states");
    return sweep_common(stream, cfg, states_dev, n, 0, negative_dev, values_dev, decrease_dev,
                        threshold_dev, mean_dev, err_dev);
}

}
```

### safe_learning_b200/csrc/gp_tile.cuh

```cuda
#pragma once
#define SLB_EVAL_NOINLINE 1
#include "common.cuh"

#include <string.h>

#include <atomic>


#include "gp_args.h"

namespace {

#ifndef SLB_TP
#define SLB_TP SLB_TILE_POINTS
#endif
constexpr int TP = SLB_TP;
static_assert(TP == 32 || TP == 64, "TP must be 32 or 64");
constexpr int PANEL = 256;
constexpr int KSTR = TP + 2;
constexpr int NW = 8;
constexpr int NT = NW * 32;
constexpr int RQ = 32 / NW;
constexpr int NB = TP / 8;
constexpr int CTAS_PER_SM = 1;
constexpr int NRED = 1 + SLB_MAX_OUT;
constexpr int PREFETCH_CTAS = SLB_NUM_SMS * CTAS_PER_SM;

constexpr size_t SMEM_KS = (size_t)(PANEL / 8) * 4 * KSTR * 2 * sizeof(double);
constexpr size_t SMEM_Z = (size_t)SLB_MAX_IN * TP * sizeof(double);
constexpr size_t SMEM_RED = (size_t)NW * TP * NRED * sizeof(double);
constexpr size_t SMEM_TOT = (size_t)NRED * TP * sizeof(double);
constexpr size_t SMEM_POST = (size_t)2 * SLB_MAX_OUT * TP * sizeof(double);
constexpr size_t SMEM_EXPTAB = 64 * sizeof(double);
constexpr size_t SMEM_XP = (size_t)PANEL * SLB_MAX_IN * sizeof(double);
constexpr size_t SMEM_KEXPR = (sizeof(slb_kernel) + 15) / 16 * 16;
constexpr size_t SMEM_PRE = (size_t)4 * TP * sizeof(double);
constexpr size_t SMEM_TOTAL = SMEM_KS + SMEM_Z + SMEM_RED + SMEM_TOT + SMEM_POST + SMEM_EXPTAB +
                              SMEM_XP + SMEM_KEXPR + SMEM_PRE;

SLB_DEV double2 ldg_stream2(const double2* p) {
    double2 v;
    asm volatile("ld.global.nc.L1::no_allocate.v2.f64 {%0, %1}, [%2];"
                 : "=d"(v.x), "=d"(v.y) : "l"(p));
    return v;
}

SLB_DEV void dmma884(double& c0, double& c1, double a, double b) {
    asm volatile("mma.sync.aligned.m8n8k4.row.col.f64.f64.f64.f64 {%0,%1}, {%2}, {%3}, {%0,%1};"
                 : "+d"(c0), "+d"(c1) : "d"(a), "d"(b));
}

constexpr int RING = TP == 64 ? 3 : 5;
constexpr int BG = 4;

template <int Q0>
SLB_DEV void mma_run(double (&acc)[RQ][NB][2], const double2* const (&ap)[RQ], int m0, int m1,
                     const double2* ks_lane) {
    double2 ar[RING][RQ];
    const int m1m = m1 - 1;
#pragma unroll
    for (int d = 0; d < RING; ++d) {
        const int md = min(m0 + d, m1m);
#pragma unroll
        for (int q = Q0; q < RQ; ++q) ar[d][q] = ldg_stream2(ap[q] + md * 32);
    }
    int m = m0;
#pragma unroll 1
    while (true) {
#pragma unroll
        for (int d = 0; d < RING; ++d) {
            if (m >= m1) return;
            const double2* kb = ks_lane + m * (4 * KSTR);
#pragma unroll
            for (int half = 0; half < NB; half += BG) {
                double2 b[BG];
#pragma unroll
                for (int nb = 0; nb < BG; ++nb) b[nb] = kb[(half + nb) * 8];
#pragma unroll
                for (int q = Q0; q < RQ; ++q)
#pragma unroll
                    for (int nb = 0; nb < BG; ++nb)
                        dmma884(acc[q][half + nb][0], acc[q][half + nb][1], ar[d][q].x, b[nb].x);
#pragma unroll
                for (int q = Q0; q < RQ; ++q)
#pragma unroll
                    for (int nb = 0; nb < BG; ++nb)
                        dmma884(acc[q][half + nb][0], acc[q][half + nb][1], ar[d][q].y, b[nb].y);
            }
            const int mp = min(m + RING, m1m);
#pragma unroll
            for (int q = Q0; q < RQ; ++q) ar[d][q] = ldg_stream2(ap[q] + mp * 32);
            ++m;
        }
    }
}

template <int NBT>
SLB_DEV void row_lane_reduce(const double (&v)[2 * NBT], int lane, double* red_q) {
    constexpr int NV = 2 * NBT;
    const bool g2 = (lane & 16) != 0, g1 = (lane & 8) != 0, g0 = (lane & 4) != 0;
    double w8[NV / 2], w4[NV / 4];
#pragma unroll
    for (int i = 0; i < NV / 2; ++i) {
        const double send = g2 ? v[i] : v[i + NV / 2];
        const double keep = g2 ? v[i + NV / 2] : v[i];
        w8[i] = keep + __shfl_xor_sync(0xffffffffu, send, 16);
    }
#pragma unroll
    for (int i = 0; i < NV / 4; ++i) {
        const double send = g1 ? w8[i] : w8[i + NV / 4];
        const double keep = g1 ? w8[i + NV / 4] : w8[i];
        w4[i] = keep + __shfl_xor_sync(0xffffffffu, send, 8);
    }
    if constexpr (NBT == 8) {
        double w2[2];
#pragma unroll
        for (int i = 0; i < 2; ++i) {
            const double send = g0 ? w4[i] : w4[i + 2];
            const double keep = g0 ? w4[i + 2] : w4[i];
            w2[i] = keep + __shfl_xor_sync(0xffffffffu, send, 4);
        }
        double* slot = red_q + (8 * (lane >> 2) + 2 * (lane & 3)) * NRED;
        slot[0] += w2[0];
        slot[NRED] += w2[1];
    } else {
        static_assert(NBT == 4, "written for 8 or 4 column blocks");
        const double send = g0 ? w4[0] : w4[1];
        const double keep = g0 ? w4[1] : w4[0];
        const double w1 = keep + __shfl_xor_sync(0xffffffffu, send, 4);
        const int g = lane >> 2;
        red_q[(8 * (g >> 1) + 2 * (lane & 3) + (g & 1)) * NRED] += w1;
    }
}

template <int DIN, bool TIMING, bool KEXPR>
SLB_DEV void gp_tile_body(const slb_sweep& cfg, const slb_gp_args& a, unsigned char* smem_raw,
                          const int64_t tile_index, const int64_t npts, const int grp, const int G,
                          const int fsel, const int FS, const bool first_tile) {
    double* Ks = reinterpret_cast<double*>(smem_raw);
    double* zraw = Ks + (PANEL / 8) * 4 * KSTR * 2;
    double* red = zraw + SLB_MAX_IN * TP;
    double* tot = red + NW * TP * NRED;
    double* post = tot + NRED * TP;
    double* exptab = post + 2 * SLB_MAX_OUT * TP;
    double* Xp = exptab + 64;
    slb_kernel* kexpr = reinterpret_cast<slb_kernel*>(Xp + PANEL * SLB_MAX_IN);
    double* pre = reinterpret_cast<double*>(reinterpret_cast<unsigned char*>(kexpr) + SMEM_KEXPR);

    const int tid = threadIdx.x, lane = tid & 31, warp = tid >> 5;
    prefetch_descriptor_operands(cfg);
    const double exp_entry = c_exp2_tab[tid & 63];
    const int64_t tile0 = tile_index * TP;
    const int D = cfg.gp.num_outputs;
    long long t_gen = 0, t_mma = 0, t_epi = 0, t_mark = 0, t_sync = 0, t_s0 = 0;
    const long long t_start = TIMING ? clock64() : 0;
    long long g_start = 0;
    if (TIMING) asm volatile("mov.u64 %0, %globaltimer;" : "=l"(g_start));

    if (first_tile && blockIdx.x < PREFETCH_CTAS) {
        for (int f = 0; f < cfg.gp.num_factors; ++f) {
            const slb_gp_factor& F = cfg.gp.factors[f];
            const char* base = reinterpret_cast<const char*>(F.Wpack);
            const size_t nbytes = (size_t)F.nrb * (F.nrb + 1) * 32 * sizeof(double);
            for (size_t off = ((size_t)blockIdx.x * NT + tid) * 128; off < nbytes;
                 off += (size_t)PREFETCH_CTAS * NT * 128)
                asm volatile("prefetch.global.L2 [%0];" ::"l"(base + off));
        }
    }

    if (tid < 64) exptab[tid] = exp_entry;

    if (tid < TP) {
        int64_t rel = tile0 + tid;
        if (rel > npts - 1) rel = npts - 1;
        if (a.index_list != nullptr) rel = a.index_list[rel];
        double z[SLB_MAX_IN];
        if (a.mode == MODE_PREDICT) {
#pragma unroll
            for (int c = 0; c < DIN; ++c) z[c] = a.points[rel * DIN + c];
        } else {
            const int d = cfg.grid.ndim;
            double x[SLB_MAX_DIM];
            if (a.mode == MODE_SWEEP_GRID) {
                grid_index_to_state(cfg.grid, a.idx_begin + rel, x);
            } else {
                for (int c = 0; c < d; ++c) x[c] = a.points[rel * d + c];
            }
            double u[SLB_MAX_OUT];
            const int m = eval_fn_small(cfg.policy, x, u);
            for (int c = 0; c < d; ++c) z[c] = x[c];
            for (int c = 0; c < m; ++c) z[d + c] = u[c];
        }
#pragma unroll
        for (int c = 0; c < DIN; ++c) zraw[c * TP + tid] = z[c];
    } else if (tid < 2 * TP && a.mode != MODE_PREDICT) {
        const int p = tid - TP;
        int64_t rel = tile0 + p;
        if (rel > npts - 1) rel = npts - 1;
        if (a.index_list != nullptr) rel = a.index_list[rel];
        const int d = cfg.grid.ndim;
        double x[SLB_MAX_DIM];
        if (a.mode == MODE_SWEEP_GRID) {
            grid_index_to_state(cfg.grid, a.idx_begin + rel, x);
        } else {
            for (int c = 0; c < d; ++c) x[c] = a.points[rel * d + c];
        }
        lyapunov_state_terms(cfg, x, a.mode == MODE_SWEEP_GRID ? a.idx_begin + rel : -1, &pre[p],
                             &pre[TP + p]);
    }
    __syncthreads();

    const int wg_ = warp & 3, wr_ = warp >> 2;
    const int wslot = wr_ == 0 ? wg_ : 7 - wg_;
    const int p_gen = tid & (TP - 1);
    const int jg = tid / TP;
    const double2* ks_lane = reinterpret_cast<const double2*>(Ks) + (lane & 3) * KSTR + (lane >> 2);

    auto factor_epilogue = [&](int f, bool general, double s2) {
        const slb_gp_factor& F = cfg.gp.factors[f];
        if (tid < TP) {
            int qty = 1;
            for (int o = 0; o < D; ++o) {
                const slb_gp_output& Go = cfg.gp.outputs[o];
                if (Go.factor != f) continue;
                double mx = 0.0;
                if (Go.prior_mean != nullptr) {
                    mx = f64mul(zraw[tid], Go.prior_mean[0]);
                    for (int c = 1; c < DIN; ++c)
                        mx = f64add(mx, f64mul(zraw[c * TP + tid], Go.prior_mean[c]));
                    mx = f64mul(F.scale, mx);
                }
                const double fmean = f64add(tot[qty * TP + tid], mx) / F.scale;
                double kss = F.kss;
                if (general) {
                    double zt[DIN];
#pragma unroll
                    for (int c = 0; c < DIN; ++c) zt[c] = zraw[c * TP + tid];
                    kss = s2 * kernel_expr_diag<DIN>(*kexpr, zt);
                }
                const double fvar = f64sub(kss, tot[tid]) / s2;
                post[o * TP + tid] = fmean;
                post[(SLB_MAX_OUT + o) * TP + tid] =
                    a.want_var ? fvar : f64mul(Go.beta, sqrt(fvar));
                ++qty;
            }
        }
    };

    const bool split = G * FS > 1;
    for (int f = 0; f < cfg.gp.num_factors; ++f) {
        if (fsel >= 0 && f != fsel) continue;
        const slb_gp_factor& F = cfg.gp.factors[f];
        const int M = F.M, nrb = F.nrb;
        const int nk4 = (M + 3) >> 2;
        const double s2 = f64mul(F.scale, F.scale);
        const double variance = F.variance;
        const double* __restrict__ Xs = F.Xs;

        const bool general = KEXPR && F.kernel.num_prims > 0;
        if (general) {
            __syncthreads();
            const int* src = reinterpret_cast<const int*>(&F.kernel);
            for (int i = tid; i < (int)(sizeof(slb_kernel) / sizeof(int)); i += NT)
                reinterpret_cast<int*>(kexpr)[i] = src[i];
            __syncthreads();
        }
        double zs[DIN];
#pragma unroll
        for (int c = 0; c < DIN; ++c)
            zs[c] = general ? zraw[c * TP + p_gen] : zraw[c * TP + p_gen] / F.lengthscales[c];
        for (int i = lane; i < TP * NRED; i += 32) red[warp * TP * NRED + i] = 0.0;
        __syncwarp();
        int resident = -1;

        int rlo = 0, rhi = nrb;
        if (G > 1) {
            rlo = __double2int_rd((double)nrb * sqrt((double)grp / (double)G));
            rhi = grp + 1 == G ? nrb : __double2int_rd((double)nrb * sqrt((double)(grp + 1) / (double)G));
        }
        for (int pbeg = rlo; pbeg < rhi; pbeg += 32) {
            double acc[RQ][NB][2];
#pragma unroll
            for (int q = 0; q < RQ; ++q)
#pragma unroll
                for (int nb = 0; nb < NB; ++nb) { acc[q][nb][0] = 0.0; acc[q][nb][1] = 0.0; }

            const int pend = min(pbeg + 32, rhi);
            int bq[RQ];
#pragma unroll
            for (int q = 0; q < RQ; ++q) bq[q] = pend - 1 - wslot - NW * (RQ - 1 - q);

            const int jp_last = (pend - 1) >> 5;
            for (int jp = 0; jp <= jp_last; ++jp) {
                const int nkp = min(64, nk4 - 64 * jp);
                if (jp != resident) {
                    if (TIMING) t_s0 = clock64();
                    __syncthreads();
                    if (TIMING) { t_mark = clock64(); t_sync += t_mark - t_s0; }
                    const int j0 = PANEL * jp;
                    const int nj = min(PANEL, M - j0);
                    for (int i = tid; i < nj * DIN; i += NT) Xp[i] = Xs[(size_t)j0 * DIN + i];
                    __syncthreads();
                    constexpr int PS = NT / TP / 4;
                    static_assert(NT / TP == 4 * PS, "generation needs a multiple of 4 groups");
                    const int gr = jg & 3, gpo = jg >> 2;
                    const int npairs = (nkp + 1) >> 1;
                    double2* ks2 = reinterpret_cast<double2*>(Ks);
                    constexpr int GP = 2;
                    if (general) {
                        for (int mm = gpo; mm < npairs; mm += GP * PS) {
                            const double* xr[2 * GP];
#pragma unroll
                            for (int u = 0; u < 2 * GP; ++u) {
                                const int jj = 8 * (mm + PS * (u >> 1)) + 4 * (u & 1) + gr;
                                xr[u] = Xp + min(jj, nj - 1) * DIN;
                            }
                            double kv[2 * GP];
                            kernel_expr_cross_n<DIN, 2 * GP>(*kexpr, zs, xr, exptab, kv);
#pragma unroll
                            for (int u = 0; u < 2 * GP; ++u) {
                                const int jj = 8 * (mm + PS * (u >> 1)) + 4 * (u & 1) + gr;
                                kv[u] = jj < nj ? s2 * kv[u] : 0.0;
                            }
#pragma unroll
                            for (int g = 0; g < GP; ++g)
                                if (mm + PS * g < npairs)
                                    ks2[((mm + PS * g) * 4 + gr) * KSTR + p_gen] =
                                        make_double2(kv[2 * g], kv[2 * g + 1]);
                        }
                    } else
                    for (int mm = gpo; mm < npairs; mm += GP * PS) {
                        double t2[2 * GP];
#pragma unroll
                        for (int u = 0; u < 2 * GP; ++u) {
                            const int jj = min(8 * (mm + PS * (u >> 1)) + 4 * (u & 1) + gr, nj - 1);
                            const double* xr = Xp + jj * DIN;
                            double acc2 = 0.0;
#pragma unroll
                            for (int c = 0; c < DIN; ++c) {
                                const double df = zs[c] - xr[c];
                                acc2 = fma(df, df, acc2);
                            }
                            t2[u] = acc2;
                        }
                        double kv[2 * GP];
#pragma unroll
                        for (int u = 0; u < 2 * GP; ++u) {
                            const int jj = 8 * (mm + PS * (u >> 1)) + 4 * (u & 1) + gr;
                            const double k = s2 * (variance * exp_neg_tab(-0.5 * t2[u], exptab));
                            kv[u] = jj < nj ? k : 0.0;
                        }
#pragma unroll
                        for (int g = 0; g < GP; ++g)
                            if (mm + PS * g < npairs)
                                ks2[((mm + PS * g) * 4 + gr) * KSTR + p_gen] =
                                    make_double2(kv[2 * g], kv[2 * g + 1]);
                    }
                    resident = jp;
                    if (TIMING) { t_s0 = clock64(); t_gen += t_s0 - t_mark; }
                    __syncthreads();
                    if (TIMING) t_sync += clock64() - t_s0;
                }
                if (TIMING) t_mark = clock64();
                const int npairs_mma = (nkp + 1) >> 1;
                int mend[RQ];
                const double2* ap[RQ];
#pragma unroll
                for (int q = 0; q < RQ; ++q) {
                    const bool valid = bq[q] >= pbeg;
                    const int me = valid ? min(npairs_mma, max(0, bq[q] - 32 * jp + 1)) : 0;
                    mend[q] = me;
                    const int64_t b = valid ? bq[q] : 0;
                    ap[q] = reinterpret_cast<const double2*>(F.Wpack) +
                            (b * (b + 1) / 2 + 32 * jp) * 32 + lane;
                }
                int mprev = 0;
                if (mend[0] > mprev) { mma_run<0>(acc, ap, mprev, mend[0], ks_lane); mprev = mend[0]; }
                if (mend[1] > mprev) { mma_run<1>(acc, ap, mprev, mend[1], ks_lane); mprev = mend[1]; }
                if (mend[2] > mprev) { mma_run<2>(acc, ap, mprev, mend[2], ks_lane); mprev = mend[2]; }
                if (mend[3] > mprev) { mma_run<3>(acc, ap, mprev, mend[3], ks_lane); mprev = mend[3]; }
                if (TIMING) t_mma += clock64() - t_mark;
            }
            if (TIMING) t_mark = clock64();

            int qty = 0;
            for (int o = -1; o < D; ++o) {
                double al[RQ] = {};
                if (o >= 0) {
                    if (cfg.gp.outputs[o].factor != f) continue;
                    const double* alpha = cfg.gp.outputs[o].alpha;
#pragma unroll
                    for (int q = 0; q < RQ; ++q)
                        if (bq[q] >= pbeg) al[q] = __ldg(alpha + 8 * bq[q] + (lane >> 2));
                }
                constexpr int NV = 2 * NB;
                double v[NV];
#pragma unroll
                for (int nb = 0; nb < NB; ++nb) {
#pragma unroll
                    for (int e = 0; e < 2; ++e) {
                        double t = 0.0;
#pragma unroll
                        for (int q = 0; q < RQ; ++q) {
                            const double x = acc[q][nb][e];
                            t = fma(x, (o < 0) ? x : al[q], t);
                        }
                        v[nb * 2 + e] = t;
                    }
                }
                row_lane_reduce<NB>(v, lane, red + (size_t)warp * TP * NRED + qty);
                ++qty;
            }
            __syncwarp();
            if (TIMING) t_epi += clock64() - t_mark;
        }

        if (TIMING) t_s0 = clock64();
        __syncthreads();
        if (TIMING) t_sync += clock64() - t_s0;
        if (tid < TP) {
            for (int r = 0; r < NRED; ++r) {
                double s = 0.0;
#pragma unroll
                for (int w = 0; w < NW; ++w) s += red[(w * TP + tid) * NRED + r];
                tot[r * TP + tid] = s;
            }
        }
        __syncthreads();

        if (split) {
            double* part = a.split_partial + ((size_t)blockIdx.x * SLB_MAX_OUT + f) * (NRED * TP);
            for (int i = tid; i < NRED * TP; i += NT) part[i] = tot[i];
            __syncthreads();
            continue;
        }
        factor_epilogue(f, general, s2);
        __syncthreads();
    }

    if (split) {
        __shared__ int s_ticket;
        __threadfence();
        __syncthreads();
        if (tid == 0) s_ticket = atomicAdd(a.split_ticket + tile_index, 1);
        __syncthreads();
        if (s_ticket != G * FS - 1) {
            if (TIMING && lane == 0) {
                long long* t = a.timing + ((size_t)blockIdx.x * NW + warp) * 8;
                long long g_end;
                asm volatile("mov.u64 %0, %globaltimer;" : "=l"(g_end));
                t[0] = t_gen; t[1] = t_mma; t[2] = t_epi; t[3] = clock64() - t_start;
                t[4] = g_start; t[5] = g_end; t[6] = t_sync; t[7] = 1;
            }
            return;
        }
        __threadfence();
        if (tid == 0) a.split_ticket[tile_index] = 0;
        for (int f = 0; f < cfg.gp.num_factors; ++f) {
            const slb_gp_factor& F = cfg.gp.factors[f];
            for (int i = tid; i < NRED * TP; i += NT) {
                double sum = 0.0;
                const size_t cta0 = (size_t)tile_index * (G * FS) + (FS > 1 ? (size_t)f * G : 0);
                for (int g2 = 0; g2 < G; ++g2)
                    sum += __ldcg(a.split_partial + ((cta0 + g2) * SLB_MAX_OUT + f) * (NRED * TP) + i);
                tot[i] = sum;
            }
            const bool general = KEXPR && F.kernel.num_prims > 0;
            if (general) {
                const int* src = reinterpret_cast<const int*>(&F.kernel);
                for (int i = tid; i < (int)(sizeof(slb_kernel) / sizeof(int)); i += NT)
                    reinterpret_cast<int*>(kexpr)[i] = src[i];
            }
            __syncthreads();
            factor_epilogue(f, general, f64mul(F.scale, F.scale));
            __syncthreads();
        }
    }

    if (TIMING && lane == 0) {
        long long* t = a.timing + ((size_t)blockIdx.x * NW + warp) * 8;
        long long g_end;
        asm volatile("mov.u64 %0, %globaltimer;" : "=l"(g_end));
        t[0] = t_gen; t[1] = t_mma; t[2] = t_epi; t[3] = clock64() - t_start;
        t[4] = g_start; t[5] = g_end; t[6] = t_sync; t[7] = 0;
    }
    {
        const int p = tid & (TP - 1);
        const bool live = tile0 + p < npts;
        int64_t rel = live ? tile0 + p : 0;
        if (a.index_list != nullptr) rel = a.index_list[rel];
        if (tid < 2 * TP && live) {
            double mu[SLB_MAX_OUT], er[SLB_MAX_OUT];
            for (int o = 0; o < D; ++o) {
                mu[o] = post[o * TP + p];
                er[o] = post[(SLB_MAX_OUT + o) * TP + p];
            }
            if (tid < TP) {
                if (a.mean != nullptr) for (int o = 0; o < D; ++o) a.mean[rel * D + o] = mu[o];
                if (a.err != nullptr) for (int o = 0; o < D; ++o) a.err[rel * D + o] = er[o];
                if (a.mode != MODE_PREDICT) {
                    double vm[1];
                    eval_fn_small(cfg.lyapunov, mu, vm);
                    pre[2 * TP + p] = vm[0];
                }
            } else if (a.mode != MODE_PREDICT) {
                pre[3 * TP + p] = lyapunov_error_bound(cfg, mu, er);
            }
        }
        if (a.mode == MODE_PREDICT) return;
        __syncthreads();
        bool neg = false;
        if (tid < TP && live) {
            const slb_decision r =
                lyapunov_combine(pre[p], pre[TP + p], pre[2 * TP + p], pre[3 * TP + p]);
            neg = r.negative;
            a.negative[rel] = r.negative ? 1 : 0;
            if (a.values != nullptr) a.values[rel] = r.vx;
            if (a.decrease != nullptr) a.decrease[rel] = r.decrease;
            if (a.threshold != nullptr) a.threshold[rel] = r.threshold;
        }
        if (a.fold.rec != nullptr && tid < TP) fold_decided(a.fold, live, neg, rel, a.idx_begin);
    }
}

template <int DIN, bool TIMING, bool KEXPR, int TPV>
__global__ void __launch_bounds__(NT, CTAS_PER_SM)
gp_tile_kernel(const __grid_constant__ slb_sweep cfg, const slb_gp_args a) {
    extern __shared__ __align__(16) unsigned char smem_raw[];
    int64_t tile_index = blockIdx.x;
    int64_t tile_end = tile_index + 1, tile_step = 1;
    int grp = 0, G = 1;
    int fsel = -1, FS = 1;
    int64_t npts = a.n;
    if (a.count != nullptr) {
        prefetch_descriptor_operands(cfg);
        npts = (int64_t)*a.count;
        if (npts <= a.count_min || npts > a.count_max) return;
        const int64_t ntiles = (npts + TP - 1) / TP;
        if (a.split_partial != nullptr) {
            int64_t spare = (int64_t)gridDim.x / ntiles;
            const int nfac = cfg.gp.num_factors;
            if (nfac > 1 && spare >= 2 * nfac) {
                FS = nfac;
                spare /= nfac;
            }
            G = (int)(spare < 1 ? 1 : (spare > SLB_SPLIT_MAX ? SLB_SPLIT_MAX : spare));
            const int per_tile = G * FS;
            if ((int64_t)blockIdx.x >= ntiles * per_tile) return;
            tile_index = blockIdx.x / per_tile;
            tile_end = tile_index + 1;
            const int rem = (int)(blockIdx.x % per_tile);
            grp = rem % G;
            if (FS > 1) fsel = rem / G;
        } else {
            tile_end = ntiles;
            tile_step = gridDim.x;
        }
        if (tile_index * TP >= npts) return;
    }
    for (int64_t tile = tile_index; tile < tile_end; tile += tile_step) {
        gp_tile_body<DIN, TIMING, KEXPR>(cfg, a, smem_raw, tile, npts, grp, G, fsel, FS, tile == tile_index);
        if (tile + tile_step < tile_end) __syncthreads();
    }
}

template <int DIN, bool TIMING, bool KEXPR, int TPV = TP>
int launch_gp_tile(cudaStream_t st, const slb_sweep& cfg, const slb_gp_args& a) {
    static_assert(TPV == TP, "TPV only disambiguates the symbol");
    static std::atomic<bool> configured[64];
    int device = 0;
    SLB_CUDA(cudaGetDevice(&device));
    if (device < 0 || device >= 64 || !configured[device].load(std::memory_order_acquire)) {
        SLB_CUDA(cudaFuncSetAttribute(gp_tile_kernel<DIN, TIMING, KEXPR, TP>,
                                      cudaFuncAttributeMaxDynamicSharedMemorySize,
                                      (int)SMEM_TOTAL));
        if (device >= 0 && device < 64) configured[device].store(true, std::memory_order_release);
    }
    int64_t tiles = (a.n + TP - 1) / TP;
    if (a.count != nullptr && a.split_partial == nullptr && tiles > PREFETCH_CTAS) tiles = PREFETCH_CTAS;
    gp_tile_kernel<DIN, TIMING, KEXPR, TP><<<(unsigned)tiles, NT, SMEM_TOTAL, st>>>(cfg, a);
    SLB_LAUNCH_CHECK();
    return 0;
}

}
```

### safe_learning_b200/csrc/gp_tile_inst.cu

```cuda
#include "gp_tile.cuh"

#ifndef SLB_TILE_DIN
#error "compile with -DSLB_TILE_DIN=<1..6>"
#endif

template <int DIN, int TPV>
int slb_gp_tile_launch(cudaStream_t st, const slb_sweep& cfg, const slb_gp_args& a, bool kexpr,
                       bool timing) {
#if SLB_TILE_DIN == 3 && SLB_TP == 64
    if (timing) return launch_gp_tile<3, true, false>(st, cfg, a);
#else
    if (timing) {
        slb_set_error("phase timing is compiled for d_in = 3, 64-point tiles only");
        return 1;
    }
#endif
    return kexpr ? launch_gp_tile<DIN, false, true>(st, cfg, a)
                 : launch_gp_tile<DIN, false, false>(st, cfg, a);
}

template int slb_gp_tile_launch<SLB_TILE_DIN, SLB_TP>(cudaStream_t, const slb_sweep&, const slb_gp_args&,
                                                      bool, bool);
```

Measured before the change: 573.7 million.

## Reuse filter side records in refine tiles and add closed-form Lyapunov kernel

```diff
diff --git a/include/slb200.h b/include/slb200.h
--- a/include/slb200.h
+++ b/include/slb200.h
@@ -188,6 +188,7 @@
 int         slb_debug_phase_timing(void* buffer_dev);
 int         slb_debug_head_timing(void* buffer_dev);
 int         slb_debug_stage1_timing(void* buffer_dev);
+int         slb_debug_refine_timing(void* buffer_dev);
 int         slb_record_factor_dependency(void* stream);
 int         slb_restore_tables(void* dst_dev, const void* src_host, int64_t split_bytes, int64_t total_bytes,
                                void* stream, void* side_stream);
diff --git a/safe_learning_b200/_native.py b/safe_learning_b200/_native.py
--- a/safe_learning_b200/_native.py
+++ b/safe_learning_b200/_native.py
@@ -126,6 +126,7 @@
     "slb_debug_phase_timing": (C.c_int, [_vp]),
     "slb_debug_head_timing": (C.c_int, [_vp]),
     "slb_debug_stage1_timing": (C.c_int, [_vp]),
+    "slb_debug_refine_timing": (C.c_int, [_vp]),
     "slb_record_factor_dependency": (C.c_int, [_vp]),
     "slb_restore_tables": (C.c_int, [_vp, _vp, _i64, _i64, _vp, _vp]),
     "slb_debug_refine_split": (C.c_int, [_i64]),
diff --git a/safe_learning_b200/csrc/common.cuh b/safe_learning_b200/csrc/common.cuh
--- a/safe_learning_b200/csrc/common.cuh
+++ b/safe_learning_b200/csrc/common.cuh
@@ -881,24 +881,27 @@
     *threshold_out = f64mul(f64mul(-lvx, f64add(1.0, lf)), cfg.tau);
 }
 
+SLB_DEV double lyapunov_error_sum(const double* lv, int nl, const double* err, int d) {
+    double bound = f64mul(lv[0], err[0]);
+    for (int j = 1; j < d; ++j) bound = f64add(bound, f64mul(nl == 1 ? lv[0] : lv[j], err[j]));
+    return bound;
+}
+
 SLB_DEV double lyapunov_error_bound(const slb_sweep& cfg, const double* mu, const double* err) {
-    const int d = cfg.grid.ndim;
-    double tmp[SLB_MAX_OUT];
-    double bound;
-    if (cfg.lipschitz_v.kind != SLB_FN_NONE) {
-        const int nl = eval_fn_small(cfg.lipschitz_v, mu, tmp);
-        if (nl == 1) {
-            bound = f64mul(tmp[0], err[0]);
-            for (int j = 1; j < d; ++j) bound = f64add(bound, f64mul(tmp[0], err[j]));
-        } else {
-            bound = f64mul(tmp[0], err[0]);
-            for (int j = 1; j < d; ++j) bound = f64add(bound, f64mul(tmp[j], err[j]));
-        }
-    } else {
-        bound = f64mul(cfg.lv_const, err[0]);
-        for (int j = 1; j < d; ++j) bound = f64add(bound, f64mul(cfg.lv_const, err[j]));
-    }
-    return bound;
+    double lv[SLB_MAX_OUT];
+    int nl = 1;
+    lv[0] = cfg.lv_const;
+    if (cfg.lipschitz_v.kind != SLB_FN_NONE) nl = eval_fn_small(cfg.lipschitz_v, mu, lv);
+    return lyapunov_error_sum(lv, nl, err, cfg.grid.ndim);
+}
+
+template <int D>
+SLB_DEV double lyapunov_error_bound_closed(const slb_sweep& cfg, const double (&mu)[D], const double (&err)[D]) {
+    int nl = 1;
+    slb_vec<SLB_MAX_LIN_OUT> lv;
+    lv.v[0] = cfg.lv_const;
+    if (cfg.lipschitz_v.kind != SLB_FN_NONE) lv = eval_linear_reg<D, SLB_MAX_LIN_OUT>(cfg.lipschitz_v, mu, nl);
+    return lyapunov_error_sum(lv.v, nl, err, D);
 }
 
 SLB_DEV slb_decision lyapunov_combine(double vx, double threshold, double vm, double bound) {
diff --git a/safe_learning_b200/csrc/filter.cu b/safe_learning_b200/csrc/filter.cu
--- a/safe_learning_b200/csrc/filter.cu
+++ b/safe_learning_b200/csrc/filter.cu
@@ -24,7 +24,6 @@
 static_assert(sizeof(slb_fold) <= WS_PARTIAL - WS_FOLD && WS_FOLD % 16 == 0, "fold record slot");
 
 
-struct filter_side { double dec0, thr, guard, coef[SLB_MAX_OUT], z[SLB_MAX_IN], dm[SLB_MAX_OUT]; };
 
 struct filter_plan {
     int mean_scheme;
@@ -48,6 +47,7 @@
     int64_t* list_a;
     filter_side* side_a;
     int64_t* list_b;
+    int64_t* slot_b;
     unsigned long long* counts;
     unsigned long long* stats;
     int chunk_rows;
@@ -317,7 +317,7 @@
     const long long slot = stage1_finish(a, valid, rel, sane ? screened : -1, vx);
     if (slot >= 0) {
         filter_side* dst = a.side_a + slot;
-        dst->dec0 = vx;
+        dst->vx = vx;
         dst->thr = thr;
 #pragma unroll
         for (int c = 0; c < DIN; ++c) dst->z[c] = z[c];
@@ -358,6 +358,7 @@
 
     double shi[SLB_MAX_OUT];
     prior_sigma_bound<DIN>(cfg.gp, t.z, shi);
+    t.vx = vx;
     const long long slot = stage1_finish(a, valid, rel, sane ? decide(t, shi, cfg.gp.num_outputs) : -1, vx);
     if (slot >= 0) a.side_a[slot] = t;
     timing_mark(a, HEAD_CTAS * 8);
@@ -541,7 +542,7 @@
         for (int w = 0; w < warp; ++w) slot += s_cnt[w];
         a.list_a[slot] = rel;
         filter_side* dst = a.side_a + slot;
-        dst->dec0 = vx;
+        dst->vx = vx;
         dst->thr = thr;
         dst->z[0] = x[0];
         dst->z[1] = x[1];
@@ -788,7 +789,7 @@
     if (t.k >= 0) {
         t.rel = a.list_a[t.k];
         const filter_side* e = a.side_a + t.k;
-        t.vx = e->dec0;
+        t.vx = e->vx;
         t.thr = e->thr;
 #pragma unroll
         for (int j = 0; j < D; ++j) { t.mu[j] = e->coef[j]; t.dm[j] = e->dm[j]; }
@@ -822,18 +823,25 @@
 SLB_DEV int64_t entry_rel(const filter_side&, int64_t rel) { return rel; }
 template <int DIN, int D>
 SLB_DEV int64_t entry_rel(const cf_entry<DIN, D>& t, int64_t) { return t.rel; }
+SLB_DEV int64_t entry_slot(const filter_side&, int64_t grp) { return grp * HP + (threadIdx.x & 31); }
+template <int DIN, int D>
+SLB_DEV int64_t entry_slot(const cf_entry<DIN, D>& t, int64_t) { return t.k; }
 
 SLB_DEV void head_wait_landings(uint64_t* bar) {
     for (int b = 0; b < 3; ++b) slb_bulk::mbar_wait(bar + b, 0);
 }
 
-SLB_DEV void head_group_finish(const filter_args& a, bool mine, int outcome, int64_t rel, unsigned* s_stat) {
+SLB_DEV void head_group_finish(const filter_args& a, bool mine, int outcome, int64_t rel, int64_t k,
+                               unsigned* s_stat) {
     const int lane = threadIdx.x & 31;
     const bool undecided = mine && outcome < 0;
     if (mine && outcome >= 0) a.negative[rel] = outcome > 0 ? 1 : 0;
     if (a.fold.rec != nullptr) fold_decided(a.fold, mine && outcome >= 0, outcome > 0, rel, a.idx_begin);
     const long long slot = list_append(undecided, a.counts + 1);
-    if (undecided) a.list_b[slot] = rel;
+    if (undecided) {
+        a.list_b[slot] = rel;
+        a.slot_b[slot] = k;
+    }
     const unsigned dec = __ballot_sync(0xffffffffu, mine && !undecided);
     const unsigned und = __ballot_sync(0xffffffffu, undecided);
     if (lane == 0) {
@@ -1007,7 +1015,8 @@
                 if constexpr (CD > 0)
                     if (need) outcome = head_mean_decision(cfg, t, vx, shi, mu_s, merr_s, slot);
                 head_mark(a, HM_DECIDED);
-                head_group_finish(a, mine, outcome, entry_rel(t, rel), s_stat);
+                head_group_finish(a, mine, outcome, entry_rel(t, rel),
+                                  entry_slot(t, grp0 + (int64_t)warp * gridDim.x), s_stat);
             }
             __syncthreads();
         }
@@ -1046,7 +1055,7 @@
             }
             if (active) {
                 head_mark(a, HM_DECIDED);
-                head_group_finish(a, mine, outcome, entry_rel(t, rel), s_stat);
+                head_group_finish(a, mine, outcome, entry_rel(t, rel), entry_slot(t, grp), s_stat);
             }
         }
     }
@@ -1204,7 +1213,8 @@
 int slb_launch_refine(cudaStream_t st, const slb_sweep& cfg, int64_t n_max, int64_t idx_begin,
                       const int64_t* list, const unsigned long long* count, uint8_t* negative,
                       double* values, double* mean, double* err, double* split_partial, int* split_ticket,
-                      const slb_fold_target& fold);
+                      const slb_fold_target& fold, const filter_side* side, const int64_t* side_slot,
+                      bool closed);
 
 extern "C" {
 
@@ -1242,7 +1252,7 @@
 int64_t slb_filter_workspace(int64_t n) {
     if (n < 0) n = 0;
     if (n > CHUNK) n = CHUNK;
-    return WS_HEAD + n * (int64_t)(2 * sizeof(int64_t) + sizeof(filter_side));
+    return WS_HEAD + n * (int64_t)(3 * sizeof(int64_t) + sizeof(filter_side));
 }
 
 int slb_debug_filter_lists(int64_t n, int64_t* offsets) {
@@ -1296,7 +1306,8 @@
     double* partial = reinterpret_cast<double*>(ws + WS_PARTIAL);
     a.list_a = reinterpret_cast<int64_t*>(ws + WS_HEAD);
     a.list_b = a.list_a + cap;
-    a.side_a = reinterpret_cast<filter_side*>(a.list_b + cap);
+    a.slot_b = a.list_b + cap;
+    a.side_a = reinterpret_cast<filter_side*>(a.slot_b + cap);
     a.stats = reinterpret_cast<unsigned long long*>(stats_dev);
     const int din = cfg->gp.input_dim;
     a.chunk_rows = mean_chunk_rows(din, nomax, 24);
@@ -1325,7 +1336,8 @@
         if (!(g_filter_stages & 2)) continue;
         rc = slb_launch_refine(st, *cfg, n, idx_begin + off, a.list_b, a.counts + 1,
                                negative_dev + off, values_dev ? values_dev + off : nullptr,
-                               nullptr, nullptr, partial, tickets, a.fold);
+                               nullptr, nullptr, partial, tickets, a.fold, a.side_a, a.slot_b,
+                               a.plan.mean_scheme == SLB_MEAN_GRID_FACTORED);
         if (rc) return rc;
     }
     return 0;
@@ -1377,7 +1389,7 @@
     SLB_CUDA(cudaMemsetAsync(ws + 64, 0, SLB_SPLIT_TICKET_BYTES, st));
     return slb_launch_refine(st, *cfg, n_max, idx_begin, list_dev, count_dev, negative_dev, values_dev, mean_dev,
                              err_dev, reinterpret_cast<double*>(ws + WS_PARTIAL), reinterpret_cast<int*>(ws + 64),
-                             slb_fold_target{});
-}
-
-}
+                             slb_fold_target{}, nullptr, nullptr, false);
+}
+
+}
diff --git a/safe_learning_b200/csrc/gp_args.h b/safe_learning_b200/csrc/gp_args.h
--- a/safe_learning_b200/csrc/gp_args.h
+++ b/safe_learning_b200/csrc/gp_args.h
@@ -4,6 +4,9 @@
 enum { MODE_SWEEP_GRID = 0, MODE_SWEEP_STATES = 1, MODE_PREDICT = 2 };
 enum { SLB_SPLIT_ITEMS = 512, SLB_SPLIT_MAX = 8, SLB_SPLIT_TICKET_BYTES = 2048 };
 #define SLB_SPLIT_PARTIAL_BYTES ((size_t)SLB_SPLIT_ITEMS * SLB_MAX_OUT * (1 + SLB_MAX_OUT) * 64 * sizeof(double))
+enum { SLB_REFINE_MARKS = 16 };
+
+struct filter_side { double dec0, thr, guard, vx, coef[SLB_MAX_OUT], z[SLB_MAX_IN], dm[SLB_MAX_OUT]; };
 
 struct slb_gp_args {
     const double* points;
@@ -23,6 +26,10 @@
     double* split_partial;
     int* split_ticket;
     slb_fold_target fold;
+    const filter_side* side;
+    const int64_t* side_slot;
+    int32_t closed;
+    unsigned long long* marks;
     long long* timing;
 };
 
diff --git a/safe_learning_b200/csrc/gp_sweep.cu b/safe_learning_b200/csrc/gp_sweep.cu
--- a/safe_learning_b200/csrc/gp_sweep.cu
+++ b/safe_learning_b200/csrc/gp_sweep.cu
@@ -59,13 +59,15 @@
                          double* threshold, double* mean);
 
 static long long* g_timing_buffer = nullptr;
+static unsigned long long* g_refine_timing = nullptr;
 
 static int64_t g_refine_split = 32 * SLB_NUM_SMS;
 
 int slb_launch_refine(cudaStream_t st, const slb_sweep& cfg, int64_t n_max, int64_t idx_begin,
                       const int64_t* list, const unsigned long long* count, uint8_t* negative,
                       double* values, double* mean, double* err, double* split_partial, int* split_ticket,
-                      const slb_fold_target& fold) {
+                      const slb_fold_target& fold, const filter_side* side, const int64_t* side_slot,
+                      bool closed) {
     slb_gp_args a;
     memset(&a, 0, sizeof(a));
     a.idx_begin = idx_begin; a.mode = MODE_SWEEP_GRID;
@@ -73,6 +75,8 @@
     a.mean = mean; a.err = err;
     a.index_list = list; a.count = count;
     a.fold = fold;
+    a.side = side; a.side_slot = side_slot;
+    a.closed = side != nullptr && closed;
     a.timing = g_timing_buffer;
     const int tps[2] = {32, 64};
     const int64_t lo[2] = {0, g_refine_split};
@@ -81,11 +85,12 @@
         if (lo[v] >= hi[v] || lo[v] >= n_max) continue;
         a.count_min = lo[v]; a.count_max = hi[v];
         a.n = n_max < hi[v] ? n_max : hi[v];
-        a.split_partial = nullptr; a.split_ticket = nullptr;
+        a.split_partial = nullptr; a.split_ticket = nullptr; a.marks = nullptr;
         if (v == 0 && split_partial != nullptr) {
             if (a.n < (int64_t)SLB_NUM_SMS * tps[v]) a.n = (int64_t)SLB_NUM_SMS * tps[v];
             if ((a.n + tps[v] - 1) / tps[v] <= SLB_SPLIT_ITEMS) {
                 a.split_partial = split_partial; a.split_ticket = split_ticket;
+                a.marks = g_refine_timing;
             }
         }
         const int rc = dispatch_gp_tile(st, cfg, a, tps[v]);
@@ -143,6 +148,11 @@
     return 0;
 }
 
+int slb_debug_refine_timing(void* buffer_dev) {
+    g_refine_timing = static_cast<unsigned long long*>(buffer_dev);
+    return 0;
+}
+
 int64_t slb_packed_len(int32_t M) {
     if (M <= 0) return 0;
     const int64_t nrb = (M + 7) / 8;
diff --git a/safe_learning_b200/csrc/gp_tile.cuh b/safe_learning_b200/csrc/gp_tile.cuh
--- a/safe_learning_b200/csrc/gp_tile.cuh
+++ b/safe_learning_b200/csrc/gp_tile.cuh
@@ -133,7 +133,17 @@
     }
 }
 
-template <int DIN, bool TIMING, bool KEXPR>
+enum { RM_ENTRY, RM_PROLOGUE, RM_GEN, RM_MMA = RM_GEN + 4, RM_PARTIAL = RM_MMA + 4, RM_TICKET, RM_FACTORS, RM_DECIDED,
+       RM_EXIT, RM_FINISHER };
+static_assert(RM_FINISHER < SLB_REFINE_MARKS, "refine marks");
+SLB_DEV void refine_mark(const slb_gp_args& a, int slot) {
+    if (TP != 32 || a.marks == nullptr || (threadIdx.x & 31) != 0) return;
+    unsigned long long t;
+    asm volatile("mov.u64 %0, %%globaltimer;" : "=l"(t));
+    atomicMax(a.marks + blockIdx.x * SLB_REFINE_MARKS + slot, t);
+}
+
+template <int DIN, bool TIMING, bool KEXPR, int CD>
 SLB_DEV void gp_tile_body(const slb_sweep& cfg, const slb_gp_args& a, unsigned char* smem_raw,
                           const int64_t tile_index, const int64_t npts, const int grp, const int G,
                           const int fsel, const int FS, const bool first_tile) {
@@ -170,15 +180,47 @@
 
     if (tid < 64) exptab[tid] = exp_entry;
 
-    if (tid < TP) {
-        int64_t rel = tile0 + tid;
-        if (rel > npts - 1) rel = npts - 1;
-        if (a.index_list != nullptr) rel = a.index_list[rel];
-        double z[SLB_MAX_IN];
-        if (a.mode == MODE_PREDICT) {
-#pragma unroll
-            for (int c = 0; c < DIN; ++c) z[c] = a.points[rel * DIN + c];
+    if (tid < 2 * TP && (CD > 0 || a.side != nullptr)) {
+        const int p = tid & (TP - 1);
+        int64_t i = tile0 + p;
+        if (i > npts - 1) i = npts - 1;
+        const filter_side* e = a.side + a.side_slot[i];
+        if (tid < TP) {
+#pragma unroll
+            for (int c = 0; c < DIN; ++c) zraw[c * TP + p] = e->z[c];
         } else {
+            pre[p] = e->vx;
+            pre[TP + p] = e->thr;
+        }
+    } else if constexpr (CD == 0) {
+        if (tid < TP) {
+            int64_t rel = tile0 + tid;
+            if (rel > npts - 1) rel = npts - 1;
+            if (a.index_list != nullptr) rel = a.index_list[rel];
+            double z[SLB_MAX_IN];
+            if (a.mode == MODE_PREDICT) {
+#pragma unroll
+                for (int c = 0; c < DIN; ++c) z[c] = a.points[rel * DIN + c];
+            } else {
+                const int d = cfg.grid.ndim;
+                double x[SLB_MAX_DIM];
+                if (a.mode == MODE_SWEEP_GRID) {
+                    grid_index_to_state(cfg.grid, a.idx_begin + rel, x);
+                } else {
+                    for (int c = 0; c < d; ++c) x[c] = a.points[rel * d + c];
+                }
+                double u[SLB_MAX_OUT];
+                const int m = eval_fn_small(cfg.policy, x, u);
+                for (int c = 0; c < d; ++c) z[c] = x[c];
+                for (int c = 0; c < m; ++c) z[d + c] = u[c];
+            }
+#pragma unroll
+            for (int c = 0; c < DIN; ++c) zraw[c * TP + tid] = z[c];
+        } else if (tid < 2 * TP && a.mode != MODE_PREDICT) {
+            const int p = tid - TP;
+            int64_t rel = tile0 + p;
+            if (rel > npts - 1) rel = npts - 1;
+            if (a.index_list != nullptr) rel = a.index_list[rel];
             const int d = cfg.grid.ndim;
             double x[SLB_MAX_DIM];
             if (a.mode == MODE_SWEEP_GRID) {
@@ -186,29 +228,12 @@
             } else {
                 for (int c = 0; c < d; ++c) x[c] = a.points[rel * d + c];
             }
-            double u[SLB_MAX_OUT];
-            const int m = eval_fn_small(cfg.policy, x, u);
-            for (int c = 0; c < d; ++c) z[c] = x[c];
-            for (int c = 0; c < m; ++c) z[d + c] = u[c];
-        }
-#pragma unroll
-        for (int c = 0; c < DIN; ++c) zraw[c * TP + tid] = z[c];
-    } else if (tid < 2 * TP && a.mode != MODE_PREDICT) {
-        const int p = tid - TP;
-        int64_t rel = tile0 + p;
-        if (rel > npts - 1) rel = npts - 1;
-        if (a.index_list != nullptr) rel = a.index_list[rel];
-        const int d = cfg.grid.ndim;
-        double x[SLB_MAX_DIM];
-        if (a.mode == MODE_SWEEP_GRID) {
-            grid_index_to_state(cfg.grid, a.idx_begin + rel, x);
-        } else {
-            for (int c = 0; c < d; ++c) x[c] = a.points[rel * d + c];
-        }
-        lyapunov_state_terms(cfg, x, a.mode == MODE_SWEEP_GRID ? a.idx_begin + rel : -1, &pre[p],
-                             &pre[TP + p]);
+            lyapunov_state_terms(cfg, x, a.mode == MODE_SWEEP_GRID ? a.idx_begin + rel : -1, &pre[p],
+                                 &pre[TP + p]);
+        }
     }
     __syncthreads();
+    refine_mark(a, RM_PROLOGUE);
 
     const int wg_ = warp & 3, wr_ = warp >> 2;
     const int wslot = wr_ == 0 ? wg_ : 7 - wg_;
@@ -360,6 +385,7 @@
                     if (TIMING) { t_s0 = clock64(); t_gen += t_s0 - t_mark; }
                     __syncthreads();
                     if (TIMING) t_sync += clock64() - t_s0;
+                    refine_mark(a, RM_GEN + min(jp, 3));
                 }
                 if (TIMING) t_mark = clock64();
                 const int npairs_mma = (nkp + 1) >> 1;
@@ -380,6 +406,7 @@
                 if (mend[2] > mprev) { mma_run<2>(acc, ap, mprev, mend[2], ks_lane); mprev = mend[2]; }
                 if (mend[3] > mprev) { mma_run<3>(acc, ap, mprev, mend[3], ks_lane); mprev = mend[3]; }
                 if (TIMING) t_mma += clock64() - t_mark;
+                refine_mark(a, RM_MMA + min(jp, 3));
             }
             if (TIMING) t_mark = clock64();
 
@@ -432,6 +459,7 @@
             double* part = a.split_partial + ((size_t)blockIdx.x * SLB_MAX_OUT + f) * (NRED * TP);
             for (int i = tid; i < NRED * TP; i += NT) part[i] = tot[i];
             __syncthreads();
+            refine_mark(a, RM_PARTIAL);
             continue;
         }
         factor_epilogue(f, general, s2);
@@ -444,7 +472,9 @@
         __syncthreads();
         if (tid == 0) s_ticket = atomicAdd(a.split_ticket + tile_index, 1);
         __syncthreads();
+        refine_mark(a, RM_TICKET);
         if (s_ticket != G * FS - 1) {
+            refine_mark(a, RM_EXIT);
             if (TIMING && lane == 0) {
                 long long* t = a.timing + ((size_t)blockIdx.x * NW + warp) * 8;
                 long long g_end;
@@ -475,6 +505,7 @@
             factor_epilogue(f, general, f64mul(F.scale, F.scale));
             __syncthreads();
         }
+        refine_mark(a, RM_FACTORS);
     }
 
     if (TIMING && lane == 0) {
@@ -489,7 +520,23 @@
         const bool live = tile0 + p < npts;
         int64_t rel = live ? tile0 + p : 0;
         if (a.index_list != nullptr) rel = a.index_list[rel];
-        if (tid < 2 * TP && live) {
+        if constexpr (CD > 0) {
+            if (tid < 2 * TP && live) {
+                double mu[CD], er[CD];
+#pragma unroll
+                for (int o = 0; o < CD; ++o) {
+                    mu[o] = post[o * TP + p];
+                    er[o] = post[(SLB_MAX_OUT + o) * TP + p];
+                }
+                if (tid < TP) {
+                    if (a.mean != nullptr) for (int o = 0; o < CD; ++o) a.mean[rel * CD + o] = mu[o];
+                    if (a.err != nullptr) for (int o = 0; o < CD; ++o) a.err[rel * CD + o] = er[o];
+                    pre[2 * TP + p] = eval_quadratic_reg<CD>(cfg.lyapunov, mu);
+                } else {
+                    pre[3 * TP + p] = lyapunov_error_bound_closed<CD>(cfg, mu, er);
+                }
+            }
+        } else if (tid < 2 * TP && live) {
             double mu[SLB_MAX_OUT], er[SLB_MAX_OUT];
             for (int o = 0; o < D; ++o) {
                 mu[o] = post[o * TP + p];
@@ -520,12 +567,16 @@
             if (a.threshold != nullptr) a.threshold[rel] = r.threshold;
         }
         if (a.fold.rec != nullptr && tid < TP) fold_decided(a.fold, live, neg, rel, a.idx_begin);
-    }
-}
-
-template <int DIN, bool TIMING, bool KEXPR, int TPV>
-__global__ void __launch_bounds__(NT, CTAS_PER_SM)
-gp_tile_kernel(const __grid_constant__ slb_sweep cfg, const slb_gp_args a) {
+        refine_mark(a, RM_DECIDED);
+        if (split) {
+            refine_mark(a, RM_EXIT);
+            if (TP == 32 && a.marks != nullptr && tid == 0) a.marks[blockIdx.x * SLB_REFINE_MARKS + RM_FINISHER] = 1;
+        }
+    }
+}
+
+template <int DIN, bool TIMING, bool KEXPR, int CD>
+SLB_DEV void gp_tile_run(const slb_sweep& cfg, const slb_gp_args& a) {
     extern __shared__ __align__(16) unsigned char smem_raw[];
     int64_t tile_index = blockIdx.x;
     int64_t tile_end = tile_index + 1, tile_step = 1;
@@ -557,28 +608,43 @@
             tile_step = gridDim.x;
         }
         if (tile_index * TP >= npts) return;
+        refine_mark(a, RM_ENTRY);
     }
     for (int64_t tile = tile_index; tile < tile_end; tile += tile_step) {
-        gp_tile_body<DIN, TIMING, KEXPR>(cfg, a, smem_raw, tile, npts, grp, G, fsel, FS, tile == tile_index);
+        gp_tile_body<DIN, TIMING, KEXPR, CD>(cfg, a, smem_raw, tile, npts, grp, G, fsel, FS, tile == tile_index);
         if (tile + tile_step < tile_end) __syncthreads();
     }
 }
 
-template <int DIN, bool TIMING, bool KEXPR, int TPV = TP>
+template <int DIN, bool TIMING, bool KEXPR, int TPV>
+__global__ void __launch_bounds__(NT, CTAS_PER_SM)
+gp_tile_kernel(const __grid_constant__ slb_sweep cfg, const slb_gp_args a) {
+    gp_tile_run<DIN, TIMING, KEXPR, 0>(cfg, a);
+}
+
+template <int DIN, int CD, int TPV>
+__global__ void __launch_bounds__(NT, CTAS_PER_SM)
+gp_tile_closed_kernel(const __grid_constant__ slb_sweep cfg, const slb_gp_args a) {
+    gp_tile_run<DIN, false, false, CD>(cfg, a);
+}
+
+template <int DIN, bool TIMING, bool KEXPR, int CD = 0, int TPV = TP>
 int launch_gp_tile(cudaStream_t st, const slb_sweep& cfg, const slb_gp_args& a) {
     static_assert(TPV == TP, "TPV only disambiguates the symbol");
     static std::atomic<bool> configured[64];
+    void (*kernel)(slb_sweep, slb_gp_args) = gp_tile_kernel<DIN, TIMING, KEXPR, TP>;
+    if constexpr (CD > 0) kernel = gp_tile_closed_kernel<DIN, CD, TP>;
     int device = 0;
     SLB_CUDA(cudaGetDevice(&device));
     if (device < 0 || device >= 64 || !configured[device].load(std::memory_order_acquire)) {
-        SLB_CUDA(cudaFuncSetAttribute(gp_tile_kernel<DIN, TIMING, KEXPR, TP>,
+        SLB_CUDA(cudaFuncSetAttribute(kernel,
                                       cudaFuncAttributeMaxDynamicSharedMemorySize,
                                       (int)SMEM_TOTAL));
         if (device >= 0 && device < 64) configured[device].store(true, std::memory_order_release);
     }
     int64_t tiles = (a.n + TP - 1) / TP;
     if (a.count != nullptr && a.split_partial == nullptr && tiles > PREFETCH_CTAS) tiles = PREFETCH_CTAS;
-    gp_tile_kernel<DIN, TIMING, KEXPR, TP><<<(unsigned)tiles, NT, SMEM_TOTAL, st>>>(cfg, a);
+    kernel<<<(unsigned)tiles, NT, SMEM_TOTAL, st>>>(cfg, a);
     SLB_LAUNCH_CHECK();
     return 0;
 }
diff --git a/safe_learning_b200/csrc/gp_tile_inst.cu b/safe_learning_b200/csrc/gp_tile_inst.cu
--- a/safe_learning_b200/csrc/gp_tile_inst.cu
+++ b/safe_learning_b200/csrc/gp_tile_inst.cu
@@ -15,6 +15,9 @@
         return 1;
     }
 #endif
+#if SLB_TILE_DIN == 3
+    if (a.closed) return launch_gp_tile<3, false, false, 2>(st, cfg, a);
+#endif
     return kexpr ? launch_gp_tile<DIN, false, true>(st, cfg, a)
                  : launch_gp_tile<DIN, false, false>(st, cfg, a);
 }
```

Result: faster. 593.2 million (median of 6 runs) (+3.4%).
